# thu-ml/zhusuan

Hardware: NVIDIA H100
Metric: leapfrog-steps*chains/sec (higher is better)
Workload: dtype f32

## Files before the change

### include/zsb200.h

```cpp
#ifndef ZSB200_H_
#define ZSB200_H_
#include <stddef.h>
#include <stdint.h>

#ifdef __cplusplus
extern "C" {
#endif

#define ZSB_OK 0
#define ZSB_ERR_INVALID (-1)
#define ZSB_ERR_CUDA (-2)
#define ZSB_ERR_UNSUPPORTED (-3)

int zsb_version(void);
int zsb_last_error(char* buf, size_t n);
int zsb_device_count(void);
int zsb_stream_sync(void* stream);
int zsb_random_set_device_epoch(const uint32_t* epoch);
int zsb_random_bump_epoch(uint32_t* epoch, uint32_t by, void* stream);

enum {
  ZSB_HMC_STATE_T = 0, ZSB_HMC_STATE_STEP_SIZE = 1, ZSB_HMC_STATE_TUNER_STEP = 2,
  ZSB_HMC_STATE_LOG_EPS_BAR = 3, ZSB_HMC_STATE_H_BAR = 4, ZSB_HMC_STATE_MU = 5,
  ZSB_HMC_STATE_EWMV_T = 6, ZSB_HMC_STATE_EPS_USED = 7, ZSB_HMC_STATE_ACC_MEAN = 8,
  ZSB_HMC_STATE_FLAGS = 9 ,
  ZSB_HMC_STATE_SEARCH_LAST = 10, ZSB_HMC_STATE_SEARCH_COND = 11, ZSB_HMC_STATE_SIZE = 16
};

int zsb_logprob_normal_f32(const float* given, int64_t given_n, const float* mean, int64_t mean_n,
                           const float* logstd, int64_t logstd_n, float* out, int64_t n_out,
                           int64_t group, void* stream);
int zsb_logprob_normal_bwd_f32(const float* given, int64_t given_n, const float* mean,
                               int64_t mean_n, const float* logstd, int64_t logstd_n,
                               const float* gout, int64_t n_out, int64_t group, float* dgiven,
                               float* dmean, float* dlogstd, void* stream);
int zsb_logprob_bernoulli_f32(const float* given, int64_t given_n, const float* logits,
                              int64_t logits_n, float* out, int64_t n_out, int64_t group,
                              void* stream);
int zsb_logprob_bernoulli_bwd_f32(const float* given, int64_t given_n, const float* logits,
                                  int64_t logits_n, const float* gout, int64_t n_out,
                                  int64_t group, float* dlogits, void* stream);
int zsb_logprob_categorical_f32(const int32_t* given, int64_t given_n, const float* logits,
                                int64_t logits_rows, int64_t n_categories, float* out,
                                int64_t rows, void* stream);
int zsb_logprob_categorical_bwd_f32(const int32_t* given, int64_t given_n, const float* logits,
                                    int64_t logits_rows, int64_t n_categories, const float* gout,
                                    float* dlogits, int64_t rows, void* stream);
int zsb_logprob_dirichlet_f32(const float* given, int64_t given_rows, const float* alpha,
                              int64_t alpha_rows, int64_t n_categories, float* out, int64_t rows,
                              void* stream);
int zsb_logprob_dirichlet_bwd_given_f32(const float* given, int64_t given_rows,
                                        const float* alpha, int64_t alpha_rows,
                                        int64_t n_categories, const float* gout, float* dgiven,
                                        int64_t rows, void* stream);
int zsb_logprob_unnorm_multinomial_f32(const float* given, int64_t given_rows,
                                       const float* logits, int64_t logits_rows,
                                       int64_t n_categories, int normalize_logits, float* out,
                                       int64_t rows, void* stream);
int zsb_logprob_unnorm_multinomial_bwd_f32(const float* given, int64_t given_rows,
                                           const float* logits, int64_t logits_rows,
                                           int64_t n_categories, int normalize_logits,
                                           const float* gout, float* dlogits, int64_t rows,
                                           void* stream);
int zsb_logprob_mvn_chol_f32(const float* given, int64_t given_rows, const float* mean,
                             int64_t mean_rows, const float* cov_tril, int64_t tril_mats,
                             int64_t n_dim, float* out, float* x_out, int64_t rows, void* stream);
int zsb_logprob_mvn_chol_bwd_given_f32(const float* x_in, const float* cov_tril,
                                       int64_t tril_mats, int64_t n_dim, const float* gout,
                                       float* dgiven, int64_t rows, void* stream);
int zsb_group_sum_f32(const float* in, float* out, int64_t n_out, int64_t group, void* stream);

int zsb_reparam_normal_f32(const float* mean, int64_t mean_n, const float* logstd,
                           int64_t logstd_n, const float* eps, uint64_t seed, uint32_t iter,
                           float* z_out, float* eps_out, float* logq_out, int64_t n_out,
                           int64_t group, void* stream);
int zsb_sample_bernoulli_i32(const float* logits, int64_t logits_n, const float* u, uint64_t seed,
                             uint32_t iter, int32_t* out, int64_t n, void* stream);

int zsb_logprob_univariate_f32(int dist, const float* given, int64_t given_n, const float* a,
                               int64_t a_n, const float* b, int64_t b_n, float* out,
                               int64_t n_out, int64_t group, void* stream);
int zsb_logprob_univariate_bwd_f32(int dist, const float* given, int64_t given_n, const float* a,
                                   int64_t a_n, const float* b, int64_t b_n, const float* gout,
                                   int64_t n_out, int64_t group, float* dgiven, float* da,
                                   float* db, void* stream);

int zsb_reduce_fwd_f32(int op, const float* x, float* out, int64_t outer, int64_t K, int64_t inner,
                       void* stream);
int zsb_reduce_bwd_f32(int op, const float* x, const float* y, const float* gout, float* dx,
                       int64_t outer, int64_t K, int64_t inner, void* stream);

int zsb_vimco_signal_f32(const float* x, float* signal, float* lme, int64_t outer, int64_t K,
                         int64_t inner, void* stream);
int zsb_normalized_weights_f32(const float* x, float* w, int64_t outer, int64_t K, int64_t inner,
                               void* stream);

int zsb_linear_tc_kpad(int K);
int zsb_linear_tc_nparts(int J);
int zsb_split16_pad_f32(const float* src, int64_t rows, int K, void* planes, float* scale,
                        void* stream);
int zsb_linear_tc_slices(int64_t R, int J, int K);
int zsb_linear_tc_f32(int epi, const void* w_planes, const float* scale_w, const void* h_planes,
                      const float* scale_h, const float* bias, const float* x_obs, int64_t n_x,
                      const float* gout, float* out, float* part, int64_t R, int J, int K,
                      int relu, void* stream);
int zsb_linear_tc_amax_f32(int epi, const void* w_planes, const float* scale_w,
                           const void* h_planes, const float* scale_h, const float* bias,
                           const float* x_obs, int64_t n_x, const float* gout, float* out,
                           float* part, int64_t R, int J, int K, int relu, float* amax_scale,
                           void* stream);
int zsb_split16_dual_f32(const float* src, const float* mask_src, int64_t R, int K, void* planes,
                         float* col_sum, float* scale, int have_amax, void* stream);

int zsb_linear_tc_dgrad_f32(const void* w_planes, const float* scale_w, const void* g_planes,
                            const float* scale_g, int64_t R, int J, int K, float* out,
                            float* amax_scale, void* stream);
int zsb_linear_tc_wgrad_f32(const void* h_planes, const float* scale_h, int K,
                            const void* g_planes, const float* scale_g, int J, int64_t R,
                            float* out, float* part, void* stream);

int zsb_linear_tc_bern_sample_f32(const void* w_planes, const float* scale_w, const void* h_planes,
                                  const float* scale_h, int h_binary, const float* bias,
                                  const float* u_in, uint64_t seed, uint32_t iter, int S,
                                  void* h_out, int h_int, void* h_planes_out, float* logq,
                                  float* part, int64_t R, int J, int K, void* stream);
int zsb_linear_tc_bern_given_f32(int epi, const void* w_planes, const float* scale_w,
                                 const void* h_planes, const float* scale_h, int h_binary,
                                 const float* bias, const float* given, int S, const float* gout,
                                 float* out, float* part, int64_t R, int J, int K,
                                 float* amax_scale, void* stream);
int zsb_linear_tc_cat_sample_f32(const void* w_planes, const float* scale_w, const void* h_planes,
                                 const float* scale_h, int h_binary, const float* bias,
                                 const float* u_in, uint64_t seed, uint32_t iter, int S,
                                 int32_t* cls, void* onehot, int h_int, float* logq, int64_t R,
                                 int C, int K, void* stream);
int zsb_linear_tc_cat_given_f32(int epi, const void* w_planes, const float* scale_w,
                                const void* h_planes, const float* scale_h, int h_binary,
                                const float* bias, const float* given, int64_t n_g, int S,
                                const float* gout, float* out, int64_t R, int C, int K,
                                float* amax_scale, void* stream);
int zsb_linear_tc_normal_sample_f32(const void* w_planes, const float* scale_w,
                                    const void* h_planes, const float* scale_h, int h_binary,
                                    const float* bias, const float* eps_in, uint64_t seed,
                                    uint32_t iter, int S, float* z, float* logq, float* part,
                                    float* mean_out, float* logstd_out, int64_t R, int D, int K,
                                    float* amax_scale, void* stream);
int zsb_linear_normal_grad_f32(const float* logstd, const float* gz, const float* glq,
                               const float* eps_in, uint64_t seed, uint32_t iter,
                               const uint32_t* epoch, int reparam, int S, int64_t R, int D,
                               float* dpre, float* amax_scale, void* stream);
int zsb_linear_tc_bin_f32(int epi, const void* w_planes, const float* scale_w,
                          const void* h_planes, const float* scale_h, const float* bias,
                          const float* x_obs, int64_t n_x, const float* gout, float* out,
                          float* part, int64_t R, int J, int K, int relu, float* amax_scale,
                          void* stream);
int zsb_linear_tc_wgrad_bin_f32(const void* h_planes, const float* scale_h, int K,
                                const void* g_planes, const float* scale_g, int J, int64_t R,
                                float* out, float* part, void* stream);

int zsb_linear_tc_class_f32(const void* w_planes, const float* scale_w, const void* h_planes,
                            const float* scale_h, int h_binary, const float* bias,
                            const float* ctab, int C, const int32_t* cls, int64_t n_cls,
                            float* out, int64_t R, int J, int K, int relu, float* amax_scale,
                            void* stream);
int zsb_split16_class_f32(const float* src, const float* mask_src, int64_t R, int K,
                          const int32_t* cls, int64_t n_cls, int C, void* planes, float* col_sum,
                          float* dtab, float* scale, int have_amax, void* stream);

int zsb_split16_noisy_f32(const float* h, int64_t n_h, const float* noise, int64_t R, int K,
                          void* planes, float* scale, void* stream);
int zsb_linear_tc_bn_f32(int training, int bessel, const void* w_planes, const float* scale_w,
                         const void* h_planes, const float* scale_h, int h_binary,
                         const float* gamma, const float* beta, float* moving_mean,
                         float* moving_var, float rate, float eps, float* stats, float* a,
                         float* part, float* out, int64_t R, int J, int K, int relu,
                         float* amax_scale, void* stream);
int zsb_bn_finish_fused_f32(const float* a, const float* part, int64_t R, int J,
                            const float* gamma, const float* beta, float* moving_mean,
                            float* moving_var, float rate, float eps, float* stats, float* out,
                            int relu, float* amax_scale, void* stream);
int zsb_bn_grad_f32(int training, const float* g, const float* y, const float* a,
                    const float* stats, const float* gamma, int relu, int64_t R, int J,
                    float* part, float* dbeta, float* dgamma, void* planes, float* scale,
                    void* stream);
int zsb_bn_grad_f32out(int training, const float* g, const float* y, const float* a,
                       const float* stats, const float* gamma, int relu, int64_t R, int J,
                       float* part, float* dbeta, float* dgamma, float* da, float* scale,
                       void* stream);
int zsb_noisy_grad_f32(const float* d, const float* h, int64_t n_h, const float* noise, int64_t R,
                       int K, float* dnoise, float* dh, void* stream);

int zsb_effective_sample_size_f32(const float* samples, int64_t M, int64_t D, float* ess,
                                  void* stream);

int zsb_hmc_acc_parts(void);
int zsb_hmc_mass_parts(void);
int zsb_hmc_momentum_f32(float* p, const float* noise, const float* mass, int64_t mass_n,
                         int64_t chains, int64_t row_len, uint64_t seed, uint32_t iter,
                         uint32_t stream_id, int64_t row0, float* k_out, int accumulate,
                         const float* iter_state, void* stream);
int zsb_hmc_kinetic_f32(const float* p, const float* mass, int64_t mass_n, int64_t chains,
                        int64_t row_len, float* k_out, int accumulate, void* stream);
int zsb_hmc_leapfrog_q_f32(float* q, const float* p, const float* mass, int64_t mass_n,
                           int64_t row_len, const float* eps_dev, float scale, int64_t n,
                           void* stream);
int zsb_hmc_leapfrog_p_f32(float* p, const float* g, const float* eps_dev, float scale, int64_t n,
                           void* stream);
int zsb_hmc_mh_f32(const float* lp0, const float* lp1, const float* k0, const float* k1,
                   const float* u, uint64_t seed, uint32_t iter, int64_t row0, int64_t chains,
                   float* h0, float* h1, float* acc, int32_t* accept, float* lp_sel,
                   float* acc_part, int* n_part_out , float* state, void* stream);
int zsb_hmc_select_f32(float* q, const float* q_new, const int32_t* accept, int64_t chains,
                       int64_t row_len, void* stream);
int zsb_hmc_acc_sum_f32(const float* acc_part, int n_part, int64_t chains, float* stats,
                        void* stream);
int zsb_hmc_begin_f32(float* state, int start_search, void* stream);
int zsb_hmc_ewmv_bump_f32(float* state, void* stream);
int zsb_hmc_search_update_f32(float* state, const float* stats, float target, void* stream);
int zsb_hmc_tune_f32(float* state, const float* stats, int has_tuner, int adapt, float fresh_start,
                     float gamma, float t0, float kappa, float delta, float t_now, void* stream);
int zsb_hmc_mass_stats_f32(const float* q, const float* ewmv_mean, int64_t chains, int64_t D,
                           float* part, float* stats, void* stream);
int zsb_hmc_mass_update_f32(float* ewmv_mean, float* ewmv_var, float* mass, const float* stats,
                            float n_chains_global, int64_t D, float decay, float ewmv_t_new,
                            int adapt, int use_ones, float* state, void* stream);

int zsb_hmc_diag_normal_step_f32(float* q, const float* noise, const float* u, const float* mean,
                                 int64_t mean_n, const float* logstd, int64_t logstd_n,
                                 const float* mass, int64_t mass_n, float* state, int n_leapfrogs,
                                 int64_t chains, int64_t D, uint64_t seed, uint32_t iter,
                                 int64_t row0, int search_mode, float* p0_out, float* h0, float* h1,
                                 float* lp0, float* lp_sel, float* acc, int32_t* accept,
                                 float* acc_part, int* n_part_out , void* stream);

int zsb_hmc_dense_ntiles(int64_t D, int impl);
int zsb_hmc_dense_leapfrog_f32(const float* q_cur, const float* q_cur_lo, float* q_next,
                               float* q_next_lo, const float* p_in, float* p_out,
                               const float* P, const float* P_lo, const float* bvec,
                               const float* mu, const float* mass, const float* state,
                               float p_scale, float* lp_part, float* k_part, int64_t chains,
                               int64_t D, int impl, void* stream);
int zsb_hmc_dense_split_lo_f32(const float* q, float* lo, int64_t n, void* stream);
int zsb_hmc_dense_traj_prepare_f32(const float* q, const float* p, const float* mass, void* planes,
                                   float* scales, int64_t chains, int64_t D, void* stream);
int zsb_hmc_dense_leapfrog_h16_pass_f32(const float* q_cur, const void* q_cur_planes,
                                        float* q_next, void* q_next_planes, const float* p_in,
                                        float* p_out, const void* P_h16, const void* P_l16,
                                        float* scales, int pass_index, const float* bvec,
                                        const float* mu, const float* mass, const float* state,
                                        float p_scale, float* lp_part, float* k_part,
                                        int64_t chains, int64_t D, void* stream);
int zsb_hmc_dense_resident_h16_f32(void* planes0, void* planes1, void* spare0, void* spare1,
                                   const float* p0, float* pw, const void* P_h16,
                                   const void* P_l16, float* scales, const float* bvec,
                                   const float* mu, const float* mass, const float* state,
                                   float* lp0_part, float* lp1_part, float* k_part,
                                   int64_t chains, int64_t D, int n_leapfrogs, void* stream);
int zsb_hmc_dense_select_traj_planes_f32(float* q, const void* planes, const void* spare,
                                         const float* record, const int32_t* accept,
                                         int64_t chains, int64_t D, void* stream);
int zsb_hmc_dense_finish_f32(const float* lp_part, const float* k_part, int ntiles, int64_t chains,
                             float const_term, float* lp_out, float* k_out, void* stream);

int zsb_sample_categorical_i32(const float* logits, int64_t logit_rows, int64_t rows,
                               int64_t n_categories, int64_t n_samples, const float* u,
                               uint64_t seed, uint32_t iter, int32_t* out, void* stream);
int zsb_sample_dirichlet_f32(const float* alpha, int64_t alpha_rows, int64_t n_rows,
                             int64_t n_categories, const float* gammas, uint64_t seed,
                             uint32_t iter, float* out, void* stream);
int zsb_sample_gamma_f32(const float* alpha, int64_t alpha_rows, const float* beta,
                         int64_t beta_rows, int64_t n_rows, int64_t row_len, uint64_t seed,
                         uint32_t iter, float* out, void* stream);
int zsb_sample_base_noise_f32(int kind, float* out, int64_t n, uint64_t seed, uint32_t iter,
                              void* stream);
int zsb_sample_count_i32(int kind, const float* param, int64_t param_n, int64_t n_experiments,
                         const float* u, uint64_t seed, uint32_t iter, int32_t* out, int64_t n,
                         void* stream);

int zsb_lntm_phi_t_f32(const float* beta, int64_t n_topics, int64_t n_vocab, float* phi_t,
                       void* stream);
int zsb_lntm_logjoint_f32(const float* eta, const float* eta_mean, const float* eta_logstd,
                          const float* phi_t, const int64_t* doc_ptr, const int32_t* word_idx,
                          const float* word_cnt, const int64_t* doc_ids, const float* temperature,
                          float* lp_out, float* grad_out, int64_t chains, int64_t docs,
                          int64_t n_topics, void* stream);
int zsb_lntm_mstep_f32(const float* eta, const float* phi_t, const int64_t* doc_ptr,
                       const int32_t* word_idx, const float* word_cnt, const int64_t* doc_ids,
                       float* lp_out, float* ratio, float* theta, int64_t chains, int64_t docs,
                       int64_t nnz, int64_t n_topics, void* stream);
int zsb_lntm_mstep_grad_f32(const float* g, const float* ratio, const float* theta,
                            const float* phi_t, const int64_t* csc_ptr, const int32_t* csc_entry,
                            const int32_t* entry_doc, const int32_t* doc_slot, float* G,
                            float* dbeta, int64_t chains, int64_t docs, int64_t nnz,
                            int64_t n_topics, int64_t n_vocab, void* stream);

int zsb_pmf_logjoint_f32(const float* lat, const float* fixed, const int64_t* row_ptr,
                         const int32_t* col_idx, const float* rating, const int64_t* nbr_ptr,
                         const int32_t* nbr_idx, float logstd_lat, float logstd_fixed,
                         float logstd_rating, float* lp_out, float* grad_out, float* work,
                         int64_t K, int64_t n_rows, int64_t n_cols, int64_t D, int64_t chunk_size,
                         void* stream);

int zsb_planar_flow_fwd_f32(const float* z_in, const float* lq_in, const float* b,
                            const float* aux_u, const float* w, float* z_out, float* lq_out,
                            float* ck, int64_t R, int64_t d, int64_t n_iters, void* stream);
int zsb_planar_flow_warps(int64_t R, int64_t d, int64_t n_iters);
int zsb_planar_flow_bwd_f32(const float* ck, const float* gz_out, const float* glq,
                            const float* b, const float* aux_u, const float* w, float* gz_in,
                            float* part, float* db, float* daux_u, float* dw, int64_t R,
                            int64_t d, int64_t n_iters, void* stream);

int zsb_iaf_fwd_f32(const float* z_in, const float* lq_in, const float* m_w, const float* s_w,
                    float* z_out, float* lq_out, float* ck, int64_t R, int64_t d,
                    int64_t n_iters, int update, void* stream);
int zsb_iaf_slices(int64_t R, int64_t d, int64_t n_iters);
int zsb_iaf_bwd_f32(const float* ck, const float* gz_out, const float* glq, const float* m_w,
                    const float* s_w, float* gz_in, float* part, float* dm_w, float* ds_w,
                    int64_t R, int64_t d, int64_t n_iters, int update, void* stream);

int zsb_gp_cond_fwd_f32(const float* x, const float* z, const float* s, const float* Li,
                        const float* V, float* mean, float* stdv, float* A_out, int64_t B,
                        int64_t M, int64_t d, int64_t K, void* stream);
int zsb_gp_cond_parts(int64_t B, int64_t M, int64_t d, int64_t K);
int zsb_gp_cond_bwd_f32(const float* x, const float* z, const float* s, const float* Li,
                        const float* V, const float* A, const float* stdv, const float* g_mean,
                        const float* g_std, float* part, float* dz, float* ds, float* dLi,
                        float* dV, int64_t B, int64_t M, int64_t d, int64_t K, void* stream);

int zsb_conv3x3_fwd_f32(const float* x, const float* gate, const float* W, const float* b,
                        const float* residual, float* y, int64_t R, int64_t Hc, int64_t Wc,
                        int64_t Cin, int64_t Cout, int stride, int transpose, int relu,
                        void* stream);
int zsb_conv3x3_wgrad_parts(int64_t R, int64_t Hc, int64_t Wc, int stride);
int zsb_conv3x3_wgrad_f32(const float* big, const float* small, const float* gate, int grad_big,
                          float* part, float* dW, float* db, int64_t R, int64_t Hc, int64_t Wc,
                          int64_t Ca, int64_t Cb, int stride, void* stream);

int zsb_conv_gather_split_f32(const float* x, int64_t N, int64_t Hb, int64_t Wb, int64_t C,
                              int64_t Hs, int64_t Ws, int k, int stride, int pt, int pl,
                              void* planes, float* scale, int have_amax, void* stream);
int zsb_conv_col2im_f32(int epi, const float* cols, int64_t N, int64_t Hb, int64_t Wb, int64_t C,
                        int64_t Hs, int64_t Ws, int k, int stride, int pt, int pl,
                        const float* bias, const float* residual, const float* gamma,
                        const float* beta, const float* moving_mean, const float* moving_var,
                        float eps, int relu, float* stats, float* pre, float* part, float* out,
                        float* amax_scale, void* stream);
int zsb_conv_sigmoid_grad_f32(const float* g, const float* y, int64_t R, int C, float* gp,
                              float* part, float* db, float* scale, void* stream);
int zsb_conv_relu_grad_f32(const float* g, const float* y, int64_t R, int C, int relu, float* gp,
                           float* part, float* db, float* scale, void* stream);

int zsb_sgmcmc_parts(void);
int zsb_sgmcmc_sgld_f32(float* q, const float* g, const float* noise, float lr, int64_t chains,
                        int64_t row_len, uint64_t seed, uint32_t iter, int64_t row0,
                        void* stream);
int zsb_sgmcmc_psgld_f32(float* q, float* aux, const float* g, const float* noise, float lr,
                         float decay, float epsilon, int64_t chains, int64_t row_len,
                         uint64_t seed, uint32_t iter, int64_t row0, void* stream);
int zsb_sgmcmc_resample_v_f32(float* v, const float* noise, float lr, int64_t chains,
                              int64_t row_len, uint64_t seed, uint32_t iter, int64_t row0,
                              void* stream);
int zsb_sgmcmc_half_q_f32(float* q, const float* v, int64_t n, void* stream);
int zsb_sgmcmc_sghmc_f32(float* q, float* v, const float* g, const float* noise, float lr,
                         float alpha, float beta, int second_order, int64_t chains,
                         int64_t row_len, uint64_t seed, uint32_t iter, int64_t row0,
                         float* part, float* mean_k, void* stream);
int zsb_sgmcmc_sgnht_vec_f32(float* q, float* v, float* alpha, const float* g, const float* noise,
                             float lr, float a, float tune_rate, int second_order, int64_t chains,
                             int64_t row_len, uint64_t seed, uint32_t iter, int64_t row0,
                             float* mean_k_out, void* stream);
int zsb_sgmcmc_mean_sq_f32(const float* v, int64_t n, float* part, float* out, void* stream);
int zsb_sgmcmc_sgnht_scalar_f32(float* q, float* v, const float* alpha_eff, const float* g,
                                const float* noise, float lr, float a, int second_order,
                                int64_t chains, int64_t row_len, uint64_t seed, uint32_t iter,
                                int64_t row0, float* part, float* mean_k, void* stream);
int zsb_sgmcmc_sgnht_alpha_f32(float* out, const float* in, const float* mean_k, float coef,
                               float lr, void* stream);

int zsb_sgmcmc_sghmc_bnn_f32(float* w0, float* w1, float* v0, float* v1, const float* x,
                             const float* y, int B, int n_in, int H, const float* logstd0,
                             int64_t logstd0_n, const float* logstd1, int64_t logstd1_n,
                             float y_logstd, float n_train, float lr, float alpha, float beta,
                             int second_order, int resample, const float* noise0,
                             const float* noise1, const float* resample0, const float* resample1,
                             uint64_t seed, uint32_t iter, int64_t row0, float* part,
                             float* mean_k, int64_t chains, void* stream);

enum zsb_sgmcmc_method {
  ZSB_SGMCMC_SGHMC = 0,
  ZSB_SGMCMC_SGLD = 1,
  ZSB_SGMCMC_PSGLD = 2,
  ZSB_SGMCMC_SGNHT_VEC = 3,
  ZSB_SGMCMC_SGNHT_SCALAR = 4
};

int zsb_sgmcmc_bnn_step_f32(int method, float* w0, float* w1, float* v0, float* v1, float* aux0,
                            float* aux1, const float* alpha_eff0, const float* alpha_eff1,
                            const float* x, const float* y, int B, int n_in, int H,
                            const float* logstd0, int64_t logstd0_n, const float* logstd1,
                            int64_t logstd1_n, float y_logstd, float n_train, float lr,
                            float friction, float variance_estimate, float decay, float epsilon,
                            float variance_extra, float tune_rate, int second_order, int resample,
                            const float* noise0, const float* noise1, const float* resample0,
                            const float* resample1, uint64_t seed, uint32_t iter, int64_t row0,
                            float* part, float* mean_k0, float* mean_k1, int64_t chains,
                            void* stream);

int zsb_bnn_logjoint_f32(const float* w0, const float* w1, const float* x, const float* y,
                         int64_t B, int n_in, int H, const float* logstd0, int64_t logstd0_n,
                         const float* logstd1, int64_t logstd1_n, const float* y_logstd,
                         float n_train, float* lp, float* g0, float* g1, float* g_ylogstd,
                         float* y_mean, float* log_lik, int64_t K, void* stream);

#ifdef __cplusplus
}
#endif
#endif
```

### zhusuan_b200/_lib.py

```python
import ctypes
import os
import re

_HERE = os.path.dirname(os.path.abspath(__file__))
_ROOT = os.path.dirname(_HERE)
LIB_PATH = os.path.join(_HERE, "libzsb200.so")
HEADER_PATH = os.path.join(_ROOT, "include", "zsb200.h")

_CTYPES = {
    "int": ctypes.c_int, "int64_t": ctypes.c_int64, "uint64_t": ctypes.c_uint64,
    "uint32_t": ctypes.c_uint32, "int32_t": ctypes.c_int32,
    "float": ctypes.c_float, "size_t": ctypes.c_size_t,
}


def parse_header(path=HEADER_PATH):
    src = open(path).read()
    src = re.sub(r"/\*\s*host\s*\*/", " __host__ ", src)
    src = re.sub(r"/\*.*?\*/", " ", src, flags=re.S)
    protos = {}
    for m in re.finditer(r"\bint\s+(zsb_\w+)\s*\(([^)]*)\)\s*;", src):
        name, args = m.group(1), m.group(2).strip()
        sig = []
        if args and args != "void":
            for a in args.split(","):
                a = a.strip()
                host = "__host__" in a
                a = a.replace("__host__", "").strip()
                is_ptr = "*" in a
                toks = a.replace("*", " ").replace("const", " ").split()
                base, argname = toks[0], toks[-1]
                if is_ptr:
                    if host and base == "int":
                        ct = ctypes.POINTER(ctypes.c_int)
                    elif base == "char":
                        ct = ctypes.c_char_p
                    else:
                        ct = ctypes.c_void_p
                else:
                    ct = _CTYPES[base]
                sig.append((ct, argname, host))
        protos[name] = sig
    return protos


class ZsbError(RuntimeError):
    pass


class _Lib(object):
    def __init__(self):
        self._dll = None
        self.protos = parse_header()

    def load(self):
        if self._dll is None:
            if not os.path.exists(LIB_PATH):
                raise ZsbError(
                    "zhusuan_b200: %s is missing -- build it with "
                    "`python -c 'import __graft_entry__ as g; g.build()'` "
                    "(make -C zhusuan_b200/csrc).  There is no CPU fallback."
                    % LIB_PATH)
            dll = ctypes.CDLL(LIB_PATH)
            for name, sig in self.protos.items():
                fn = getattr(dll, name)
                fn.restype = ctypes.c_int
                fn.argtypes = [s[0] for s in sig]
            self._dll = dll
        return self._dll

    def last_error(self):
        buf = ctypes.create_string_buffer(512)
        self.load().zsb_last_error(buf, 512)
        return buf.value.decode("utf-8", "replace")

    _KERNELS = {"zsb_hmc_mass_stats_f32": 2, "zsb_hmc_dense_traj_prepare_f32": 3, "zsb_hmc_dense_resident_h16_f32": 1, "zsb_sgmcmc_sghmc_f32": 2,
                "zsb_sgmcmc_mean_sq_f32": 2, "zsb_sgmcmc_sgnht_scalar_f32": 2,
                "zsb_split16_pad_f32": 3, "zsb_linear_tc_f32": 2, "zsb_planar_flow_bwd_f32": 2,
                "zsb_iaf_bwd_f32": 2, "zsb_lntm_mstep_grad_f32": 2,
                "zsb_gp_cond_bwd_f32": 2, "zsb_conv3x3_wgrad_f32": 2,
                "zsb_conv_gather_split_f32": 3, "zsb_conv_sigmoid_grad_f32": 2,
                "zsb_conv_relu_grad_f32": 2,
                "zsb_linear_tc_bn_f32": 3, "zsb_bn_finish_fused_f32": 2, "zsb_bn_grad_f32": 5,
                "zsb_bn_grad_f32out": 3}
    launches = 0

    def call(self, name, *args):
        fn = getattr(self.load(), name)
        rc = fn(*args)
        self.launches += self._KERNELS.get(name, 1)
        if rc != 0:
            raise ZsbError("%s failed (%d): %s" % (name, rc, self.last_error()))
        return rc


lib = _Lib()


def ptr(t):
    if t is None:
        return None
    if not t.is_cuda:
        raise ZsbError(
            "zhusuan_b200 kernels need CUDA tensors (got a %s tensor); "
            "there is no CPU fallback." % t.device)
    if not t.is_contiguous():
        raise ZsbError("zhusuan_b200: non-contiguous tensor passed to a kernel")
    return t.data_ptr()


def stream():
    import torch
    return torch.cuda.current_stream().cuda_stream
```

### zhusuan_b200/csrc/hmc_dense.cu

```cuda
#include "common.cuh"

namespace {

constexpr int BM = 128, BN = 128, BK = 16;
constexpr int APAD = 4;


__global__ void __launch_bounds__(256, 2)
dense_leapfrog_simt_kernel(const float* __restrict__ q_cur, float* __restrict__ q_next,
                           const float* __restrict__ p_in, float* __restrict__ p_out,
                           const float* __restrict__ P, const float* __restrict__ bvec,
                           const float* __restrict__ mu, const float* __restrict__ mass,
                           const float* __restrict__ state, float p_scale,
                           float* __restrict__ lp_part, float* __restrict__ k_part,
                           int64_t chains, int D) {
  __shared__ __align__(16) float As[2][BK][BM + APAD];
  __shared__ __align__(16) float Bs[2][BK][BN];

  const int tid = threadIdx.x;
  const int tx = tid & 15, ty = tid >> 4;
  const int64_t m0 = (int64_t)blockIdx.y * BM;
  const int n0 = blockIdx.x * BN;

  const int a_row = tid >> 2;
  const int a_k4 = (tid & 3) * 4;
  const int b_row = tid >> 5;
  const int b_n4 = (tid & 31) * 4;

  float acc[8][8];
#pragma unroll
  for (int i = 0; i < 8; ++i)
#pragma unroll
    for (int j = 0; j < 8; ++j) acc[i][j] = 0.f;

  float4 a_reg[2], b_reg[2];
  auto load_tiles = [&](int k0) {
#pragma unroll
    for (int h = 0; h < 2; ++h) {
      const int64_t m = m0 + a_row + h * 64;
      a_reg[h] = (m < chains)
                     ? *reinterpret_cast<const float4*>(q_cur + m * D + k0 + a_k4)
                     : make_float4(0.f, 0.f, 0.f, 0.f);
      const int n = n0 + b_n4;
      b_reg[h] = (n < D) ? *reinterpret_cast<const float4*>(P + (int64_t)(k0 + b_row + h * 8) * D + n)
                         : make_float4(0.f, 0.f, 0.f, 0.f);
    }
  };
  auto store_tiles = [&](int buf) {
#pragma unroll
    for (int h = 0; h < 2; ++h) {
      const int r = a_row + h * 64;
      As[buf][a_k4 + 0][r] = a_reg[h].x;
      As[buf][a_k4 + 1][r] = a_reg[h].y;
      As[buf][a_k4 + 2][r] = a_reg[h].z;
      As[buf][a_k4 + 3][r] = a_reg[h].w;
      *reinterpret_cast<float4*>(&Bs[buf][b_row + h * 8][b_n4]) = b_reg[h];
    }
  };

  const int nk = D / BK;
  load_tiles(0);
  store_tiles(0);
  __syncthreads();
  for (int kt = 0; kt < nk; ++kt) {
    const int buf = kt & 1;
    if (kt + 1 < nk) load_tiles((kt + 1) * BK);
#pragma unroll
    for (int k = 0; k < BK; ++k) {
      const float4 a0 = *reinterpret_cast<const float4*>(&As[buf][k][ty * 4]);
      const float4 a1 = *reinterpret_cast<const float4*>(&As[buf][k][64 + ty * 4]);
      const float4 b0 = *reinterpret_cast<const float4*>(&Bs[buf][k][tx * 4]);
      const float4 b1 = *reinterpret_cast<const float4*>(&Bs[buf][k][64 + tx * 4]);
      const float a[8] = {a0.x, a0.y, a0.z, a0.w, a1.x, a1.y, a1.z, a1.w};
      const float b[8] = {b0.x, b0.y, b0.z, b0.w, b1.x, b1.y, b1.z, b1.w};
#pragma unroll
      for (int i = 0; i < 8; ++i)
#pragma unroll
        for (int j = 0; j < 8; ++j) acc[i][j] = fmaf(a[i], b[j], acc[i][j]);
    }
    if (kt + 1 < nk) store_tiles(buf ^ 1);
    __syncthreads();
  }

  const float eps = state[ZSB_ST_EPS_USED];
  const float s2 = mul(eps, p_scale);
#pragma unroll
  for (int i = 0; i < 8; ++i) {
    const int64_t m = m0 + (i < 4 ? ty * 4 + i : 64 + ty * 4 + (i - 4));
    float lp_acc = 0.f, k_acc = 0.f;
    if (m < chains) {
#pragma unroll
      for (int h = 0; h < 2; ++h) {
        const int n = n0 + h * 64 + tx * 4;
        if (n < D) {
          const float4 pv = *reinterpret_cast<const float4*>(p_in + m * D + n);
          const float4 qv = *reinterpret_cast<const float4*>(q_cur + m * D + n);
          const float4 ms = *reinterpret_cast<const float4*>(mass + n);
          float4 bv = make_float4(0.f, 0.f, 0.f, 0.f), mv = bv;
          if (bvec) bv = *reinterpret_cast<const float4*>(bvec + n);
          if (mu) mv = *reinterpret_cast<const float4*>(mu + n);
          const float pe[4] = {pv.x, pv.y, pv.z, pv.w}, qe[4] = {qv.x, qv.y, qv.z, qv.w};
          const float me[4] = {ms.x, ms.y, ms.z, ms.w}, be[4] = {bv.x, bv.y, bv.z, bv.w};
          const float ue[4] = {mv.x, mv.y, mv.z, mv.w};
          float pn[4], qn[4];
#pragma unroll
          for (int j = 0; j < 4; ++j) {
            const float g = sub(be[j], acc[i][h * 4 + j]);
            pn[j] = add(pe[j], mul(s2, g));
            qn[j] = add(qe[j], mul(eps, fdiv(pn[j], me[j])));
            lp_acc += (qe[j] - ue[j]) * g;
            k_acc += fdiv(mul(pn[j], pn[j]), me[j]);
          }
          *reinterpret_cast<float4*>(p_out + m * D + n) = make_float4(pn[0], pn[1], pn[2], pn[3]);
          if (q_next)
            *reinterpret_cast<float4*>(q_next + m * D + n) = make_float4(qn[0], qn[1], qn[2], qn[3]);
        }
      }
    }
    if (lp_part) {
#pragma unroll
      for (int o = 8; o > 0; o >>= 1) lp_acc += __shfl_xor_sync(0xffffffffu, lp_acc, o);
      if (tx == 0 && m < chains) lp_part[(int64_t)blockIdx.x * chains + m] = lp_acc;
    }
    if (k_part) {
#pragma unroll
      for (int o = 8; o > 0; o >>= 1) k_acc += __shfl_xor_sync(0xffffffffu, k_acc, o);
      if (tx == 0 && m < chains) k_part[(int64_t)blockIdx.x * chains + m] = k_acc;
    }
  }
}

__global__ void __launch_bounds__(256) dense_finish_kernel(const float* __restrict__ lp_part,
                                                           const float* __restrict__ k_part,
                                                           int ntiles, int64_t chains,
                                                           float const_term,
                                                           float* __restrict__ lp_out,
                                                           float* __restrict__ k_out) {
  for (int64_t c = (int64_t)blockIdx.x * blockDim.x + threadIdx.x; c < chains;
       c += (int64_t)gridDim.x * blockDim.x) {
    if (lp_part && lp_out) {
      float s = 0.f;
      for (int t = 0; t < ntiles; ++t) s += lp_part[(int64_t)t * chains + c];
      lp_out[c] = add(mul(0.5f, s), const_term);
    }
    if (k_part && k_out) {
      float s = 0.f;
      for (int t = 0; t < ntiles; ++t) s += k_part[(int64_t)t * chains + c];
      k_out[c] = mul(0.5f, s);
    }
  }
}

}

int zsb_dense_leapfrog_tc_launch(const float* q_cur, const float* q_cur_lo, float* q_next,
                                 float* q_next_lo, const float* p_in, float* p_out,
                                 const float* P_hi, const float* P_lo, const float* bvec,
                                 const float* mu, const float* mass, const float* state,
                                 float p_scale, float* lp_part, float* k_part, int64_t chains,
                                 int D, cudaStream_t st);
int zsb_dense_split_lo_launch(const float* q, float* lo, int64_t n, cudaStream_t st);
int zsb_dense_tc_ntiles(int D);
int zsb_dense_leapfrog_h16_launch(const float* q_cur, const void* q_cur_planes, float* q_next,
                                  void* q_next_planes, const float* p_in, float* p_out,
                                  const void* P_h16, const void* P_l16, float* scales,
                                  int pass_index, const float* bvec, const float* mu,
                                  const float* mass, const float* state, float p_scale,
                                  float* lp_part, float* k_part, int64_t chains, int D,
                                  cudaStream_t st);
int zsb_dense_h16_prepare_launch(const float* q, const float* p, const float* mass, void* planes,
                                 float* scales, int64_t chains, int64_t D, cudaStream_t st);
int zsb_dense_res_h16_launch(void* planes0, void* planes1, void* spare0, void* spare1,
                             const float* p0, float* pw, const void* P_h16, const void* P_l16,
                             float* scales, const float* bvec, const float* mu, const float* mass,
                             const float* state, float* lp0_part, float* lp1_part, float* k_part,
                             int64_t chains, int D, int L, cudaStream_t st);
int zsb_dense_select_planes_launch(float* q, const void* planes, const void* spare,
                                   const float* record, const int32_t* accept, int64_t chains,
                                   int64_t D, cudaStream_t st);

extern "C" {

int zsb_hmc_dense_ntiles(int64_t D, int impl) {
  if (impl == 1) return zsb_dense_tc_ntiles((int)D);
  return (int)zsb_ceil_div(D, BN);
}

int zsb_hmc_dense_leapfrog_f32(const float* q_cur, const float* q_cur_lo, float* q_next,
                               float* q_next_lo, const float* p_in, float* p_out,
                               const float* P, const float* P_lo, const float* bvec,
                               const float* mu, const float* mass, const float* state,
                               float p_scale, float* lp_part, float* k_part, int64_t chains,
                               int64_t D, int impl, void* stream) {
  ZSB_REQUIRE(q_cur && p_in && p_out && P && mass && state, "zsb_hmc_dense_leapfrog_f32: null arg");
  ZSB_REQUIRE(chains > 0 && D > 0 && D % BK == 0 && D <= (1 << 20),
              "zsb_hmc_dense_leapfrog_f32: D must be a positive multiple of 16");
  ZSB_REQUIRE(q_next != q_cur, "zsb_hmc_dense_leapfrog_f32: q_next must not alias q_cur");
  cudaStream_t st = (cudaStream_t)stream;
  if (impl == 1) {
    ZSB_REQUIRE(P_lo && q_cur_lo, "zsb_hmc_dense_leapfrog_f32: impl 1 needs the P_lo / q_lo splits");
    return zsb_dense_leapfrog_tc_launch(q_cur, q_cur_lo, q_next, q_next_lo, p_in, p_out, P, P_lo,
                                        bvec, mu, mass, state, p_scale, lp_part, k_part, chains,
                                        (int)D, st);
  }
  ZSB_REQUIRE(impl == 0, "zsb_hmc_dense_leapfrog_f32: unknown impl %d", impl);
  dim3 grid((unsigned)zsb_ceil_div(D, BN), (unsigned)zsb_ceil_div(chains, BM));
  dense_leapfrog_simt_kernel<<<grid, 256, 0, st>>>(q_cur, q_next, p_in, p_out, P, bvec, mu, mass,
                                                   state, p_scale, lp_part, k_part, chains, (int)D);
  return zsb_check_launch("hmc_dense_leapfrog_simt");
}

int zsb_hmc_dense_split_lo_f32(const float* q, float* lo, int64_t n, void* stream) {
  ZSB_REQUIRE(q && lo && n >= 0, "zsb_hmc_dense_split_lo_f32: bad args");
  if (n == 0) return ZSB_OK;
  return zsb_dense_split_lo_launch(q, lo, n, (cudaStream_t)stream);
}

int zsb_hmc_dense_traj_prepare_f32(const float* q, const float* p, const float* mass, void* planes,
                                   float* scales, int64_t chains, int64_t D, void* stream) {
  ZSB_REQUIRE(q && p && mass && planes && scales && chains > 0 && D > 0,
              "zsb_hmc_dense_traj_prepare_f32: bad args");
  return zsb_dense_h16_prepare_launch(q, p, mass, planes, scales, chains, D,
                                      (cudaStream_t)stream);
}
int zsb_hmc_dense_leapfrog_h16_pass_f32(const float* q_cur, const void* q_cur_planes,
                                        float* q_next, void* q_next_planes, const float* p_in,
                                        float* p_out, const void* P_h16, const void* P_l16,
                                        float* scales, int pass_index, const float* bvec,
                                        const float* mu, const float* mass, const float* state,
                                        float p_scale, float* lp_part, float* k_part,
                                        int64_t chains, int64_t D, void* stream) {
  ZSB_REQUIRE(q_cur && p_in && p_out && P_h16 && P_l16 && mass && state && scales,
              "zsb_hmc_dense_leapfrog_h16_pass_f32: null arg");
  ZSB_REQUIRE(q_next != q_cur, "zsb_hmc_dense_leapfrog_h16_pass_f32: q_next must not alias q_cur");
  ZSB_REQUIRE(pass_index >= 0, "zsb_hmc_dense_leapfrog_h16_pass_f32: pass_index < 0");
  return zsb_dense_leapfrog_h16_launch(q_cur, q_cur_planes, q_next, q_next_planes, p_in, p_out,
                                       P_h16, P_l16, scales, pass_index, bvec, mu, mass, state,
                                       p_scale, lp_part, k_part, chains, (int)D,
                                       (cudaStream_t)stream);
}

int zsb_hmc_dense_resident_h16_f32(void* planes0, void* planes1, void* spare0, void* spare1,
                                   const float* p0, float* pw, const void* P_h16,
                                   const void* P_l16, float* scales, const float* bvec,
                                   const float* mu, const float* mass, const float* state,
                                   float* lp0_part, float* lp1_part, float* k_part,
                                   int64_t chains, int64_t D, int n_leapfrogs, void* stream) {
  ZSB_REQUIRE(planes0 && planes1 && spare0 && spare1 && p0 && pw && P_h16 && P_l16 && scales &&
                  mass && state && lp0_part && lp1_part && k_part,
              "zsb_hmc_dense_resident_h16_f32: null arg");
  ZSB_REQUIRE(p0 != pw, "zsb_hmc_dense_resident_h16_f32: aliased buffers");
  return zsb_dense_res_h16_launch(planes0, planes1, spare0, spare1, p0, pw, P_h16, P_l16, scales,
                                  bvec, mu, mass, state, lp0_part, lp1_part, k_part, chains, (int)D,
                                  n_leapfrogs, (cudaStream_t)stream);
}
int zsb_hmc_dense_select_traj_planes_f32(float* q, const void* planes, const void* spare,
                                         const float* record, const int32_t* accept,
                                         int64_t chains, int64_t D, void* stream) {
  ZSB_REQUIRE(q && planes && spare && record && accept && chains > 0 && D > 0 && D % 2 == 0,
              "zsb_hmc_dense_select_traj_planes_f32: bad args");
  return zsb_dense_select_planes_launch(q, planes, spare, record, accept, chains, D,
                                        (cudaStream_t)stream);
}

int zsb_hmc_dense_finish_f32(const float* lp_part, const float* k_part, int ntiles, int64_t chains,
                             float const_term, float* lp_out, float* k_out, void* stream) {
  ZSB_REQUIRE(chains > 0 && ntiles > 0, "zsb_hmc_dense_finish_f32: bad sizes");
  int64_t blocks = zsb_ceil_div(chains, 256);
  if (blocks > ZSB_NUM_SMS * 8) blocks = ZSB_NUM_SMS * 8;
  dense_finish_kernel<<<(unsigned)blocks, 256, 0, (cudaStream_t)stream>>>(
      lp_part, k_part, ntiles, chains, const_term, lp_out, k_out);
  return zsb_check_launch("hmc_dense_finish");
}

}
```

### zhusuan_b200/csrc/hmc_dense_epilogue.cuh

```cuda
#pragma once
#include "tc_common.cuh"

namespace {

constexpr int kScaleHdr = 8, kScaleRec = 4;
constexpr float kPlaneKeep = 65280.f;
constexpr float kHalfOverflow = 65520.f;

__device__ __forceinline__ const float* scale_rec(const float* scales, int pass) {
  return scales + kScaleHdr + kScaleRec * pass;
}
__device__ __forceinline__ bool plane_spare_in(const float* scales, int pass) {
  return pass > 0 && __float_as_uint(scale_rec(scales, pass)[3]) != 0u;
}
__device__ __forceinline__ float plane_scale_in(const float* scales, int pass) {
  return scale_rec(scales, pass)[plane_spare_in(scales, pass) ? 1 : 0];
}
__device__ __forceinline__ float next_plane_scale(const float* __restrict__ scales, int pass,
                                                  float eps, float s2, float sq) {
  const float* r = scale_rec(scales, pass);
  const float mq = r[2];
  const float drift = pass == 0 ? eps * r[3] : mq + r[2 - kScaleRec];
  const float bound = mq + drift + eps * s2 * scales[7] * (scales[5] + scales[4] * mq);
  if (bound * sq < kPlaneKeep || !(bound <= 3.0e38f)) return sq;
  return pow2_plane_scale(bound);
}
__device__ __forceinline__ void publish_plane_scale(float* __restrict__ scales, int pass,
                                                    float sq_next, float sq_alt, float qmax,
                                                    bool overflow, int quarter, int lane) {
  unsigned int* r = reinterpret_cast<unsigned int*>(scales + kScaleHdr + kScaleRec * (pass + 1));
  const float mq = warp_max(qmax);
  const bool any_overflow = __any_sync(0xffffffffu, overflow);
  if (lane == 0) {
    atomicMax(r + 2, __float_as_uint(mq));
    if (any_overflow) atomicOr(r + 3, 1u);
  }
  if (blockIdx.x == 0 && quarter == 0 && lane == 0) {
    reinterpret_cast<float*>(r)[0] = sq_next;
    reinterpret_cast<float*>(r)[1] = sq_alt;
    r[kScaleRec + 2] = 0u;
    r[kScaleRec + 3] = 0u;
  }
}

struct EpiArgs {
  const float* __restrict__ q_cur; float* __restrict__ q_next; float* __restrict__ q_next_lo;
  const float* __restrict__ p_in; float* __restrict__ p_out;
  float* __restrict__ lp_part; float* __restrict__ k_part;
  int64_t chains; int D;
  float acc_scale; float q_scale;
};
template <int H16>
__device__ __forceinline__ void store_split(const EpiArgs& a, float* __restrict__ lo_f32,
                                            __half* __restrict__ hi_pl, __half* __restrict__ lo_pl,
                                            uint32_t off, float qn) {
  if (H16) {
    const float x = qn * a.q_scale;
    const __half h = __float2half_rn(x);
    hi_pl[off] = h;
    lo_pl[off] = __float2half_rn(x - __half2float(h));
  } else {
    lo_f32[off] = qn - __uint_as_float(__float_as_uint(qn) & 0xFFFFE000u);
  }
}
template <int MODE, int DC, int H16>
__device__ __forceinline__ void epilogue_half_tile(const EpiArgs& a, uint32_t trow, int n,
                                                   bool n_ok, int64_t c0, int64_t part_row,
                                                   int lane, float s2, float eps_over_m,
                                                   float inv_m, float b_n, float mu_n,
                                                   float& amax) {
  constexpr int NCOL = BN;
  const uint32_t D = DC ? (uint32_t)DC : (uint32_t)a.D;
  const int64_t chains = a.chains;
  const bool has_next = a.q_next != nullptr;
  const bool warp_n_ok = __all_sync(0xffffffffu, n_ok);
  const bool fast_tile = warp_n_ok && (c0 + NCOL <= chains);

  const int64_t off_t = c0 * (int64_t)D + n;
  const float* __restrict__ pin0 = a.p_in + off_t;
  const float* __restrict__ qc0 = a.q_cur + off_t;
  float* __restrict__ po0 = a.p_out + off_t;
  float* __restrict__ qn0 = has_next ? a.q_next + off_t : nullptr;
  float* __restrict__ lo0 = (has_next && H16 == 0) ? a.q_next_lo + off_t : nullptr;
  __half* __restrict__ hi_pl0 =
      (has_next && H16 == 1) ? reinterpret_cast<__half*>(a.q_next_lo) + off_t : nullptr;
  __half* __restrict__ lo_pl0 = (has_next && H16 == 1) ? hi_pl0 + chains * (int64_t)D : nullptr;

  auto compute = [&](const uint32_t* v, const float* pe, const float* qe, int c) {
    const size_t cb = (size_t)c * D;
    float* __restrict__ po = po0 + cb;
    float* __restrict__ qn_p = has_next ? qn0 + cb : nullptr;
    float* __restrict__ lo_p = (has_next && H16 == 0) ? lo0 + cb : nullptr;
    __half* __restrict__ hp = (has_next && H16 == 1) ? hi_pl0 + cb : nullptr;
    __half* __restrict__ lp = (has_next && H16 == 1) ? lo_pl0 + cb : nullptr;
    float lpv[MODE >= 1 ? 16 : 1], kv[MODE >= 2 ? 16 : 1];
#pragma unroll
    for (int j = 0; j < 16; ++j) {
      const float g = b_n - a.acc_scale * __uint_as_float(v[j]);
      const float pn = fmaf(s2, g, pe[j]);
      po[(uint32_t)j * D] = pn;
      if (MODE >= 1) lpv[j] = (qe[j] - mu_n) * g;
      if (MODE >= 2) kv[j] = pn * pn * inv_m;
      if (has_next) {
        const float qn = fmaf(eps_over_m, pn, qe[j]);
        qn_p[(uint32_t)j * D] = qn;
        if (H16 == 1) amax = fmaxf(amax, fabsf(qn));
        store_split<H16>(a, lo_p, hp, lp, (uint32_t)j * D, qn);
      }
    }
    if (MODE >= 1) {
      const float sum = warp_transpose_sum16(lpv, lane);
      if (lane < 16) a.lp_part[part_row + c0 + c + lane] = sum;
    }
    if (MODE >= 2) {
      const float sum = warp_transpose_sum16(kv, lane);
      if (lane < 16) a.k_part[part_row + c0 + c + lane] = sum;
    }
  };
  auto load = [&](float* pe, float* qe, int c) {
    const float* __restrict__ pin = pin0 + (size_t)c * D;
    const float* __restrict__ qc = qc0 + (size_t)c * D;
#pragma unroll
    for (int j = 0; j < 16; ++j) {
      pe[j] = __ldcs(pin + (uint32_t)j * D);
      qe[j] = __ldg(qc + (uint32_t)j * D);
    }
  };

  if (fast_tile) {
    float pa[16], qa[16], pb[16], qb[16];
    uint32_t va[16], vb[16];
    load(pa, qa, 0);
#pragma unroll 1
    for (int c = 0; c < NCOL; c += 32) {
      load(pb, qb, c + 16);
      acc_ld16(trow + 4u * (uint32_t)c, va);
      compute(va, pa, qa, c);
      if (c + 32 < NCOL) load(pa, qa, c + 32);
      acc_ld16(trow + 4u * (uint32_t)(c + 16), vb);
      compute(vb, pb, qb, c + 16);
    }
  } else {
#pragma unroll 1
    for (int c = 0; c < NCOL; c += 16) {
      uint32_t v[16];
      acc_ld16(trow + 4u * (uint32_t)c, v);
      const int64_t cbase = c0 + c;
      if (cbase < chains) {
        const size_t cb = (size_t)c * D;
        float pe[16], qe[16];
        float lpv[MODE >= 1 ? 16 : 1], kv[MODE >= 2 ? 16 : 1];
#pragma unroll
        for (int j = 0; j < 16; ++j) {
          const bool ok = n_ok && cbase + j < chains;
          pe[j] = ok ? pin0[cb + (uint32_t)j * D] : 0.f;
          qe[j] = ok ? qc0[cb + (uint32_t)j * D] : 0.f;
        }
#pragma unroll
        for (int j = 0; j < 16; ++j) {
          const bool ok = n_ok && cbase + j < chains;
          const float g = b_n - a.acc_scale * __uint_as_float(v[j]);
          const float pn = fmaf(s2, g, pe[j]);
          if (MODE >= 1) lpv[j] = ok ? (qe[j] - mu_n) * g : 0.f;
          if (MODE >= 2) kv[j] = ok ? pn * pn * inv_m : 0.f;
          if (ok) {
            po0[cb + (uint32_t)j * D] = pn;
            if (has_next) {
              const float qn = fmaf(eps_over_m, pn, qe[j]);
              qn0[cb + (uint32_t)j * D] = qn;
              if (H16 == 1) amax = fmaxf(amax, fabsf(qn));
              store_split<H16>(a, lo0 + cb, hi_pl0 + cb, lo_pl0 + cb, (uint32_t)j * D, qn);
            }
          }
        }
        if (MODE >= 1) {
          const float sum = warp_transpose_sum16(lpv, lane);
          if (lane < 16 && cbase + lane < chains) a.lp_part[part_row + cbase + lane] = sum;
        }
        if (MODE >= 2) {
          const float sum = warp_transpose_sum16(kv, lane);
          if (lane < 16 && cbase + lane < chains) a.k_part[part_row + cbase + lane] = sum;
        }
      }
    }
  }
}

}
```

### zhusuan_b200/csrc/hmc_dense_res.cu

```cuda
#include "hmc_dense_epilogue.cuh"

namespace {

struct ResEpi {
  const __half* __restrict__ hi_cur; const __half* __restrict__ lo_cur;
  __half* __restrict__ hi_nxt; __half* __restrict__ lo_nxt;
  const __half* __restrict__ hi_cur_s; const __half* __restrict__ lo_cur_s;
  __half* __restrict__ hi_nxt_s; __half* __restrict__ lo_nxt_s;
  const float* __restrict__ p_in; float* __restrict__ p_out;
  float* __restrict__ lp_part; float* __restrict__ k_part;
  int64_t chains; int D;
  float sq, inv_sq, acc_scale;
  float rescale;
};

template <int MODE, int NEXT, int DC, bool SPARE>
__device__ __forceinline__ void epilogue_planes(const ResEpi& a, uint32_t trow, int n, bool n_ok,
                                                int64_t c0, int64_t part_row, int lane, float s2,
                                                float eps_over_m_sq, float inv_m, float b_n,
                                                float mu_n, float& qmax) {
  constexpr int NCOL = BN;
  const uint32_t D = DC ? (uint32_t)DC : (uint32_t)a.D;
  const int64_t chains = a.chains;
  const bool warp_n_ok = __all_sync(0xffffffffu, n_ok);
  const bool fast_tile = warp_n_ok && (c0 + NCOL <= chains);
  const int64_t off_t = c0 * (int64_t)D + n;
  const float* __restrict__ pin0 = a.p_in + off_t;
  float* __restrict__ po0 = a.p_out + off_t;
  const unsigned short* __restrict__ hc0 =
      reinterpret_cast<const unsigned short*>(a.hi_cur) + off_t;
  const unsigned short* __restrict__ lc0 =
      reinterpret_cast<const unsigned short*>(a.lo_cur) + off_t;
  __half* __restrict__ hn0 = NEXT ? a.hi_nxt + off_t : nullptr;
  __half* __restrict__ ln0 = NEXT ? a.lo_nxt + off_t : nullptr;
  __half* __restrict__ hs0 = SPARE ? a.hi_nxt_s + off_t : nullptr;
  __half* __restrict__ ls0 = SPARE ? a.lo_nxt_s + off_t : nullptr;

  auto element = [&](float acc, float p, uint32_t hl, float& pn, float& lpv, float& kv,
                     float& Qn) {
    const float Q = __half2float(__ushort_as_half((unsigned short)(hl & 0xFFFFu))) +
                    __half2float(__ushort_as_half((unsigned short)(hl >> 16)));
    const float g = b_n - a.acc_scale * acc;
    pn = fmaf(s2, g, p);
    if (MODE >= 1) lpv = (Q * a.inv_sq - mu_n) * g;
    if (MODE >= 2) kv = pn * pn * inv_m;
    if (NEXT) Qn = fmaf(eps_over_m_sq, pn, Q);
  };

  if (fast_tile) {
    auto load = [&](float* pe, uint32_t* he, int c) {
      const size_t cb = (size_t)c * D;
#pragma unroll
      for (int j = 0; j < 16; ++j) {
        pe[j] = __ldcg(pin0 + cb + (uint32_t)j * D);
        const uint32_t h = __ldcg(hc0 + cb + (uint32_t)j * D);
        const uint32_t l = __ldcg(lc0 + cb + (uint32_t)j * D);
        he[j] = h | (l << 16);
      }
    };
    float ss_a = 0.f, ss_b = 0.f;
    auto compute = [&](const uint32_t* v, const float* pe, const uint32_t* he, int c, float& ss) {
      const size_t cb = (size_t)c * D;
      float lpv[MODE >= 1 ? 16 : 1], kv[MODE >= 2 ? 16 : 1];
#pragma unroll
      for (int j = 0; j < 16; j += 2) {
        float pn[2], lp1[2] = {0.f, 0.f}, k1[2] = {0.f, 0.f}, Qn[2] = {0.f, 0.f};
#pragma unroll
        for (int t = 0; t < 2; ++t) {
          element(__uint_as_float(v[j + t]), pe[j + t], he[j + t], pn[t], lp1[t], k1[t], Qn[t]);
          po0[cb + (uint32_t)(j + t) * D] = pn[t];
          if (MODE >= 1) lpv[j + t] = lp1[t];
          if (MODE >= 2) kv[j + t] = k1[t];
          if (NEXT && !SPARE) ss = fmaf(Qn[t], Qn[t], ss);
          if (SPARE) qmax = fmaxf(qmax, fabsf(Qn[t]));
        }
        if (NEXT) {
          const __half2 h2 = __floats2half2_rn(Qn[0], Qn[1]);
          const float2 hf = __half22float2(h2);
          const __half2 l2 = __floats2half2_rn(Qn[0] - hf.x, Qn[1] - hf.y);
          hn0[cb + (uint32_t)j * D] = __low2half(h2);
          hn0[cb + (uint32_t)(j + 1) * D] = __high2half(h2);
          ln0[cb + (uint32_t)j * D] = __low2half(l2);
          ln0[cb + (uint32_t)(j + 1) * D] = __high2half(l2);
        }
        if (SPARE) {
          const float x0 = Qn[0] * a.rescale, x1 = Qn[1] * a.rescale;
          const __half2 h2 = __floats2half2_rn(x0, x1);
          const float2 hf = __half22float2(h2);
          const __half2 l2 = __floats2half2_rn(x0 - hf.x, x1 - hf.y);
          hs0[cb + (uint32_t)j * D] = __low2half(h2);
          hs0[cb + (uint32_t)(j + 1) * D] = __high2half(h2);
          ls0[cb + (uint32_t)j * D] = __low2half(l2);
          ls0[cb + (uint32_t)(j + 1) * D] = __high2half(l2);
        }
      }
      if (MODE >= 1) {
        const float sum = warp_transpose_sum16(lpv, lane);
        if (lane < 16) a.lp_part[part_row + c0 + c + lane] = sum;
      }
      if (MODE >= 2) {
        const float sum = warp_transpose_sum16(kv, lane);
        if (lane < 16) a.k_part[part_row + c0 + c + lane] = sum;
      }
    };
    float pa[16], pb[16];
    uint32_t ha[16], hb[16], va[16], vb[16];
    load(pa, ha, 0);
#pragma unroll 1
    for (int c = 0; c < NCOL; c += 32) {
      load(pb, hb, c + 16);
      acc_ld16(trow + 4u * (uint32_t)c, va);
      compute(va, pa, ha, c, ss_a);
      if (c + 32 < NCOL) load(pa, ha, c + 32);
      acc_ld16(trow + 4u * (uint32_t)(c + 16), vb);
      compute(vb, pb, hb, c + 16, ss_b);
    }
    if (NEXT && !SPARE) {
      const float norm = sqrtf(ss_a + ss_b) * (1.f + 0x1p-10f);
      qmax = fmaxf(qmax, norm == norm ? norm : INFINITY);
    }
  } else {
#pragma unroll 1
    for (int c = 0; c < NCOL; c += 16) {
      uint32_t v[16];
      acc_ld16(trow + 4u * (uint32_t)c, v);
      const int64_t cbase = c0 + c;
      if (cbase < chains) {
        const size_t cb = (size_t)c * D;
        float lpv[MODE >= 1 ? 16 : 1], kv[MODE >= 2 ? 16 : 1];
#pragma unroll
        for (int j = 0; j < 16; ++j) {
          const bool ok = n_ok && cbase + j < chains;
          float p = 0.f;
          uint32_t hl = 0u;
          if (ok) {
            p = __ldcg(pin0 + cb + (uint32_t)j * D);
            hl = (uint32_t)__ldcg(hc0 + cb + (uint32_t)j * D) |
                 ((uint32_t)__ldcg(lc0 + cb + (uint32_t)j * D) << 16);
          }
          float pn, lp1 = 0.f, k1 = 0.f, Qn = 0.f;
          element(__uint_as_float(v[j]), p, hl, pn, lp1, k1, Qn);
          const __half hh = __float2half_rn(Qn);
          const __half ll = __float2half_rn(Qn - __half2float(hh));
          if (NEXT && ok) qmax = fmaxf(qmax, fabsf(Qn));
          if (MODE >= 1) lpv[j] = ok ? lp1 : 0.f;
          if (MODE >= 2) kv[j] = ok ? k1 : 0.f;
          if (ok) {
            po0[cb + (uint32_t)j * D] = pn;
            if (NEXT) {
              hn0[cb + (uint32_t)j * D] = hh;
              ln0[cb + (uint32_t)j * D] = ll;
            }
            if (SPARE) {
              const float x = Qn * a.rescale;
              const __half hs = __float2half_rn(x);
              hs0[cb + (uint32_t)j * D] = hs;
              ls0[cb + (uint32_t)j * D] = __float2half_rn(x - __half2float(hs));
            }
          }
        }
        if (MODE >= 1) {
          const float sum = warp_transpose_sum16(lpv, lane);
          if (lane < 16 && cbase + lane < chains) a.lp_part[part_row + cbase + lane] = sum;
        }
        if (MODE >= 2) {
          const float sum = warp_transpose_sum16(kv, lane);
          if (lane < 16 && cbase + lane < chains) a.k_part[part_row + cbase + lane] = sum;
        }
      }
    }
  }
}


struct ProducerState {
  int spare_in, n0, c0;
};
__device__ __forceinline__ ProducerState& producer_state() {
  __shared__ ProducerState ps;
  return ps;
}

template <int MODE, int NEXT, int DC, int CX, int CY>
struct ResW {
  static constexpr int KIND = 1, RB = 64, MNA = 0, MNB = 0;
  static constexpr int CLUSTER = CX * CY;
  static constexpr int KE = RB / 2;
  static constexpr uint32_t TX = Cfg<RB>::STAGE;
  CUtensorMap m_phi, m_plo, m_qhi, m_qlo, m_shi, m_slo;
  ResEpi ea;
  const float* bvec; const float* mu; const float* mass; const float* state;
  float* scales;
  float p_scale;
  int n_blk, D_rt, pass;
  struct EpiState { float qmax = 0.f; };

  __device__ __forceinline__ int D() const { return DC ? DC : D_rt; }
  __host__ __device__ __forceinline__ int64_t units() const {
    return ((ea.chains + BN - 1) / BN) * (int64_t)n_blk;
  }
  __device__ __forceinline__ void tile(int64_t u, int& nb, int64_t& cb) const {
    const uint64_t cu = (uint64_t)u / CLUSTER;
    const int r = (int)((uint64_t)u % CLUSTER);
    const uint32_t nbx = (uint32_t)(n_blk / CX);
    nb = (int)(cu % nbx) * CX + r % CX;
    cb = (int64_t)(cu / nbx) * CY + r / CX;
  }
  __device__ __forceinline__ void kb_range(int64_t, int& kb0, int& kb1) const {
    kb0 = 0;
    kb1 = D() / KE;
  }
  __device__ __forceinline__ void prefetch() const {
    tma_prefetch_desc(&m_phi); tma_prefetch_desc(&m_plo);
    tma_prefetch_desc(&m_qhi); tma_prefetch_desc(&m_qlo);
    tma_prefetch_desc(&m_shi); tma_prefetch_desc(&m_slo);
    producer_state().spare_in = plane_spare_in(scales, pass);
  }
  __device__ __forceinline__ void load(int64_t u, int kb, uint32_t sa, uint32_t fb) const {
    using C = Cfg<RB>;
    ProducerState& ps = producer_state();
    if (kb == 0) {
      int nb;
      int64_t cb;
      tile(u, nb, cb);
      ps.n0 = nb * BM;
      ps.c0 = (int)cb * BN;
    }
    const int n0 = ps.n0, c0 = ps.c0;
    const bool s = ps.spare_in != 0;
    const CUtensorMap* qh = s ? &m_shi : &m_qhi;
    const CUtensorMap* ql = s ? &m_slo : &m_qlo;
    const int r = (int)(u % CLUSTER), rx = r % CX, ry = r / CX;
    if constexpr (CY == 1) {
      tma_load_2d(sa, &m_phi, fb, kb * KE, n0);
      tma_load_2d(sa + C::A_TILE, &m_plo, fb, kb * KE, n0);
    } else {
      constexpr int rows = BM / CY;
      uint16_t mask = 0;
#pragma unroll
      for (int y = 0; y < CY; ++y) mask |= (uint16_t)(1u << (y * CX + rx));
      const uint32_t o = (uint32_t)(ry * rows * RB);
      tma_load_2d_mc(sa + o, &m_phi, fb, kb * KE, n0 + ry * rows, mask);
      tma_load_2d_mc(sa + C::A_TILE + o, &m_plo, fb, kb * KE, n0 + ry * rows, mask);
    }
    if constexpr (CX == 1) {
      tma_load_2d(sa + 2 * C::A_TILE, qh, fb, kb * KE, c0);
      tma_load_2d(sa + 2 * C::A_TILE + C::B_TILE, ql, fb, kb * KE, c0);
    } else {
      constexpr int rows = BN / CX;
      const uint16_t mask = (uint16_t)(((1u << CX) - 1u) << (ry * CX));
      const uint32_t o = (uint32_t)(rx * rows * RB);
      tma_load_2d_mc(sa + 2 * C::A_TILE + o, qh, fb, kb * KE, c0 + rx * rows, mask);
      tma_load_2d_mc(sa + 2 * C::A_TILE + C::B_TILE + o, ql, fb, kb * KE, c0 + rx * rows, mask);
    }
  }
  __device__ __forceinline__ float sq_alt(float eps, float sq) const {
    return next_plane_scale(scales, pass, eps, mul(eps, p_scale), sq);
  }
  __device__ __forceinline__ void epilogue(int64_t u, uint32_t trow, int quarter, int lane,
                                           EpiState& st) const {
    int nb;
    int64_t cb;
    tile(u, nb, cb);
    const int n = nb * BM + quarter * 32 + lane;
    const int64_t c0 = cb * BN;
    const bool n_ok = n < D();
    const float eps = state[ZSB_ST_EPS_USED];
    const float s2 = mul(eps, p_scale);
    const bool spare_in = plane_spare_in(scales, pass);
    const float sq = plane_scale_in(scales, pass);
    const float m_n = n_ok ? mass[n] : 1.f;
    const float eps_over_m_sq = mul(fdiv(eps, m_n), sq);
    const float inv_m = fdiv(1.f, m_n);
    const float b_n = (n_ok && bvec) ? bvec[n] : 0.f;
    const float mu_n = (n_ok && mu) ? mu[n] : 0.f;
    const int64_t part_row = (int64_t)(nb * 4 + quarter) * ea.chains;
    ResEpi a = ea;
    if (spare_in) {
      a.hi_cur = ea.hi_cur_s;
      a.lo_cur = ea.lo_cur_s;
    }
    a.sq = sq;
    a.inv_sq = fdiv(1.f, sq);
    a.acc_scale = 1.f / (scales[3] * sq);
    a.rescale = NEXT ? sq_alt(eps, sq) * a.inv_sq : 1.f;
    if (a.rescale == 1.f)
      epilogue_planes<MODE, NEXT, DC, false>(a, trow, n, n_ok, c0, part_row, lane, s2,
                                             eps_over_m_sq, inv_m, b_n, mu_n, st.qmax);
    else
      epilogue_planes<MODE, NEXT, DC, true>(a, trow, n, n_ok, c0, part_row, lane, s2,
                                            eps_over_m_sq, inv_m, b_n, mu_n, st.qmax);
  }
  __device__ __forceinline__ void epi_finish(EpiState& st, int quarter, int lane) const {
    if (!NEXT) return;
    const float sq = plane_scale_in(scales, pass);
    const float alt = sq_alt(state[ZSB_ST_EPS_USED], sq);
    publish_plane_scale(scales, pass, sq, alt, st.qmax * (1.f / sq),
                        alt != sq && !(st.qmax < kHalfOverflow), quarter, lane);
  }
};

constexpr int RES_CX = 2, RES_CY = 1;

template <int DC, int CX, int CY>
int res_pass(const CUtensorMap& phi, const CUtensorMap& plo, const CUtensorMap& qhi,
             const CUtensorMap& qlo, const CUtensorMap& shi, const CUtensorMap& slo,
             const ResEpi& ea, const float* bvec, const float* mu, const float* mass,
             const float* state, float* scales, int pass, float p_scale, int n_blk, int D,
             int mode, cudaStream_t st) {
  if (mode == 1) {
    const ResW<1, 1, DC, CX, CY> w{phi, plo, qhi, qlo, shi, slo, ea, bvec, mu, mass, state,
                                   scales, p_scale, n_blk, D, pass};
    return tc_launch(w, st, "hmc_dense_resident");
  }
  if (mode == 0) {
    const ResW<0, 1, DC, CX, CY> w{phi, plo, qhi, qlo, shi, slo, ea, bvec, mu, mass, state,
                                   scales, p_scale, n_blk, D, pass};
    return tc_launch(w, st, "hmc_dense_resident");
  }
  const ResW<2, 0, DC, CX, CY> w{phi, plo, qhi, qlo, shi, slo, ea, bvec, mu, mass, state, scales,
                                 p_scale, n_blk, D, pass};
  return tc_launch(w, st, "hmc_dense_resident");
}

template <int DC>
int res_pass(bool cluster, const CUtensorMap& phi, const CUtensorMap& plo, const CUtensorMap& qhi,
             const CUtensorMap& qlo, const CUtensorMap& shi, const CUtensorMap& slo,
             const ResEpi& ea, const float* bvec, const float* mu, const float* mass,
             const float* state, float* scales, int pass, float p_scale, int n_blk, int D,
             int mode, cudaStream_t st) {
  return cluster ? res_pass<DC, RES_CX, RES_CY>(phi, plo, qhi, qlo, shi, slo, ea, bvec, mu, mass,
                                                state, scales, pass, p_scale, n_blk, D, mode, st)
                 : res_pass<DC, 1, 1>(phi, plo, qhi, qlo, shi, slo, ea, bvec, mu, mass, state,
                                      scales, pass, p_scale, n_blk, D, mode, st);
}

__global__ void __launch_bounds__(256) select_planes_kernel(float* __restrict__ q,
                                                            const __half* __restrict__ planes,
                                                            const __half* __restrict__ spare,
                                                            const float* __restrict__ record,
                                                            const int32_t* __restrict__ accept,
                                                            int64_t chains, int64_t D) {
  const bool use_spare = __float_as_uint(record[3]) != 0u;
  const float inv_sq = 1.f / record[use_spare ? 1 : 0];
  if (use_spare) planes = spare;
  const int lane = threadIdx.x & 31;
  const int n8 = (int)(D >> 3);
  const int64_t wstride = (int64_t)gridDim.x * 8;
  for (int64_t c = (int64_t)blockIdx.x * 8 + (threadIdx.x >> 5); c < chains; c += wstride) {
    if (!accept[c]) continue;
    const uint4* __restrict__ hi = reinterpret_cast<const uint4*>(planes + c * D);
    const uint4* __restrict__ lo = reinterpret_cast<const uint4*>(planes + (chains + c) * D);
    float4* __restrict__ qr = reinterpret_cast<float4*>(q + c * D);
    for (int i0 = lane; i0 < n8; i0 += 128) {
      uint4 h[4], l[4];
#pragma unroll
      for (int u = 0; u < 4; ++u) {
        const int i = i0 + 32 * u;
        if (i < n8) { h[u] = __ldcs(hi + i); l[u] = __ldcs(lo + i); }
      }
#pragma unroll
      for (int u = 0; u < 4; ++u) {
        const int i = i0 + 32 * u;
        if (i < n8) {
          const uint32_t hw[4] = {h[u].x, h[u].y, h[u].z, h[u].w};
          const uint32_t lw[4] = {l[u].x, l[u].y, l[u].z, l[u].w};
          float o[8];
#pragma unroll
          for (int k = 0; k < 4; ++k) {
            const float2 hf = __half22float2(*reinterpret_cast<const __half2*>(&hw[k]));
            const float2 lf = __half22float2(*reinterpret_cast<const __half2*>(&lw[k]));
            o[2 * k] = (hf.x + lf.x) * inv_sq;
            o[2 * k + 1] = (hf.y + lf.y) * inv_sq;
          }
          qr[2 * i] = make_float4(o[0], o[1], o[2], o[3]);
          qr[2 * i + 1] = make_float4(o[4], o[5], o[6], o[7]);
        }
      }
    }
  }
}

}

int zsb_dense_res_h16_launch(void* planes0, void* planes1, void* spare0, void* spare1,
                             const float* p0, float* pw,
                             const void* P_h16, const void* P_l16, float* scales,
                             const float* bvec, const float* mu, const float* mass,
                             const float* state, float* lp0_part, float* lp1_part, float* k_part,
                             int64_t chains, int D, int L, cudaStream_t st) {
  if (D % 64 != 0 || D < 64 || L < 1 || chains <= 0 || chains >= (1LL << 31)) {
    zsb_set_error("dense_res: needs D %% 64 == 0, n_leapfrogs >= 1");
    return ZSB_ERR_INVALID;
  }
  if (planes0 == planes1 || !spare0 || !spare1 || spare0 == spare1) {
    zsb_set_error("dense_res: planes1, spare0 and spare1 must be separate work buffers");
    return ZSB_ERR_INVALID;
  }
  const int n_blk = (D + BM - 1) / BM;
  const int64_t c_blk = (chains + BN - 1) / BN;
  const bool cluster = n_blk % RES_CX == 0 && c_blk % RES_CY == 0;
  const uint32_t p_box = cluster ? BM / RES_CY : BM, q_box = cluster ? BN / RES_CX : BN;
  CUtensorMap phi, plo, qhi[2], qlo[2], shi[2], slo[2];
  int rc;
  constexpr int RB = ResW<0, 1, 0, 1, 1>::RB;
  if ((rc = make_map(&phi, P_h16, (uint64_t)D, (uint64_t)D, p_box, RB, 1))) return rc;
  if ((rc = make_map(&plo, P_l16, (uint64_t)D, (uint64_t)D, p_box, RB, 1))) return rc;
  __half* pl[2] = {reinterpret_cast<__half*>(planes0), reinterpret_cast<__half*>(planes1)};
  __half* sp[2] = {reinterpret_cast<__half*>(spare0), reinterpret_cast<__half*>(spare1)};
  const int64_t plane = chains * (int64_t)D;
  for (int b = 0; b < 2; ++b) {
    if ((rc = make_map(&qhi[b], pl[b], (uint64_t)chains, (uint64_t)D, q_box, RB, 1))) return rc;
    if ((rc = make_map(&qlo[b], pl[b] + plane, (uint64_t)chains, (uint64_t)D, q_box, RB, 1)))
      return rc;
    if ((rc = make_map(&shi[b], sp[b], (uint64_t)chains, (uint64_t)D, q_box, RB, 1))) return rc;
    if ((rc = make_map(&slo[b], sp[b] + plane, (uint64_t)chains, (uint64_t)D, q_box, RB, 1)))
      return rc;
  }
  for (int i = 0; i <= L; ++i) {
    const bool last = i == L;
    const int buf = i & 1;
    const ResEpi ea{pl[buf], pl[buf] + plane, pl[buf ^ 1], pl[buf ^ 1] + plane,
                    sp[buf], sp[buf] + plane, sp[buf ^ 1], sp[buf ^ 1] + plane,
                    i == 0 ? p0 : pw, pw, i == 0 ? lp0_part : lp1_part, k_part, chains, D,
                    1.f, 1.f, 1.f, 1.f};
    const int mode = last ? 2 : (i == 0 ? 1 : 0);
    const float p_scale = (i > 0 && !last) ? 1.f : 0.5f;
    rc = (D == 1024)
             ? res_pass<1024>(cluster, phi, plo, qhi[buf], qlo[buf], shi[buf], slo[buf], ea, bvec,
                              mu, mass, state, scales, i, p_scale, n_blk, D, mode, st)
             : res_pass<0>(cluster, phi, plo, qhi[buf], qlo[buf], shi[buf], slo[buf], ea, bvec, mu,
                           mass, state, scales, i, p_scale, n_blk, D, mode, st);
    if (rc != ZSB_OK) return rc;
  }
  return ZSB_OK;
}

#ifdef ZSB_PASS_PROFILE
extern "C" int zsb_pass_profile_read(unsigned long long* host, int ctas) {
  if (ctas < 0 || ctas > PASS_PROF_CTAS) return ZSB_ERR_INVALID;
  const size_t bytes = sizeof(unsigned long long) * PASS_PROF_SLOTS * (size_t)ctas;
  if (cudaMemcpyFromSymbol(host, g_pass_prof, bytes) != cudaSuccess) return ZSB_ERR_CUDA;
  static unsigned long long zeros[PASS_PROF_CTAS * PASS_PROF_SLOTS];
  if (cudaMemcpyToSymbol(g_pass_prof, zeros, sizeof(zeros)) != cudaSuccess) return ZSB_ERR_CUDA;
  return ZSB_OK;
}
#endif

int zsb_dense_select_planes_launch(float* q, const void* planes, const void* spare,
                                   const float* record, const int32_t* accept, int64_t chains,
                                   int64_t D, cudaStream_t st) {
  ZSB_REQUIRE(D % 8 == 0, "zsb_dense_select_planes: D must be a multiple of 8");
  int64_t blocks = zsb_ceil_div(chains, 8);
  if (blocks > ZSB_NUM_SMS * 16) blocks = ZSB_NUM_SMS * 16;
  if (blocks < 1) blocks = 1;
  select_planes_kernel<<<(unsigned)blocks, 256, 0, st>>>(
      q, reinterpret_cast<const __half*>(planes), reinterpret_cast<const __half*>(spare), record,
      accept, chains, D);
  return zsb_check_launch("hmc_select_planes");
}
```

### zhusuan_b200/csrc/hmc_dense_tc.cu

```cuda
#include "hmc_dense_epilogue.cuh"

namespace {

template <int OP, int MODE, int DC>
struct DenseW {
  static constexpr int KIND = OP, RB = 128, MNA = 0, MNB = 0;
  static constexpr int KE = OP ? RB / 2 : RB / 4;
  static constexpr uint32_t TX = Cfg<RB>::STAGE;
  CUtensorMap m_phi, m_plo, m_qhi, m_qlo;
  EpiArgs ea;
  const float* bvec; const float* mu; const float* mass; const float* state;
  float* scales;
  float p_scale;
  int n_blk, D_rt, pass_index;
  struct EpiState { float amax = 0.f; };

  __device__ __forceinline__ int D() const { return DC ? DC : D_rt; }
  __host__ __device__ __forceinline__ int64_t units() const {
    return ((ea.chains + BN - 1) / BN) * (int64_t)n_blk;
  }
  __device__ __forceinline__ void kb_range(int64_t, int& kb0, int& kb1) const {
    kb0 = 0;
    kb1 = D() / KE;
  }
  __device__ __forceinline__ void prefetch() const {
    tma_prefetch_desc(&m_phi);
    tma_prefetch_desc(&m_plo);
    tma_prefetch_desc(&m_qhi);
    tma_prefetch_desc(&m_qlo);
  }
  __device__ __forceinline__ void load(int64_t u, int kb, uint32_t sa, uint32_t fb) const {
    using C = Cfg<RB>;
    const int n0 = (int)(u % n_blk) * BM;
    const int c0 = (int)(u / n_blk) * BN;
    tma_load_2d(sa, &m_phi, fb, kb * KE, n0);
    tma_load_2d(sa + C::A_TILE, &m_plo, fb, kb * KE, n0);
    tma_load_2d(sa + 2 * C::A_TILE, &m_qhi, fb, kb * KE, c0);
    tma_load_2d(sa + 2 * C::A_TILE + C::B_TILE, &m_qlo, fb, kb * KE, c0);
  }
  __device__ __forceinline__ void epilogue(int64_t u, uint32_t trow, int quarter, int lane,
                                           EpiState& st) const {
    const int nb = (int)(u % n_blk);
    const int n = nb * BM + quarter * 32 + lane;
    const int64_t c0 = (u / n_blk) * BN;
    const int Dv = D();
    const bool n_ok = n < Dv;
    const float eps = state[ZSB_ST_EPS_USED];
    const float s2 = mul(eps, p_scale);
    const float m_n = n_ok ? mass[n] : 1.f;
    const float eps_over_m = fdiv(eps, m_n);
    const float inv_m = fdiv(1.f, m_n);
    const float b_n = (n_ok && bvec) ? bvec[n] : 0.f;
    const float mu_n = (n_ok && mu) ? mu[n] : 0.f;
    const int64_t part_row = (int64_t)(nb * 4 + quarter) * ea.chains;
    EpiArgs a = ea;
    if (OP == 1) {
      const float sq = scale_rec(scales, pass_index)[0];
      a.acc_scale = 1.f / (scales[3] * sq);
      a.q_scale = ea.q_next ? next_plane_scale(scales, pass_index, eps, s2, sq) : sq;
    }
    epilogue_half_tile<MODE, DC, OP>(a, trow, n, n_ok, c0, part_row, lane, s2, eps_over_m, inv_m,
                                     b_n, mu_n, st.amax);
  }
  __device__ __forceinline__ void epi_finish(EpiState& st, int quarter, int lane) const {
    if (OP == 1 && ea.q_next) {
      const float eps = state[ZSB_ST_EPS_USED];
      const float sq = next_plane_scale(scales, pass_index, eps, mul(eps, p_scale),
                                        scale_rec(scales, pass_index)[0]);
      publish_plane_scale(scales, pass_index, sq, sq, st.amax, false, quarter, lane);
    }
  }
};

__global__ void __launch_bounds__(256) split_lo_kernel(const float* __restrict__ q,
                                                       float* __restrict__ lo, int64_t n4) {
  for (int64_t i = (int64_t)blockIdx.x * blockDim.x + threadIdx.x; i < n4;
       i += (int64_t)gridDim.x * blockDim.x) {
    const float4 v = reinterpret_cast<const float4*>(q)[i];
    float4 r;
    r.x = v.x - __uint_as_float(__float_as_uint(v.x) & 0xFFFFE000u);
    r.y = v.y - __uint_as_float(__float_as_uint(v.y) & 0xFFFFE000u);
    r.z = v.z - __uint_as_float(__float_as_uint(v.z) & 0xFFFFE000u);
    r.w = v.w - __uint_as_float(__float_as_uint(v.w) & 0xFFFFE000u);
    reinterpret_cast<float4*>(lo)[i] = r;
  }
}

__global__ void __launch_bounds__(256) absmax_kernel(const float* __restrict__ q,
                                                     const float* __restrict__ p,
                                                     const float* __restrict__ mass, int64_t n,
                                                     int64_t D, float* __restrict__ scales) {
  float mq = 0.f, mv = 0.f;
  for (int64_t i = (int64_t)blockIdx.x * blockDim.x + threadIdx.x; i < n;
       i += (int64_t)gridDim.x * blockDim.x) {
    mq = finite_absmax(mq, q[i]);
    mv = finite_absmax(mv, fdiv(p[i], mass[i % D]));
  }
  mq = warp_max(mq);
  mv = warp_max(mv);
  if ((threadIdx.x & 31) == 0) {
    atomicMax(reinterpret_cast<unsigned int*>(scales) + 2, __float_as_uint(mq));
    atomicMax(reinterpret_cast<unsigned int*>(scales) + 6, __float_as_uint(mv));
  }
}
__global__ void scale_kernel(float* __restrict__ scales, const float* __restrict__ mass,
                             int64_t D) {
  float w = 0.f;
  for (int64_t i = threadIdx.x; i < D; i += 32) w = finite_absmax(w, fdiv(1.f, mass[i]));
  w = warp_max(w);
  if (threadIdx.x != 0) return;
  unsigned int* u = reinterpret_cast<unsigned int*>(scales);
  const float mq = __uint_as_float(u[2]), mv = __uint_as_float(u[6]);
  const float sq = pow2_plane_scale(mq);
  scales[0] = sq;
  scales[1] = 1.f / (scales[3] * sq);
  u[2] = 0u;
  float* r0 = scales + kScaleHdr;
  r0[0] = sq;
  r0[1] = sq;
  r0[2] = mq;
  r0[3] = mv;
  u[kScaleHdr + kScaleRec + 2] = 0u;
  u[kScaleHdr + kScaleRec + 3] = 0u;
  scales[7] = w;
  u[6] = 0u;
}
__global__ void __launch_bounds__(256) split16_kernel(const float* __restrict__ q,
                                                      __half* __restrict__ planes, int64_t n,
                                                      const float* __restrict__ scales) {
  const float sq = scales[0];
  for (int64_t i = (int64_t)blockIdx.x * blockDim.x + threadIdx.x; i < n;
       i += (int64_t)gridDim.x * blockDim.x) {
    const float x = q[i] * sq;
    const __half h = __float2half_rn(x);
    planes[i] = h;
    planes[n + i] = __float2half_rn(x - __half2float(h));
  }
}

template <int OP>
int launch_dense(const float* q_cur, const void* q_lo, float* q_next, void* q_next_lo,
                 const float* p_in, float* p_out, const void* P_hi, const void* P_lo,
                 const float* bvec, const float* mu, const float* mass, const float* state,
                 float p_scale, float* lp_part, float* k_part, int64_t chains, int D, float* scales,
                 int pass_index, cudaStream_t st, const char* what) {
  if (k_part && !lp_part) {
    zsb_set_error("%s: k_part requires lp_part", what);
    return ZSB_ERR_INVALID;
  }
  constexpr int RB = DenseW<OP, 0, 0>::RB;
  CUtensorMap m_phi, m_plo, m_qhi, m_qlo;
  int rc;
  if ((rc = make_map(&m_phi, P_hi, (uint64_t)D, (uint64_t)D, BM, RB, OP))) return rc;
  if ((rc = make_map(&m_plo, P_lo, (uint64_t)D, (uint64_t)D, BM, RB, OP))) return rc;
  const void* qh = OP ? q_lo : (const void*)q_cur;
  const void* ql = OP ? (const void*)(reinterpret_cast<const __half*>(q_lo) + chains * D) : q_lo;
  if ((rc = make_map(&m_qhi, qh, (uint64_t)chains, (uint64_t)D, BN, RB, OP))) return rc;
  if ((rc = make_map(&m_qlo, ql, (uint64_t)chains, (uint64_t)D, BN, RB, OP))) return rc;
  const EpiArgs ea{q_cur, q_next, reinterpret_cast<float*>(q_next_lo), p_in, p_out, lp_part,
                   k_part, chains, D, 1.f, 1.f};
  const int n_blk = (D + BM - 1) / BM;
#define ZSB_DENSE(MODE, DCV)                                                                   \
  do {                                                                                         \
    const DenseW<OP, MODE, DCV> w{m_phi, m_plo, m_qhi, m_qlo, ea, bvec, mu, mass, state,       \
                                  scales, p_scale, n_blk, D, pass_index};                      \
    return tc_launch(w, st, what);                                                             \
  } while (0)
#define ZSB_DENSE_MODE(DCV)                                                                    \
  do {                                                                                         \
    if (k_part) ZSB_DENSE(2, DCV);                                                             \
    else if (lp_part) ZSB_DENSE(1, DCV);                                                       \
    else ZSB_DENSE(0, DCV);                                                                    \
  } while (0)
  if constexpr (OP == 1)
    if (D == 1024) ZSB_DENSE_MODE(1024);
  ZSB_DENSE_MODE(0);
#undef ZSB_DENSE_MODE
#undef ZSB_DENSE
}

}

int zsb_dense_tc_ntiles(int D) { return 4 * ((D + BM - 1) / BM); }

int zsb_dense_leapfrog_tc_launch(const float* q_cur, const float* q_cur_lo, float* q_next,
                                 float* q_next_lo, const float* p_in, float* p_out,
                                 const float* P_hi, const float* P_lo, const float* bvec,
                                 const float* mu, const float* mass, const float* state,
                                 float p_scale, float* lp_part, float* k_part, int64_t chains,
                                 int D, cudaStream_t st) {
  if (D % 32 != 0 || D < 32) {
    zsb_set_error("dense_tc: D must be a multiple of 32");
    return ZSB_ERR_INVALID;
  }
  if (chains >= (1LL << 31) || (q_next && !q_next_lo) || !q_cur_lo) {
    zsb_set_error("dense_tc: bad arguments");
    return ZSB_ERR_INVALID;
  }
  return launch_dense<0>(q_cur, q_cur_lo, q_next, q_next_lo, p_in, p_out, P_hi, P_lo, bvec, mu,
                         mass, state, p_scale, lp_part, k_part, chains, D, nullptr, 0, st,
                         "hmc_dense_leapfrog_tc");
}

int zsb_dense_split_lo_launch(const float* q, float* lo, int64_t n, cudaStream_t st) {
  if (n % 4 != 0) {
    zsb_set_error("dense split: element count must be a multiple of 4");
    return ZSB_ERR_INVALID;
  }
  const int64_t n4 = n / 4;
  int64_t blocks = zsb_ceil_div(n4, 256);
  if (blocks > ZSB_NUM_SMS * 16) blocks = ZSB_NUM_SMS * 16;
  if (blocks < 1) blocks = 1;
  split_lo_kernel<<<(unsigned)blocks, 256, 0, st>>>(q, lo, n4);
  return zsb_check_launch("hmc_dense_split_lo");
}

int zsb_dense_leapfrog_h16_launch(const float* q_cur, const void* q_cur_planes, float* q_next,
                                  void* q_next_planes, const float* p_in, float* p_out,
                                  const void* P_h16, const void* P_l16, float* scales,
                                  int pass_index, const float* bvec, const float* mu,
                                  const float* mass, const float* state, float p_scale,
                                  float* lp_part, float* k_part, int64_t chains, int D,
                                  cudaStream_t st) {
  if (D % 64 != 0 || D < 64) {
    zsb_set_error("dense_h16: D must be a multiple of 64");
    return ZSB_ERR_INVALID;
  }
  if (chains >= (1LL << 31) || (q_next && !q_next_planes) || !q_cur_planes || !scales ||
      pass_index < 0) {
    zsb_set_error("dense_h16: bad arguments");
    return ZSB_ERR_INVALID;
  }
  return launch_dense<1>(q_cur, q_cur_planes, q_next, q_next_planes, p_in, p_out, P_h16, P_l16,
                         bvec, mu, mass, state, p_scale, lp_part, k_part, chains, D, scales,
                         pass_index, st, "hmc_dense_leapfrog_h16");
}

int zsb_dense_h16_prepare_launch(const float* q, const float* p, const float* mass, void* planes,
                                 float* scales, int64_t chains, int64_t D, cudaStream_t st) {
  const int64_t n = chains * D;
  int64_t blocks = zsb_ceil_div(n, 256 * 8);
  if (blocks > ZSB_NUM_SMS * 16) blocks = ZSB_NUM_SMS * 16;
  if (blocks < 1) blocks = 1;
  absmax_kernel<<<(unsigned)blocks, 256, 0, st>>>(q, p, mass, n, D, scales);
  scale_kernel<<<1, 32, 0, st>>>(scales, mass, D);
  split16_kernel<<<(unsigned)blocks, 256, 0, st>>>(q, reinterpret_cast<__half*>(planes), n, scales);
  return zsb_check_launch("hmc_dense_h16_prepare");
}
```

### zhusuan_b200/csrc/tc_common.cuh

```cuda
#pragma once
#include "common.cuh"
#include <cuda.h>
#include <cuda_fp16.h>

namespace {

constexpr int BM = 128;
constexpr int BN = 128;
constexpr int NUM_EPI_WARPS = 4;
constexpr int PRODUCER_WARP = 4;
constexpr int EPI_WARP0 = 5;
constexpr int NUM_THREADS = 32 * (EPI_WARP0 + NUM_EPI_WARPS);
constexpr int ACC_LD = BN + 4;
constexpr int ACC_BYTES = BM * ACC_LD * 4;
constexpr unsigned long long WAIT_TIMEOUT_NS = 2000000000ULL;

enum PassProfSlot {
  PROF_MMA_TOTAL,
  PROF_MMA_FULL,
  PROF_MMA_TEMPTY,
  PROF_MMA_STORE,
  PROF_PROD_EMPTY,
  PROF_EPI_TFULL,
  PROF_EPI_UNIT,
  PROF_UNITS,
  PASS_PROF_SLOTS
};
constexpr int PASS_PROF_CTAS = 1024;
#ifdef ZSB_PASS_PROFILE
constexpr bool kPassProfile = true;
__device__ unsigned long long g_pass_prof[PASS_PROF_CTAS * PASS_PROF_SLOTS];
#else
constexpr bool kPassProfile = false;
#endif
__device__ __forceinline__ long long prof_clock() {
  if constexpr (kPassProfile) return clock64();
  return 0;
}
__device__ __forceinline__ void prof_add(int slot, long long v) {
#ifdef ZSB_PASS_PROFILE
  if (blockIdx.x < PASS_PROF_CTAS)
    atomicAdd(&g_pass_prof[blockIdx.x * PASS_PROF_SLOTS + slot], (unsigned long long)v);
#endif
}

template <int RB>
struct Cfg {
  static constexpr int A_TILE = BM * RB;
  static constexpr int B_TILE = BN * RB;
  static constexpr int STAGE = 2 * A_TILE + 2 * B_TILE;
  static constexpr int STAGES = RB == 128 ? 2 : 5;
  static constexpr int ALIGN = RB == 128 ? 1024 : 512;
  static constexpr int SMEM = STAGES * STAGE + ACC_BYTES + 128 + ALIGN;
  static_assert(SMEM <= 227 * 1024, "operand ring exceeds shared memory");
};

__device__ __forceinline__ uint32_t smem_u32(const void* p) {
  return (uint32_t)__cvta_generic_to_shared(p);
}
__device__ __forceinline__ void mbar_init(uint32_t bar, uint32_t count) {
  asm volatile("mbarrier.init.shared::cta.b64 [%0], %1;" ::"r"(bar), "r"(count) : "memory");
}
__device__ __forceinline__ void mbar_expect_tx(uint32_t bar, uint32_t bytes) {
  asm volatile("mbarrier.arrive.expect_tx.shared::cta.b64 _, [%0], %1;" ::"r"(bar), "r"(bytes)
               : "memory");
}
__device__ __forceinline__ void mbar_arrive(uint32_t bar) {
  asm volatile("mbarrier.arrive.shared::cta.b64 _, [%0];" ::"r"(bar) : "memory");
}
__device__ __forceinline__ bool mbar_try_wait(uint32_t bar, uint32_t parity) {
  uint32_t ok;
  asm volatile(
      "{\n\t.reg .pred P1;\n\t"
      "mbarrier.try_wait.parity.shared::cta.b64 P1, [%1], %2;\n\t"
      "selp.b32 %0, 1, 0, P1;\n\t}"
      : "=r"(ok)
      : "r"(bar), "r"(parity)
      : "memory");
  return ok != 0;
}
__device__ __forceinline__ unsigned long long global_ns() {
  unsigned long long t;
  asm volatile("mov.u64 %0, %%globaltimer;" : "=l"(t));
  return t;
}
__device__ __forceinline__ void mbar_wait(uint32_t bar, uint32_t parity) {
  if (mbar_try_wait(bar, parity)) return;
  const unsigned long long t0 = global_ns();
  while (!mbar_try_wait(bar, parity))
    if (global_ns() - t0 > WAIT_TIMEOUT_NS) __trap();
}
__device__ __forceinline__ void mbar_spin(uint32_t bar, uint32_t parity) {
  while (!mbar_try_wait(bar, parity)) {
  }
}
__device__ __forceinline__ void tma_load_2d(uint32_t dst, const CUtensorMap* map, uint32_t bar,
                                            int c0, int c1) {
  asm volatile(
      "cp.async.bulk.tensor.2d.shared::cluster.global.mbarrier::complete_tx::bytes"
      " [%0], [%1, {%3, %4}], [%2];"
      ::"r"(dst), "l"(map), "r"(bar), "r"(c0), "r"(c1)
      : "memory");
}
__device__ __forceinline__ void tma_load_2d_mc(uint32_t dst, const CUtensorMap* map, uint32_t bar,
                                               int c0, int c1, uint16_t mask) {
  asm volatile(
      "cp.async.bulk.tensor.2d.shared::cluster.global.mbarrier::complete_tx::bytes"
      ".multicast::cluster [%0], [%1, {%3, %4}], [%2], %5;"
      ::"r"(dst), "l"(map), "r"(bar), "r"(c0), "r"(c1), "h"(mask)
      : "memory");
}
__device__ __forceinline__ void mbar_arrive_cluster(uint32_t bar, uint32_t cta) {
  asm volatile(
      "{\n\t.reg .b32 rb;\n\t"
      "mapa.shared::cluster.u32 rb, %0, %1;\n\t"
      "mbarrier.arrive.shared::cluster.b64 _, [rb];\n\t}"
      ::"r"(bar), "r"(cta)
      : "memory");
}
__device__ __forceinline__ void cluster_sync() {
  asm volatile("barrier.cluster.arrive.release;\n\tbarrier.cluster.wait.acquire;" ::: "memory");
}
__device__ __forceinline__ void tma_prefetch_desc(const CUtensorMap* map) {
  asm volatile("prefetch.tensormap [%0];" ::"l"(map) : "memory");
}

template <int MN, int RB>
__device__ __forceinline__ uint64_t gmma_desc(uint32_t saddr) {
  uint64_t d = (uint64_t)((saddr & 0x3FFFF) >> 4);
  if (MN) {
    d |= (uint64_t)(8192 >> 4) << 16;
    d |= (uint64_t)(1024 >> 4) << 32;
    d |= (uint64_t)1 << 62;
  } else {
    d |= (uint64_t)1 << 16;
    d |= (uint64_t)((8 * RB) >> 4) << 32;
    d |= (uint64_t)(RB == 128 ? 1 : 2) << 62;
  }
  return d;
}
__device__ __forceinline__ void wgmma_fence() {
  asm volatile("wgmma.fence.sync.aligned;" ::: "memory");
}
__device__ __forceinline__ void wgmma_commit() {
  asm volatile("wgmma.commit_group.sync.aligned;" ::: "memory");
}
template <int N>
__device__ __forceinline__ void wgmma_wait() {
  asm volatile("wgmma.wait_group.sync.aligned %0;" ::"n"(N) : "memory");
}
__device__ __forceinline__ void wgmma_tf32(float (&d)[64], uint64_t da, uint64_t db) {
  asm volatile(
      "{\n\t.reg .pred p;\n\tsetp.ne.b32 p, 1, 0;\n\t"
      "wgmma.mma_async.sync.aligned.m64n128k8.f32.tf32.tf32 {%0, %1, %2, %3, %4, %5, %6, %7, %8, %9, %10, %11, %12, %13, %14, %15, %16, %17, %18, %19, %20, %21, %22, %23, %24, %25, %26, %27, %28, %29, %30, %31, %32, %33, %34, %35, %36, %37, %38, %39, %40, %41, %42, %43, %44, %45, %46, %47, %48, %49, %50, %51, %52, %53, %54, %55, %56, %57, %58, %59, %60, %61, %62, %63}, %64, %65, p, 1, 1;\n\t}"
      : "+f"(d[0]), "+f"(d[1]), "+f"(d[2]), "+f"(d[3]), "+f"(d[4]), "+f"(d[5]), "+f"(d[6]), "+f"(d[7]), "+f"(d[8]), "+f"(d[9]), "+f"(d[10]), "+f"(d[11]), "+f"(d[12]), "+f"(d[13]), "+f"(d[14]), "+f"(d[15]), "+f"(d[16]), "+f"(d[17]), "+f"(d[18]), "+f"(d[19]), "+f"(d[20]), "+f"(d[21]), "+f"(d[22]), "+f"(d[23]), "+f"(d[24]), "+f"(d[25]), "+f"(d[26]), "+f"(d[27]), "+f"(d[28]), "+f"(d[29]), "+f"(d[30]), "+f"(d[31]), "+f"(d[32]), "+f"(d[33]), "+f"(d[34]), "+f"(d[35]), "+f"(d[36]), "+f"(d[37]), "+f"(d[38]), "+f"(d[39]), "+f"(d[40]), "+f"(d[41]), "+f"(d[42]), "+f"(d[43]), "+f"(d[44]), "+f"(d[45]), "+f"(d[46]), "+f"(d[47]), "+f"(d[48]), "+f"(d[49]), "+f"(d[50]), "+f"(d[51]), "+f"(d[52]), "+f"(d[53]), "+f"(d[54]), "+f"(d[55]), "+f"(d[56]), "+f"(d[57]), "+f"(d[58]), "+f"(d[59]), "+f"(d[60]), "+f"(d[61]), "+f"(d[62]), "+f"(d[63])
      : "l"(da), "l"(db));
}
template <int TA, int TB>
__device__ __forceinline__ void wgmma_f16(float (&d)[64], uint64_t da, uint64_t db) {
  asm volatile(
      "{\n\t.reg .pred p;\n\tsetp.ne.b32 p, 1, 0;\n\t"
      "wgmma.mma_async.sync.aligned.m64n128k16.f32.f16.f16 {%0, %1, %2, %3, %4, %5, %6, %7, %8, %9, %10, %11, %12, %13, %14, %15, %16, %17, %18, %19, %20, %21, %22, %23, %24, %25, %26, %27, %28, %29, %30, %31, %32, %33, %34, %35, %36, %37, %38, %39, %40, %41, %42, %43, %44, %45, %46, %47, %48, %49, %50, %51, %52, %53, %54, %55, %56, %57, %58, %59, %60, %61, %62, %63}, %64, %65, p, 1, 1, %66, %67;\n\t}"
      : "+f"(d[0]), "+f"(d[1]), "+f"(d[2]), "+f"(d[3]), "+f"(d[4]), "+f"(d[5]), "+f"(d[6]), "+f"(d[7]), "+f"(d[8]), "+f"(d[9]), "+f"(d[10]), "+f"(d[11]), "+f"(d[12]), "+f"(d[13]), "+f"(d[14]), "+f"(d[15]), "+f"(d[16]), "+f"(d[17]), "+f"(d[18]), "+f"(d[19]), "+f"(d[20]), "+f"(d[21]), "+f"(d[22]), "+f"(d[23]), "+f"(d[24]), "+f"(d[25]), "+f"(d[26]), "+f"(d[27]), "+f"(d[28]), "+f"(d[29]), "+f"(d[30]), "+f"(d[31]), "+f"(d[32]), "+f"(d[33]), "+f"(d[34]), "+f"(d[35]), "+f"(d[36]), "+f"(d[37]), "+f"(d[38]), "+f"(d[39]), "+f"(d[40]), "+f"(d[41]), "+f"(d[42]), "+f"(d[43]), "+f"(d[44]), "+f"(d[45]), "+f"(d[46]), "+f"(d[47]), "+f"(d[48]), "+f"(d[49]), "+f"(d[50]), "+f"(d[51]), "+f"(d[52]), "+f"(d[53]), "+f"(d[54]), "+f"(d[55]), "+f"(d[56]), "+f"(d[57]), "+f"(d[58]), "+f"(d[59]), "+f"(d[60]), "+f"(d[61]), "+f"(d[62]), "+f"(d[63])
      : "l"(da), "l"(db), "n"(TA), "n"(TB));
}

__device__ __forceinline__ void acc_ld16(uint32_t addr, uint32_t v[16]) {
#pragma unroll
  for (int i = 0; i < 4; ++i)
    asm volatile("ld.shared.v4.b32 {%0, %1, %2, %3}, [%4];"
                 : "=r"(v[4 * i]), "=r"(v[4 * i + 1]), "=r"(v[4 * i + 2]), "=r"(v[4 * i + 3])
                 : "r"(addr + 16u * i));
}

__device__ __forceinline__ float warp_transpose_sum16(float v[16], int lane) {
#pragma unroll
  for (int i = 0; i < 16; ++i) v[i] += __shfl_xor_sync(0xffffffffu, v[i], 16);
#pragma unroll
  for (int o = 8, cnt = 16; o >= 1; o >>= 1, cnt >>= 1) {
    const bool upper = (lane & o) != 0;
#pragma unroll
    for (int i = 0; i < cnt / 2; ++i) {
      const float keep = upper ? v[i + cnt / 2] : v[i];
      const float send = upper ? v[i] : v[i + cnt / 2];
      v[i] = keep + __shfl_xor_sync(0xffffffffu, send, o);
    }
  }
  return v[0];
}

__device__ __forceinline__ float pow2_plane_scale(float m) {
  int e = 0;
  if (m > 0.f) frexpf(m, &e);
  return ldexpf(1.f, 12 - e);
}
__device__ __forceinline__ float finite_absmax(float m, float x) {
  const float a = fabsf(x);
  return (a <= 3.0e38f) ? fmaxf(m, a) : m;
}
__device__ __forceinline__ void store_hilo(__half* p, int64_t lo, float x) {
  const __half h = __float2half_rn(x);
  p[0] = h;
  p[lo] = __float2half_rn(x - __half2float(h));
}
__device__ __forceinline__ void fold_amax(float* scale, float m, int lane) {
  m = warp_max(m);
  if (lane == 0 && m > 0.f) atomicMax(reinterpret_cast<unsigned int*>(scale) + 2, __float_as_uint(m));
}

template <int KIND, int RB, int MNA, int MNB, int ZLO = 0>
__device__ __forceinline__ void mma_kblock(float (&d)[2][64], uint32_t sa) {
  using C = Cfg<RB>;
#pragma unroll
  for (int k = 0; k < RB / 32; ++k) {
    const uint32_t bo = MNB ? (uint32_t)k * 2048u : (uint32_t)k * 32u;
    const uint64_t b_hi = gmma_desc<MNB, RB>(sa + 2 * C::A_TILE + bo);
    const uint64_t b_lo = gmma_desc<MNB, RB>(sa + 2 * C::A_TILE + C::B_TILE + bo);
#pragma unroll
    for (int mh = 0; mh < 2; ++mh) {
      const uint32_t ao = MNA ? (uint32_t)mh * 8192u + (uint32_t)k * 2048u
                              : (uint32_t)(mh * 64 * RB) + (uint32_t)k * 32u;
      const uint64_t a_hi = gmma_desc<MNA, RB>(sa + ao);
      const uint64_t a_lo = gmma_desc<MNA, RB>(sa + C::A_TILE + ao);
      if (KIND == 0) {
        wgmma_tf32(d[mh], a_lo, b_hi);
        wgmma_tf32(d[mh], a_hi, b_lo);
        wgmma_tf32(d[mh], a_hi, b_hi);
      } else {
        if (!(ZLO & 1)) wgmma_f16<MNA, MNB>(d[mh], a_lo, b_hi);
        if (!(ZLO & 2)) wgmma_f16<MNA, MNB>(d[mh], a_hi, b_lo);
        wgmma_f16<MNA, MNB>(d[mh], a_hi, b_hi);
      }
    }
  }
}

template <class W, class = void>
struct ClusterOf {
  static constexpr int value = 1;
};
template <class W>
struct ClusterOf<W, decltype((void)W::CLUSTER)> {
  static constexpr int value = W::CLUSTER;
};

template <class W, class = void>
struct ZloOf {
  static constexpr int value = 0;
};
template <class W>
struct ZloOf<W, decltype((void)W::ZLO)> {
  static constexpr int value = W::ZLO;
};

__device__ __forceinline__ void acc_tile_write(uint32_t acc_base, int tid, const float (&d)[2][64],
                                               bool add) {
  const int row = 16 * (tid >> 5) + ((tid & 31) >> 2);
  const int col = 2 * (tid & 3);
#pragma unroll
  for (int mh = 0; mh < 2; ++mh)
#pragma unroll
    for (int j = 0; j < 16; ++j) {
      const uint32_t a0 = acc_base + (uint32_t)(((64 * mh + row) * ACC_LD + 8 * j + col) * 4);
      float v0 = d[mh][4 * j], v1 = d[mh][4 * j + 1], v2 = d[mh][4 * j + 2], v3 = d[mh][4 * j + 3];
      if (add) {
        float p0, p1, p2, p3;
        asm volatile("ld.shared.v2.f32 {%0, %1}, [%2];" : "=f"(p0), "=f"(p1) : "r"(a0) : "memory");
        asm volatile("ld.shared.v2.f32 {%0, %1}, [%2];" : "=f"(p2), "=f"(p3)
                     : "r"(a0 + 8u * ACC_LD * 4u) : "memory");
        v0 += p0; v1 += p1; v2 += p2; v3 += p3;
      }
      asm volatile("st.shared.v2.f32 [%0], {%1, %2};" ::"r"(a0), "f"(v0), "f"(v1) : "memory");
      asm volatile("st.shared.v2.f32 [%0], {%1, %2};" ::"r"(a0 + 8u * ACC_LD * 4u), "f"(v2),
                   "f"(v3) : "memory");
    }
}

template <class W, class = void>
struct PromoteOf {
  static constexpr int value = 0;
};
template <class W>
struct PromoteOf<W, decltype((void)W::PROMOTE_KB)> {
  static constexpr int value = W::PROMOTE_KB;
};

template <class W>
__global__ void __launch_bounds__(NUM_THREADS, 1) tc_pipeline_kernel(const __grid_constant__ W w) {
  using C = Cfg<W::RB>;
  constexpr int CS = ClusterOf<W>::value;
  extern __shared__ uint8_t smem_raw[];
  const uint32_t smem_base = (smem_u32(smem_raw) + (C::ALIGN - 1)) & ~(uint32_t)(C::ALIGN - 1);
  const uint32_t acc_base = smem_base + C::STAGES * C::STAGE;
  const uint32_t bars = acc_base + ACC_BYTES;
  const uint32_t full_bar = bars;
  const uint32_t empty_bar = bars + 8 * C::STAGES;
  const uint32_t tfull_bar = bars + 16 * C::STAGES;
  const uint32_t tempty_bar = tfull_bar + 8;

  const int warp = __shfl_sync(0xffffffffu, (int)(threadIdx.x >> 5), 0);
  const int lane = threadIdx.x & 31;
  const int64_t n_units = w.units();

  if (threadIdx.x == 0) {
    for (int s = 0; s < C::STAGES; ++s) {
      mbar_init(full_bar + 8 * s, 1);
      mbar_init(empty_bar + 8 * s, CS);
    }
    mbar_init(tfull_bar, 128);
    mbar_init(tempty_bar, 32 * NUM_EPI_WARPS);
    asm volatile("fence.mbarrier_init.release.cluster;" ::: "memory");
  }
  if constexpr (CS > 1)
    cluster_sync();
  else
    __syncthreads();
  auto release = [&](int s) {
    if constexpr (CS > 1) {
#pragma unroll
      for (int r = 0; r < CS; ++r) mbar_arrive_cluster(empty_bar + 8 * s, (uint32_t)r);
    } else {
      mbar_arrive(empty_bar + 8 * s);
    }
  };

  if (warp < 4) {
    const int tid = threadIdx.x;
    float d[2][64];
    int stage = 0;
    uint32_t phase = 0, acc_phase = 0;
    const long long t_begin = prof_clock();
    long long t_full = 0, t_tempty = 0, t_store = 0, units = 0;
    for (int64_t u = blockIdx.x; u < n_units; u += gridDim.x) {
      int kb0, kb1;
      w.kb_range(u, kb0, kb1);
#pragma unroll
      for (int mh = 0; mh < 2; ++mh)
#pragma unroll
        for (int i = 0; i < 64; ++i) d[mh][i] = 0.f;
      int prev = -1;
      [[maybe_unused]] int since = 0;
      [[maybe_unused]] bool in_tile = false;
      if constexpr (PromoteOf<W>::value > 0) {
        const long long t1 = prof_clock();
        mbar_wait(tempty_bar, acc_phase ^ 1);
        t_tempty += prof_clock() - t1;
      }
      for (int kb = kb0; kb < kb1; ++kb) {
        const uint32_t sa = smem_base + stage * C::STAGE;
        const long long t0 = prof_clock();
        mbar_spin(full_bar + 8 * stage, phase);
        t_full += prof_clock() - t0;
        wgmma_fence();
        mma_kblock<W::KIND, W::RB, W::MNA, W::MNB, ZloOf<W>::value>(d, sa);
        wgmma_commit();
        wgmma_wait<1>();
        if (prev >= 0 && tid == 0) release(prev);
        prev = stage;
        if (++stage == C::STAGES) { stage = 0; phase ^= 1; }
        if constexpr (PromoteOf<W>::value > 0) {
          if (++since == PromoteOf<W>::value && kb + 1 < kb1) {
            wgmma_wait<0>();
            if (tid == 0) release(prev);
            prev = -1;
            acc_tile_write(acc_base, tid, d, in_tile);
            in_tile = true;
            since = 0;
#pragma unroll
            for (int mh = 0; mh < 2; ++mh)
#pragma unroll
              for (int i = 0; i < 64; ++i) d[mh][i] = 0.f;
          }
        }
      }
      wgmma_wait<0>();
      if (prev >= 0 && tid == 0) release(prev);
      const long long t1 = prof_clock();
      if constexpr (PromoteOf<W>::value == 0)
        mbar_wait(tempty_bar, acc_phase ^ 1);
      const long long t2 = prof_clock();
      t_tempty += t2 - t1;
      acc_tile_write(acc_base, tid, d, in_tile);
      mbar_arrive(tfull_bar);
      acc_phase ^= 1;
      t_store += prof_clock() - t2;
      ++units;
    }
    if (kPassProfile && tid == 0) {
      prof_add(PROF_MMA_TOTAL, prof_clock() - t_begin);
      prof_add(PROF_MMA_FULL, t_full);
      prof_add(PROF_MMA_TEMPTY, t_tempty);
      prof_add(PROF_MMA_STORE, t_store);
      prof_add(PROF_UNITS, units);
    }
  } else if (warp == PRODUCER_WARP) {
    if (lane == 0) {
      w.prefetch();
      int stage = 0;
      uint32_t phase = 0;
      long long t_empty = 0;
      for (int64_t u = blockIdx.x; u < n_units; u += gridDim.x) {
        int kb0, kb1;
        w.kb_range(u, kb0, kb1);
        for (int kb = kb0; kb < kb1; ++kb) {
          const long long t0 = prof_clock();
          mbar_wait(empty_bar + 8 * stage, phase ^ 1);
          t_empty += prof_clock() - t0;
          const uint32_t fb = full_bar + 8 * stage;
          mbar_expect_tx(fb, W::TX);
          w.load(u, kb, smem_base + stage * C::STAGE, fb);
          if (++stage == C::STAGES) { stage = 0; phase ^= 1; }
        }
      }
      if (kPassProfile) prof_add(PROF_PROD_EMPTY, t_empty);
    }
  } else {
    const int quarter = warp - EPI_WARP0;
    const uint32_t trow = acc_base + (uint32_t)((quarter * 32 + lane) * ACC_LD * 4);
    typename W::EpiState st;
    uint32_t acc_phase = 0;
    long long t_tfull = 0, t_unit = 0;
    for (int64_t u = blockIdx.x; u < n_units; u += gridDim.x) {
      const long long t0 = prof_clock();
      mbar_wait(tfull_bar, acc_phase);
      const long long t1 = prof_clock();
      w.epilogue(u, trow, quarter, lane, st);
      __syncwarp();
      mbar_arrive(tempty_bar);
      acc_phase ^= 1;
      t_tfull += t1 - t0;
      t_unit += prof_clock() - t1;
    }
    if (kPassProfile && quarter == 0 && lane == 0) {
      prof_add(PROF_EPI_TFULL, t_tfull);
      prof_add(PROF_EPI_UNIT, t_unit);
    }
    w.epi_finish(st, quarter, lane);
  }
  if constexpr (CS > 1) cluster_sync();
}

template <class W>
int tc_launch(const W& w, cudaStream_t st, const char* what) {
  constexpr int CS = ClusterOf<W>::value;
  static const cudaError_t attr = cudaFuncSetAttribute(
      tc_pipeline_kernel<W>, cudaFuncAttributeMaxDynamicSharedMemorySize, Cfg<W::RB>::SMEM);
  if (attr != cudaSuccess) {
    zsb_set_error("%s: cudaFuncSetAttribute: %s", what, cudaGetErrorString(attr));
    return ZSB_ERR_CUDA;
  }
  if constexpr (CS > 1) {
    const int64_t units = w.units();
    if (units < 1 || units % CS != 0) {
      zsb_set_error("%s: %lld units do not tile by clusters of %d", what, (long long)units, CS);
      return ZSB_ERR_INVALID;
    }
    cudaLaunchAttribute cl[1];
    cl[0].id = cudaLaunchAttributeClusterDimension;
    cl[0].val.clusterDim.x = CS;
    cl[0].val.clusterDim.y = 1;
    cl[0].val.clusterDim.z = 1;
    cudaLaunchConfig_t cfg = {};
    cfg.blockDim = dim3(NUM_THREADS);
    cfg.dynamicSmemBytes = Cfg<W::RB>::SMEM;
    cfg.stream = st;
    cfg.attrs = cl;
    cfg.numAttrs = 1;
    static int max_clusters = 0;
    if (max_clusters < 1) {
      cfg.gridDim = dim3(CS);
      const cudaError_t e =
          cudaOccupancyMaxActiveClusters(&max_clusters, tc_pipeline_kernel<W>, &cfg);
      if (e != cudaSuccess || max_clusters < 1) {
        zsb_set_error("%s: no cluster of %d CTAs fits (%s)", what, CS, cudaGetErrorString(e));
        max_clusters = 0;
        return ZSB_ERR_CUDA;
      }
    }
    int64_t grid = (int64_t)max_clusters * CS;
    if (grid > units) grid = units;
    cfg.gridDim = dim3((unsigned)grid);
    const cudaError_t e = cudaLaunchKernelEx(&cfg, tc_pipeline_kernel<W>, w);
    if (e != cudaSuccess) {
      zsb_set_error("%s: cudaLaunchKernelEx: %s", what, cudaGetErrorString(e));
      return ZSB_ERR_CUDA;
    }
    return zsb_check_launch(what);
  } else {
    int dev = 0, sms = ZSB_NUM_SMS;
    cudaGetDevice(&dev);
    cudaDeviceGetAttribute(&sms, cudaDevAttrMultiProcessorCount, dev);
    int64_t grid = w.units();
    if (grid > sms) grid = sms;
    if (grid < 1) grid = 1;
    tc_pipeline_kernel<W><<<(unsigned)grid, NUM_THREADS, Cfg<W::RB>::SMEM, st>>>(w);
    return zsb_check_launch(what);
  }
}

typedef CUresult (*EncodeTiledFn)(CUtensorMap*, CUtensorMapDataType, cuuint32_t, void*,
                                  const cuuint64_t*, const cuuint64_t*, const cuuint32_t*,
                                  const cuuint32_t*, CUtensorMapInterleave, CUtensorMapSwizzle,
                                  CUtensorMapL2promotion, CUtensorMapFloatOOBfill);

EncodeTiledFn get_encode_fn() {
  static EncodeTiledFn fn = nullptr;
  if (!fn) {
    void* p = nullptr;
    cudaDriverEntryPointQueryResult qres;
    if (cudaGetDriverEntryPoint("cuTensorMapEncodeTiled", &p, cudaEnableDefault, &qres) !=
            cudaSuccess || qres != cudaDriverEntryPointSuccess)
      return nullptr;
    fn = (EncodeTiledFn)p;
  }
  return fn;
}

int make_map(CUtensorMap* map, const void* base, uint64_t rows, uint64_t cols, uint32_t box_rows,
             int rb, int half_elems = 0) {
  EncodeTiledFn enc = get_encode_fn();
  if (!enc) {
    zsb_set_error("tc: cuTensorMapEncodeTiled unavailable");
    return ZSB_ERR_CUDA;
  }
  const int esz = half_elems ? 2 : 4;
  cuuint64_t dims[2] = {cols, rows};
  cuuint64_t strides[1] = {cols * esz};
  cuuint32_t box[2] = {(cuuint32_t)(rb / esz), box_rows};
  cuuint32_t estr[2] = {1, 1};
  CUresult r = enc(map, half_elems ? CU_TENSOR_MAP_DATA_TYPE_FLOAT16 : CU_TENSOR_MAP_DATA_TYPE_FLOAT32,
                   2, (void*)base, dims, strides, box, estr,
                   CU_TENSOR_MAP_INTERLEAVE_NONE,
                   rb == 128 ? CU_TENSOR_MAP_SWIZZLE_128B : CU_TENSOR_MAP_SWIZZLE_64B,
                   CU_TENSOR_MAP_L2_PROMOTION_L2_256B, CU_TENSOR_MAP_FLOAT_OOB_FILL_NONE);
  if (r != CUDA_SUCCESS) {
    zsb_set_error("tc: cuTensorMapEncodeTiled failed (%d)", (int)r);
    return ZSB_ERR_CUDA;
  }
  return ZSB_OK;
}

}
```

### zhusuan_b200/fused.py

```python
import math

import numpy as np
import torch
from torch.autograd.function import once_differentiable

from .distributions.base import Distribution
from .distributions.multivariate import MultivariateNormalCholesky
from .distributions.univariate import Normal

__all__ = ["GaussianLogJoint", "BNNRegressionLogJoint", "LNTMLogJoint", "PMFLogJoint", "linear",
           "class_linear", "noisy_bn_linear", "bn_linear", "linear_bernoulli_log_prob",
           "LinearBernoulli", "LinearOnehotCategorical", "LinearNormal", "RBFKernel",
           "gp_conditional", "conv2d", "conv2d_transpose", "bn_conv2d", "bn_conv2d_transpose",
           "sigmoid_conv2d_transpose", "conv2d_tc", "conv2d_transpose_tc"]


class GaussianLogJoint(object):

    def __init__(self, precision, mean=None, log_det_cov=None, name="x",
                 device="cuda", impl=None):
        P64 = np.asarray(precision.detach().cpu().numpy()
                         if isinstance(precision, torch.Tensor)
                         else precision, dtype=np.float64)
        D = P64.shape[0]
        if P64.shape != (D, D):
            raise ValueError("precision must be square")
        if D % 16 != 0:
            raise ValueError("the fused dense-Gaussian path needs D % 16 == 0")
        P64 = 0.5 * (P64 + P64.T)
        self.name = name
        self.D = D
        if log_det_cov is None:
            sign, ld = np.linalg.slogdet(P64)
            log_det_cov = -ld
        self.const = float(-0.5 * (D * math.log(2 * math.pi) + log_det_cov))
        P32 = P64.astype(np.float32)
        self.P = torch.as_tensor(P32, device=device).contiguous()
        d = {"kind": "dense_gaussian", "D": D, "P": self.P,
             "const": self.const, "impl": impl}
        self.mu = None
        if mean is not None:
            mu64 = np.asarray(mean, np.float64).reshape(D)
            self.mu = torch.as_tensor(mu64.astype(np.float32), device=device)
            d["mu"] = self.mu
            d["b"] = torch.as_tensor(
                (P32.astype(np.float64) @ mu64).astype(np.float32),
                device=device)
        hi = (P32.view(np.uint32) & np.uint32(0xFFFFE000)).view(np.float32)
        lo = (P32 - hi).astype(np.float32)
        d["P_hi"] = torch.as_tensor(hi, device=device).contiguous()
        d["P_lo"] = torch.as_tensor(lo, device=device).contiguous()
        pmax = float(np.abs(P32).max())
        sP = float(2.0 ** (12 - np.frexp(pmax)[1])) if pmax > 0 else 1.0
        x = P32.astype(np.float64) * sP
        h16 = x.astype(np.float16)
        l16 = (x - h16.astype(np.float64)).astype(np.float16)
        d["sP"] = sP
        d["P_inf"] = float(np.abs(P32.astype(np.float64)).sum(1).max())
        d["b_max"] = float(d["b"].abs().max()) if "b" in d else 0.0
        d["P_h16"] = torch.as_tensor(h16, device=device).contiguous()
        d["P_l16"] = torch.as_tensor(l16, device=device).contiguous()
        self._zsb_fused = d

    def __call__(self, observed):
        x = observed[self.name]
        if self.mu is not None:
            x = x - self.mu
        return -0.5 * ((x @ self.P) * x).sum(-1) + self.const


class BNNRegressionLogJoint(object):

    MAX_IN1, MAX_H = 16, 64

    def __init__(self, x, y, logstds, n_train, y_logstd=-0.95,
                 names=("w0", "w1")):
        from .distributions import Normal
        self._Normal = Normal
        self.x, self.y = x, y
        self.logstds = [l.contiguous() for l in logstds]
        self.n_train = float(n_train)
        if isinstance(y_logstd, torch.Tensor):
            if y_logstd.dim() != 0 or y_logstd.dtype != torch.float32 or \
                    not y_logstd.is_cuda:
                raise ValueError("y_logstd must be a float or a 0-d float32 CUDA tensor, "
                                 "got %s %s on %s" % (y_logstd.dtype, tuple(y_logstd.shape),
                                                      y_logstd.device))
            self.y_logstd = y_logstd
        else:
            self.y_logstd = float(y_logstd)
        self.names = tuple(names)
        self._prior_cache = {}
        self._ys_dev = None
        self._zsb_fused = {"kind": "bnn_regression", "obj": self}

    def fused_prior_logstd(self, k, shape):
        ls = self.logstds[k]
        s = list(ls.shape)
        while s and s[0] == 1:
            s.pop(0)
        shape = tuple(int(d) for d in shape)
        if len(s) > len(shape) or any(a != 1 and a != b for a, b in
                                      zip(s[::-1], shape[::-1])):
            return None
        if not s or tuple(s) == shape[len(shape) - len(s):]:
            return ls
        key = (k, shape, ls.data_ptr(), tuple(ls.shape), ls._version)
        e = self._prior_cache.get(k)
        if e is None or e[0] != key:
            e = (key, ls.reshape(s).expand(shape).contiguous())
            self._prior_cache[k] = e
        return e[1]

    def set_batch(self, observed):
        if "x" in observed:
            self.x = observed["x"]
        if "y" in observed:
            self.y = observed["y"]

    def _y_logstd_dev(self, device):
        if isinstance(self.y_logstd, torch.Tensor):
            return self.y_logstd
        e = self._ys_dev
        if e is None or e[0] != (self.y_logstd, device):
            e = ((self.y_logstd, device),
                 torch.tensor(self.y_logstd, dtype=torch.float32, device=device))
            self._ys_dev = e
        return e[1]

    def fused_inputs(self, observed):
        try:
            w0, w1 = (_unwrap(observed[n]) for n in self.names)
        except KeyError:
            return None
        x, y = _unwrap(observed.get("x", self.x)), _unwrap(observed.get("y", self.y))
        ts = (w0, w1, x, y)
        if not all(isinstance(t, torch.Tensor) and t.is_cuda for t in ts) or \
                w0.dtype != torch.float32 or w1.dtype != torch.float32:
            return None
        if w0.dim() != 3 or w1.dim() != 3:
            return None
        K, H, in1 = (int(d) for d in w0.shape)
        if tuple(w1.shape) != (K, 1, H + 1) or not (2 <= in1 <= self.MAX_IN1) or \
                not (1 <= H <= self.MAX_H) or K < 1:
            return None
        if x.dim() != 2 or int(x.shape[1]) + 1 != in1 or x.shape[0] < 1 or \
                y.numel() != x.shape[0]:
            return None
        dev = w0.device
        if w1.device != dev or x.device != dev or y.device != dev:
            return None
        if any(ls.requires_grad or ls.dtype != torch.float32 or ls.device != dev
               for ls in self.logstds):
            return None
        if isinstance(self.y_logstd, torch.Tensor) and self.y_logstd.device != dev:
            return None
        if self.fused_prior_logstd(0, w0.shape[1:]) is None or \
                self.fused_prior_logstd(1, w1.shape[1:]) is None:
            return None
        return w0, w1, x, y

    def _launch(self, w0, w1, x, y, ys, lp=False, g0=False, g1=False, gys=False,
                ym=False, ll=False):
        from ._lib import lib, ptr, stream
        K, H, in1 = (int(d) for d in w0.shape)
        B = int(x.shape[0])
        dev = w0.device
        w0, w1 = w0.detach().contiguous(), w1.detach().contiguous()
        x = x.detach().to(torch.float32).contiguous()
        y = y.detach().to(torch.float32).contiguous().view(-1)
        ys = ys.detach()
        ls0 = self.fused_prior_logstd(0, w0.shape[1:]).detach()
        ls1 = self.fused_prior_logstd(1, w1.shape[1:]).detach()
        e = lambda want, *s: torch.empty(s, dtype=torch.float32, device=dev) if want else None
        out = (e(lp, K), e(g0, K, H, in1), e(g1, K, 1, H + 1), e(gys, K), e(ym, K, B),
               e(ll, K, B))
        lib.call("zsb_bnn_logjoint_f32", ptr(w0), ptr(w1), ptr(x), ptr(y), B, in1 - 1, H,
                 ptr(ls0), ls0.numel(), ptr(ls1), ls1.numel(), ptr(ys), self.n_train,
                 *[ptr(o) for o in out], K, stream())
        return out

    def fused_log_joint(self, observed):
        got = self.fused_inputs(observed)
        if got is None:
            raise ValueError("BNNRegressionLogJoint.fused_log_joint: these inputs need the "
                             "generic path (see fused_inputs)")
        w0, w1, x, y = got
        ys = self._y_logstd_dev(w0.device)
        if not torch.is_grad_enabled():
            return self._launch(w0, w1, x, y, ys, lp=True)[0]
        return _BNNLogJoint.apply(w0.contiguous(), w1.contiguous(), ys, self, x, y)

    def predictive(self, observed):
        got = self.fused_inputs(observed)
        if got is None:
            raise ValueError("BNNRegressionLogJoint.predictive: shapes outside the fused "
                             "kernel's limits (see fused_inputs)")
        w0, w1, x, y = got
        _, _, _, _, ym, ll = self._launch(w0, w1, x, y, self._y_logstd_dev(w0.device),
                                          ym=True, ll=True)
        return ym, ll

    def hmc_provider(self, latent_names, observed, latents):
        if list(latent_names) != list(self.names):
            return None
        obs = dict(observed)
        obs.update(zip(self.names, latents))
        if self.fused_inputs(obs) is None:
            return None
        return _BNNProvider(self, observed)

    def __call__(self, observed):
        x = observed.get("x", self.x)
        y = observed.get("y", self.y)
        w0, w1 = observed[self.names[0]], observed[self.names[1]]
        C = w0.shape[0]
        h = x.unsqueeze(0).expand(C, -1, -1)
        lp = 0.0
        for w, ls in zip((w0, w1), self.logstds):
            ones = torch.ones(h.shape[:-1] + (1,), device=h.device)
            h = torch.cat([h, ones], -1)
            h = torch.einsum("imk,ijk->ijm", w, h) / math.sqrt(h.shape[2])
            if w is w0:
                h = torch.relu(h)
            lp = lp + self._Normal(torch.zeros_like(ls), logstd=ls,
                                   group_ndims=2).log_prob(w)
        y_mean = h.squeeze(2)
        if isinstance(self.y_logstd, torch.Tensor):
            y_ls = self.y_logstd.to(y_mean.dtype).expand_as(y_mean)
        else:
            y_ls = torch.full_like(y_mean, self.y_logstd)
        lpy = self._Normal(y_mean, logstd=y_ls).log_prob(y.unsqueeze(0))
        return lp + lpy.mean(1) * self.n_train


def _unwrap(v):
    return v if isinstance(v, torch.Tensor) else getattr(v, "tensor", v)


class _BNNLogJoint(torch.autograd.Function):

    @staticmethod
    def forward(ctx, w0, w1, ys, obj, x, y):
        need = ctx.needs_input_grad
        lp, g0, g1, gys, _, _ = obj._launch(w0, w1, x, y, ys, lp=True, g0=need[0], g1=need[1],
                                            gys=need[2])
        ctx.save_for_backward(g0, g1, gys)
        return lp

    @staticmethod
    @once_differentiable
    def backward(ctx, glp):
        g0, g1, gys = ctx.saved_tensors
        glp = glp.to(torch.float32)
        d0 = g0 * glp.view(-1, 1, 1) if g0 is not None else None
        d1 = g1 * glp.view(-1, 1, 1) if g1 is not None else None
        dys = (gys * glp).sum() if gys is not None else None
        return d0, d1, dys, None, None, None


class _BNNProvider(object):

    def __init__(self, obj, observed):
        self.obj, self.observed = obj, observed

    def _obs(self, var_list):
        obs = dict(self.observed)
        obs.update(zip(self.obj.names, var_list))
        return obs

    def logp(self, var_list):
        obs = self._obs(var_list)
        got = self.obj.fused_inputs(obs)
        if got is None:
            return self.obj(obs)
        w0, w1, x, y = got
        return self.obj._launch(w0, w1, x, y, self.obj._y_logstd_dev(w0.device), lp=True)[0]

    def grad(self, var_list):
        got = self.obj.fused_inputs(self._obs(var_list))
        if got is None:
            xs = [v.detach().requires_grad_(True) for v in var_list]
            with torch.enable_grad():
                gs = torch.autograd.grad(self.obj(self._obs(xs)).sum(), xs, allow_unused=True)
            return [g.contiguous() if g is not None else torch.zeros_like(x)
                    for g, x in zip(gs, xs)]
        w0, w1, x, y = got
        out = self.obj._launch(w0, w1, x, y, self.obj._y_logstd_dev(w0.device), g0=True,
                               g1=True)
        return [out[1], out[2]]


class LNTMLogJoint(object):

    def __init__(self, x, beta, eta_mean, eta_logstd, name="eta"):
        from ._lib import lib
        self.name = name
        dev = beta.device
        x = torch.as_tensor(x, device=dev)
        self.x = x.to(torch.float32)
        self.n_docs, self.n_vocab = int(x.shape[0]), int(x.shape[1])
        nz = (self.x != 0)
        per_doc = nz.sum(1)
        self.doc_ptr = torch.zeros(self.n_docs + 1, dtype=torch.int64, device=dev)
        self.doc_ptr[1:] = torch.cumsum(per_doc, 0)
        idx = nz.nonzero(as_tuple=False)
        self.word_idx = idx[:, 1].to(torch.int32).contiguous()
        self.word_cnt = self.x[idx[:, 0], idx[:, 1]].contiguous()
        self.nnz = int(idx.shape[0])
        order = torch.sort(idx[:, 1], stable=True)[1]
        self.csc_entry = order.to(torch.int32).contiguous()
        self.entry_doc = idx[order, 0].to(torch.int32).contiguous()
        self.csc_ptr = torch.zeros(self.n_vocab + 1, dtype=torch.int64, device=dev)
        self.csc_ptr[1:] = torch.cumsum(torch.bincount(idx[:, 1], minlength=self.n_vocab), 0)
        self.eta_mean = eta_mean.detach().to(torch.float32).contiguous()
        self.eta_logstd = eta_logstd.detach().to(torch.float32).contiguous()
        self.n_topics = int(beta.shape[0])
        if self.n_topics < 1:
            raise ValueError("LNTMLogJoint: n_topics must be at least 1")
        self.n_topics_padded = 16 * -(-self.n_topics // 16)
        self.fused = dev.type == "cuda" and self.n_topics <= 128
        self.set_docs(None)
        self.set_beta(beta)
        if self.fused:
            self._zsb_fused = {"kind": "provider", "obj": self}

    def set_beta(self, beta):
        from ._lib import lib, ptr, stream
        self.beta = beta.detach().to(torch.float32).contiguous()
        if not self.fused:
            return
        self.phi_t = torch.empty((self.n_vocab, self.n_topics_padded), dtype=torch.float32,
                                 device=self.beta.device)
        lib.call("zsb_lntm_phi_t_f32", ptr(self.beta), self.n_topics, self.n_vocab,
                 ptr(self.phi_t), stream())

    def set_docs(self, doc_ids):
        if doc_ids is None:
            self.doc_ids, self._doc_slot, self.n_batch = None, None, self.n_docs
            return
        if not isinstance(doc_ids, torch.Tensor) or doc_ids.dim() != 1 or \
                doc_ids.dtype != torch.int64 or doc_ids.device != self.doc_ptr.device:
            raise ValueError("doc_ids must be a 1-D int64 tensor on %s" % self.doc_ptr.device)
        self.doc_ids = doc_ids.contiguous()
        self.n_batch = int(doc_ids.shape[0])
        self._doc_slot = torch.full((self.n_docs,), -1, dtype=torch.int32,
                                    device=doc_ids.device).scatter_(
            0, self.doc_ids, torch.arange(self.n_batch, dtype=torch.int32,
                                          device=doc_ids.device))

    def _check_eta(self, eta):
        if eta.dim() != 3 or int(eta.shape[1]) != self.n_batch or \
                int(eta.shape[2]) != self.n_topics:
            raise ValueError("eta must be [chains, %d, %d]" % (self.n_batch, self.n_topics))
        return eta.detach().to(torch.float32).contiguous()

    def _launch(self, eta, want_lp, want_grad, temperature=None):
        from ._lib import lib, ptr, stream
        if not self.fused:
            raise ValueError("LNTMLogJoint: the fused kernels need 1 <= n_topics <= 128 and a "
                             "CUDA beta (got %d topics on %s); call the object for the dense "
                             "log-joint" % (self.n_topics, self.beta.device))
        eta = self._check_eta(eta)
        chains = int(eta.shape[0])
# ... 1986 lines not shown
```

### zhusuan_b200/hmc.py

```python
import ctypes

import torch

from . import dist as zdist
from . import random as zrandom
from ._lib import lib, ptr, stream
from .framework.bn import StochasticTensor
from .utils import merge_dicts

__all__ = ["HMCInfo", "HMC"]

_F32 = torch.float32
ST_T, ST_STEP, ST_TSTEP, ST_LEB, ST_HBAR, ST_MU, ST_EWT, ST_EPS, ST_ACC, \
    ST_FLAGS, ST_SLAST, ST_SCOND = range(12)
STREAM_MOMENTUM = 1


class HMCInfo(object):

    def __init__(self, samples, acceptance_rate, updated_step_size,
                 init_momentum, orig_hamiltonian, hamiltonian, orig_log_prob,
                 log_prob):
        self.samples = samples
        self.acceptance_rate = acceptance_rate
# ... 188 lines not shown
            orig_hamiltonian=self._h0.view(chain_shape),
            hamiltonian=self._h1.view(chain_shape),
            orig_log_prob=self._lp0.view(chain_shape),
            log_prob=self._lpsel.view(chain_shape))
        self._info = info
        return _SampleOp(self), info

    def _get_log_posterior(self, var_list):
        if self._provider is not None:
            return self._provider.logp(var_list)
        joint_obs = merge_dicts(dict(zip(self._latent_k, var_list)),
                                self._observed)
        return self._log_joint(joint_obs)

    def _get_gradient(self, var_list):
        if self._provider is not None:
            return self._provider.grad(var_list)
        xs = [v.detach().requires_grad_(True) for v in var_list]
        with torch.enable_grad():
            lp = self._get_log_posterior(xs)
            gs = torch.autograd.grad(lp.sum(), xs, allow_unused=True)
        return [g.contiguous() if g is not None else torch.zeros_like(x)
                for g, x in zip(gs, xs)]

    def _eps_ptr(self):
        return self._state.data_ptr() + 4 * ST_EPS

    def _check_flags(self, final=False):
        if self._flag_event is not None and (final or self._flag_event.query()):
            self._flag_event.synchronize()
            self._flag_event = None
            if int(self._flag_host[0]) & 1:
                self._state[ST_FLAGS:ST_FLAGS + 1].zero_()
                self._flag_host.zero_()
                raise FloatingPointError(
                    'HMC: old_log_prob has numeric errors! Try better '
                    'initialization.')
        elif final and self._state.is_cuda:
            torch.cuda.current_stream().synchronize()

    def _mass_stats_into_packed(self, s):
        off = 0
        for k, q in enumerate(self._q):
            r = self._row_len[k]
            lib.call("zsb_hmc_mass_stats_f32", ptr(q), ptr(self._ew_mean[k]), self._chains, r,
                     ptr(self._mass_part[k]), self._mass_stats.data_ptr() + 4 * off, s)
            off += 2 * r

    def _prefetch_ok(self):
        return (self._pk.mass_valid and self._q_versions is not None and
                self._q_versions == [q._version for q in self._q])

    def _queue_flag_check(self):
        if self._state.is_cuda:
            self._flag_host.copy_(
                self._state[ST_FLAGS:ST_FLAGS + 1].view(torch.int32),
                non_blocking=True)
            ev = torch.cuda.Event()
            ev.record()
            self._flag_event = ev

    def _seed_now(self):
        return self._seed if self._seed is not None else zrandom.get_seed()

    def _iterate(self, adapt_step_size, adapt_mass, noise, use_graph=None):
        if not self._built:
            raise RuntimeError("call HMC.sample() first")
        self._check_flags()
        adapt_step = _flag(self.adapt_step_size if adapt_step_size is None
                           else adapt_step_size)
        adapt_m = _flag(self.adapt_mass if adapt_mass is None else adapt_mass)
        self._t += 1
        t = self._t
        init = self._has_step and (t == 1 or t == self.mass_collect_iters)
        want_graph = self._use_graph if use_graph is None else bool(use_graph)
        if (want_graph and noise is None and not init and self._fused
                and self._state.is_cuda
                and (not (adapt_m and self._has_mass) or self._prefetch_ok())):
            return self._iterate_graph(adapt_step, adapt_m)
        return self._iterate_eager(adapt_step, adapt_m, noise, t, init)

    def _needs_acc_exchange(self, adapt_step):
        return bool(self._has_step and adapt_step)

    def _iterate_graph(self, adapt_step, adapt_m):
        key = (adapt_step, adapt_m, self._seed_now())
        g = self._graphs.get(key)
        if g is None:
            self._state[ST_T] = float(self._t - 1)
            self._state[ST_EWT] = float(self._ewmv_t)
            torch.cuda.synchronize()
            g = torch.cuda.CUDAGraph()
            self._dev_mode = True
            l0 = lib.launches
            try:
                with torch.cuda.graph(g):
                    self._iterate_eager(adapt_step, adapt_m, None, self._t,
                                        False)
            finally:
                self._dev_mode = False
            self._graphs[key] = g
            self._graph_launches[key] = lib.launches - l0
            lib.launches = l0
        if adapt_m and self._has_mass:
            self._ewmv_t += 1
        g.replay()
        lib.launches += self._graph_launches[key]
        if self._world > 1 and ((adapt_m and self._has_mass) or
                                self._needs_acc_exchange(adapt_step)):
            self._pk.n_collectives += 1
        self._pk.mass_valid = bool(adapt_m and self._has_mass)
        self._q_versions = [q._version for q in self._q]
        self._queue_flag_check()
        return None

    def _iterate_eager(self, adapt_step, adapt_m, noise, t, init):
        s = stream()
        dev = self._dev_mode
        it = 0xFFFFFFFF if dev else (t & 0xFFFFFFFF)
        seed = self._seed_now()
        noise_p = noise_u = None
        if noise is not None:
            noise_p = [noise["p"][k].contiguous() for k in self._latent_k]
            noise_u = noise["u"].contiguous().view(-1)

        lib.call("zsb_hmc_begin_f32", ptr(self._state),
                 -1 if dev else int(init), s)

        if self._has_mass:
            if adapt_m:
                if not dev and not self._prefetch_ok():
                    self._mass_stats_into_packed(s)
                    self._pk.reduce_mass()
                if not dev:
                    self._ewmv_t += 1
            use_ones = 1 if t < self.mass_collect_iters else 0
            if dev:
                use_ones = -(self.mass_collect_iters + 1)
            off = 0
            for k in range(len(self._q)):
                r = self._row_len[k]
                lib.call("zsb_hmc_mass_update_f32", ptr(self._ew_mean[k]),
                         ptr(self._ew_var[k]), ptr(self._mass[k]),
                         self._mass_stats.data_ptr() + 4 * off,
                         self._n_global, r, self.mass_decay,
                         float(self._ewmv_t), int(adapt_m), use_ones,
                         ptr(self._state), s)
                off += 2 * r
            if dev and adapt_m:
                lib.call("zsb_hmc_ewmv_bump_f32", ptr(self._state), s)

        kind = self._fused["kind"] if self._fused else "generic"
        if kind == "diag_normal":
            self._iterate_diag(noise_p, noise_u, seed, it, init, s)
        elif kind == "dense_gaussian":
            self._iterate_dense(noise_p, noise_u, seed, it, init, s)
        else:
            self._iterate_generic(noise_p, noise_u, seed, it, init, s)

        lib.call("zsb_hmc_acc_sum_f32", ptr(self._acc_part),
                 self._npart.value, self._chains, ptr(self._stats), s)
        prefetch = bool(self._has_mass and adapt_m)
        if prefetch:
            self._mass_stats_into_packed(s)
        exchange = prefetch or self._needs_acc_exchange(adapt_step)
        if dev:
            if self._world > 1 and exchange:
                zdist.all_reduce_sum(self._pk.buf if prefetch else self._pk.acc, self._group)
        else:
            if exchange:
                self._pk.reduce_all(prefetch)
            else:
                self._pk.mass_valid = False
            self._q_versions = [q._version for q in self._q]
        lib.call("zsb_hmc_tune_f32", ptr(self._state), ptr(self._stats),
                 int(self._has_step), int(adapt_step), 1.0 if init else 0.0,
                 self.gamma, self.t0, self.kappa, self.target_acceptance_rate,
                 -1.0 if dev else float(t), s)
        if not dev:
            self._queue_flag_check()
        return None

    def _search(self, probe, s):
        while True:
            self.n_search_iters += 1
            probe()
            lib.call("zsb_hmc_acc_sum_f32", ptr(self._acc_part),
                     self._npart.value, self._chains, ptr(self._stats), s)
            self._pk.reduce_acc()
            lib.call("zsb_hmc_search_update_f32", ptr(self._state),
                     ptr(self._stats), self.target_acceptance_rate, s)
            if float(self._state[ST_SCOND].item()) == 0.0:
                break

    def _momentum(self, noise_p, seed, it, s):
        for k, q in enumerate(self._q):
            lib.call("zsb_hmc_momentum_f32", ptr(self._p0[k]),
                     ptr(noise_p[k]) if noise_p else None, ptr(self._mass[k]),
                     self._row_len[k], self._chains, self._row_len[k], seed,
                     it, STREAM_MOMENTUM + 16 * k, self._row0, ptr(self._k0),
                     int(k > 0), ptr(self._state), s)

    def _lf_q(self, q, p, scale, s):
        for k in range(len(q)):
            lib.call("zsb_hmc_leapfrog_q_f32", ptr(q[k]), ptr(p[k]),
                     ptr(self._mass[k]), self._row_len[k], self._row_len[k],
                     self._eps_ptr(), scale, q[k].numel(), s)

    def _lf_p(self, p, g, scale, s):
        for k in range(len(p)):
            lib.call("zsb_hmc_leapfrog_p_f32", ptr(p[k]), ptr(g[k]),
                     self._eps_ptr(), scale, p[k].numel(), s)

    def _mh_generic(self, q_new, p_new, noise_u, seed, it, s, full):
        with torch.no_grad():
            lp0 = self._get_log_posterior(self._q).reshape(-1).contiguous()
            lp1 = self._get_log_posterior(q_new).reshape(-1).contiguous()
        for k in range(len(p_new)):
            lib.call("zsb_hmc_kinetic_f32", ptr(p_new[k]), ptr(self._mass[k]),
                     self._row_len[k], self._chains, self._row_len[k],
                     ptr(self._k1), int(k > 0), s)
        if full:
            self._lp0.copy_(lp0)
        lib.call("zsb_hmc_mh_f32", ptr(lp0), ptr(lp1), ptr(self._k0),
                 ptr(self._k1), ptr(noise_u) if noise_u is not None else None,
                 seed, it, self._row0, self._chains,
                 ptr(self._h0) if full else None,
                 ptr(self._h1) if full else None, ptr(self._acc),
                 ptr(self._accept) if full else None,
                 ptr(self._lpsel) if full else None, ptr(self._acc_part),
                 ctypes.byref(self._npart), ptr(self._state), s)

    def _iterate_generic(self, noise_p, noise_u, seed, it, init, s):
        self._momentum(noise_p, seed, it, s)
        if init:
            def probe():
                q = [x.clone() for x in self._q]
                p = [x.clone() for x in self._p0]
                self._lf_p(p, self._get_gradient(q), 0.5, s)
                self._lf_q(q, p, 1.0, s)
                self._lf_p(p, self._get_gradient(q), 0.5, s)
                self._mh_generic(q, p, noise_u, seed, it, s, full=False)
            self._search(probe, s)
        cq = [x.clone() for x in self._q]
        cp = [x.clone() for x in self._p0]
        L = self.n_leapfrogs
        for i in range(L + 1):
            if i > 0:
                self._lf_q(cq, cp, 1.0, s)
            g = self._get_gradient(cq)
            self._lf_p(cp, g, 1.0 if 0 < i < L else 0.5, s)
        self._mh_generic(cq, cp, noise_u, seed, it, s, full=True)
        for k, q in enumerate(self._q):
            lib.call("zsb_hmc_select_f32", ptr(q), ptr(cq[k]),
                     ptr(self._accept), self._chains, self._row_len[k], s)

    def _iterate_diag(self, noise_p, noise_u, seed, it, init, s):
        f = self._fused
        q = self._q[0]

        def launch(search):
            lib.call("zsb_hmc_diag_normal_step_f32", ptr(q),
                     ptr(noise_p[0]) if noise_p else None,
                     ptr(noise_u) if noise_u is not None else None,
                     ptr(f["mean"]), f["mean"].numel(), ptr(f["logstd"]),
                     f["logstd"].numel(), ptr(self._mass[0]),
                     self._row_len[0], ptr(self._state), self.n_leapfrogs,
                     self._chains, self._row_len[0], seed, it, self._row0,
                     int(search), None if search else ptr(self._p0[0]),
                     ptr(self._h0), ptr(self._h1), ptr(self._lp0),
                     ptr(self._lpsel), ptr(self._acc), ptr(self._accept),
                     ptr(self._acc_part), ctypes.byref(self._npart), s)
        if init:
            self._search(lambda: launch(True), s)
        launch(False)

    def _setup_dense(self, dev):
        f = self._fused
        impl = self._dense_impl
        if impl is None:
            impl = f.get("impl")
        if impl is not None and impl not in (0, 1, 2, 5):
            raise ValueError("dense_impl must be None, 0, 1, 2 or 5, got {!r}".format(impl))
        D = f["D"]
        if impl is None:
            impl = (5 if self.n_leapfrogs >= 1 else 2) if D % 64 == 0 else \
                (1 if D % 32 == 0 else 0)
        if int(impl) in (2, 5) and D % 64 != 0:
            raise ValueError("dense_impl=2/5 (fp16 split) needs D % 64 == 0")
        self._res = int(impl) == 5 and self.n_leapfrogs >= 1
        if int(impl) == 5:
            impl = 2
        self._impl = int(impl)
        nt = lib.load().zsb_hmc_dense_ntiles(D, min(self._impl, 1))
        z = lambda *s: torch.zeros(*s, dtype=_F32, device=dev)
        self._pw = torch.empty_like(self._q[0])
        self._lo = {}
        self._pass_k = 0
        self._lp0_part, self._lp1_part = z(nt * self._chains), \
            z(nt * self._chains)
        self._k_part = z(nt * self._chains)
        self._ntiles = nt
        if self._res:
            shape = (2,) + tuple(self._q[0].shape)
            self._planes = [torch.empty(shape, dtype=torch.float16, device=dev)
                            for _ in range(2)]
            self._spare = [torch.empty(shape, dtype=torch.float16, device=dev)
                           for _ in range(2)]
            self._scales = self._plane_scales(dev)
            return
        self._qa, self._qb = torch.empty_like(self._q[0]), \
            torch.empty_like(self._q[0])
        if self._impl == 1:
            for t in (self._q[0], self._qa, self._qb):
                self._lo[t.data_ptr()] = torch.empty_like(t)
        if self._impl == 2:
            for t in (self._q[0], self._qa, self._qb):
                self._lo[t.data_ptr()] = torch.empty(
                    (2,) + tuple(t.shape), dtype=torch.float16, device=dev)
            self._scales = self._plane_scales(dev)

    def _plane_scales(self, dev):
        f = self._fused
        sc = torch.zeros(8 + 4 * (max(self.n_leapfrogs, 1) + 2), dtype=_F32, device=dev)
        sc[3], sc[4], sc[5] = f["sP"], f["P_inf"], f["b_max"]
        return sc

    def _plane_scale_of_pass(self, i):
        return self._scales[8 + 4 * i:]

    def _dense_pass(self, q_cur, q_next, p_in, p_out, scale, lp_part, k_part,
                    s):
        f = self._fused
        if self._impl == 2:
            lib.call("zsb_hmc_dense_leapfrog_h16_pass_f32", ptr(q_cur),
                     ptr(self._lo[q_cur.data_ptr()]), ptr(q_next),
                     ptr(self._lo[q_next.data_ptr()])
                     if q_next is not None else None, ptr(p_in), ptr(p_out),
                     ptr(f["P_h16"]), ptr(f["P_l16"]), ptr(self._scales),
                     self._pass_k, ptr(f.get("b")), ptr(f.get("mu")),
                     ptr(self._mass[0]), ptr(self._state), scale, ptr(lp_part),
                     ptr(k_part), self._chains, f["D"], s)
            self._pass_k += 1
            return
        tc = self._impl == 1
        lo_cur = self._lo[q_cur.data_ptr()] if tc else None
        lo_next = self._lo[q_next.data_ptr()] if tc and q_next is not None \
            else None
        lib.call("zsb_hmc_dense_leapfrog_f32", ptr(q_cur), ptr(lo_cur),
                 ptr(q_next), ptr(lo_next), ptr(p_in), ptr(p_out),
                 ptr(f["P_hi"] if tc else f["P"]),
                 ptr(f["P_lo"]) if tc else None,
                 ptr(f.get("b")), ptr(f.get("mu")), ptr(self._mass[0]),
                 ptr(self._state), scale, ptr(lp_part), ptr(k_part),
                 self._chains, f["D"], self._impl, s)

    def _dense_finish_mh(self, noise_u, seed, it, s, full):
        f = self._fused
        lib.call("zsb_hmc_dense_finish_f32", ptr(self._lp0_part), None,
                 self._ntiles, self._chains, f["const"], ptr(self._lp0), None,
                 s)
        lib.call("zsb_hmc_dense_finish_f32", ptr(self._lp1_part),
                 ptr(self._k_part), self._ntiles, self._chains, f["const"],
                 ptr(self._lp1), ptr(self._k1), s)
        lib.call("zsb_hmc_mh_f32", ptr(self._lp0), ptr(self._lp1),
                 ptr(self._k0), ptr(self._k1),
                 ptr(noise_u) if noise_u is not None else None, seed, it,
                 self._row0, self._chains,
                 ptr(self._h0) if full else None,
                 ptr(self._h1) if full else None, ptr(self._acc),
                 ptr(self._accept) if full else None,
                 ptr(self._lpsel) if full else None, ptr(self._acc_part),
                 ctypes.byref(self._npart), ptr(self._state), s)

    def _resident_trajectory(self, L, s):
        f = self._fused
        lib.call("zsb_hmc_dense_resident_h16_f32", ptr(self._planes[0]),
                 ptr(self._planes[1]), ptr(self._spare[0]), ptr(self._spare[1]),
                 ptr(self._p0[0]), ptr(self._pw),
                 ptr(f["P_h16"]), ptr(f["P_l16"]), ptr(self._scales), ptr(f.get("b")),
                 ptr(f.get("mu")), ptr(self._mass[0]), ptr(self._state),
                 ptr(self._lp0_part), ptr(self._lp1_part), ptr(self._k_part),
                 self._chains, f["D"], L, s)
        return self._planes[L & 1], self._spare[L & 1]

    def _iterate_dense_resident(self, noise_u, seed, it, init, s):
        q0 = self._q[0]

        def prepare():
            lib.call("zsb_hmc_dense_traj_prepare_f32", ptr(q0), ptr(self._p0[0]),
                     ptr(self._mass[0]), ptr(self._planes[0]), ptr(self._scales),
                     self._chains, self._row_len[0], s)
        if init:
            def probe():
                prepare()
                self._resident_trajectory(1, s)
                self._dense_finish_mh(noise_u, seed, it, s, full=False)
            self._search(probe, s)
        prepare()
        prop, spare = self._profiled(lambda: self._resident_trajectory(self.n_leapfrogs, s))
        self._dense_finish_mh(noise_u, seed, it, s, full=True)
        lib.call("zsb_hmc_dense_select_traj_planes_f32", ptr(q0), ptr(prop), ptr(spare),
                 ptr(self._plane_scale_of_pass(self.n_leapfrogs)), ptr(self._accept),
                 self._chains, self._row_len[0], s)

    def _iterate_dense(self, noise_p, noise_u, seed, it, init, s):
        q0 = self._q[0]
        self._momentum(noise_p, seed, it, s)
        if self._res:
            return self._iterate_dense_resident(noise_u, seed, it, init, s)
        if self._impl == 1:
            lib.call("zsb_hmc_dense_split_lo_f32", ptr(q0),
                     ptr(self._lo[q0.data_ptr()]), q0.numel(), s)

        def prepare():
            if self._impl == 2:
                lib.call("zsb_hmc_dense_traj_prepare_f32", ptr(q0), ptr(self._p0[0]),
                         ptr(self._mass[0]), ptr(self._lo[q0.data_ptr()]),
                         ptr(self._scales), self._chains, self._row_len[0], s)
            self._pass_k = 0
        if init:
            def probe():
                prepare()
                self._dense_pass(q0, self._qa, self._p0[0], self._pw, 0.5,
                                 self._lp0_part, None, s)
                self._dense_pass(self._qa, None, self._pw, self._pw, 0.5,
                                 self._lp1_part, self._k_part, s)
                self._dense_finish_mh(noise_u, seed, it, s, full=False)
            self._search(probe, s)
        L = self.n_leapfrogs
        prepare()

        def passes():
            cur, nxt = q0, self._qa
            p_in = self._p0[0]
            for i in range(L + 1):
                last = i == L
                self._dense_pass(
                    cur, None if last else nxt, p_in, self._pw,
                    1.0 if 0 < i < L else 0.5,
                    self._lp0_part if i == 0 else
                    (self._lp1_part if last else None),
                    self._k_part if last else None, s)
                p_in = self._pw
                if not last:
                    cur, nxt = nxt, (self._qb if nxt is self._qa else self._qa)
            return cur
        cur = self._profiled(passes)
        if L == 0:
            self._lp1_part.copy_(self._lp0_part)
        self._dense_finish_mh(noise_u, seed, it, s, full=True)
        lib.call("zsb_hmc_select_f32", ptr(q0), ptr(cur), ptr(self._accept),
                 self._chains, self._row_len[0], s)

    def _profiled(self, launch):
        prof = None if self._dev_mode else getattr(self, "_profile_events", None)
        if prof is None:
            return launch()
        e0, e1 = torch.cuda.Event(True), torch.cuda.Event(True)
        e0.record()
        out = launch()
        e1.record()
        prof.append((e0, e1))
        return out

    def state_dict(self):
        st = self._state.clone()
        st[ST_FLAGS] = 0
        d = {"t": self._t, "ewmv_t": self._ewmv_t, "state": st}
        if self._has_mass:
            d["ewmv_mean"] = [m.clone() for m in self._ew_mean]
            d["ewmv_var"] = [v.clone() for v in self._ew_var]
        return d

    def load_state_dict(self, d):
        self._t, self._ewmv_t = int(d["t"]), int(d["ewmv_t"])
        self._state.copy_(d["state"])
        self._state[ST_FLAGS] = 0
        self._pk.mass_valid = False
        self._state[ST_T] = float(self._t)
        self._state[ST_EWT] = float(self._ewmv_t)
        if self._has_mass:
            for m, s in zip(self._ew_mean, d["ewmv_mean"]):
                m.copy_(s)
            for v, s in zip(self._ew_var, d["ewmv_var"]):
                v.copy_(s)


def _suffix_ok(param_shape, data_shape):
    shape = list(param_shape)
    while shape and shape[0] == 1:
        shape.pop(0)
    n = len(shape)
    return n == 0 or list(data_shape[len(data_shape) - n:]) == shape


def _detect_diag_normal(meta_bn, observed, latent):
    from .distributions import Normal
    if len(latent) != 1 or meta_bn.log_joint is not None:
        return None
    name, q = next(iter(latent.items()))
    if not isinstance(q, torch.Tensor) or not q.is_cuda:
        return None
    try:
        bn = meta_bn.observe(**merge_dicts(latent, observed))
    except Exception:
        return None
    stoch = [n for n in bn.nodes.values() if isinstance(n, StochasticTensor)]
    if len(stoch) != 1 or stoch[0].name != name:
        return None
    d = stoch[0].dist
    if type(d) is not Normal or d.use_path_derivative:
        return None
    g = d.group_ndims
    if g < 1 or g >= q.dim() + 1:
        return None
    data_shape = tuple(q.shape[q.dim() - g:])
    if q.dim() - g < 1:
        return None
    row_len = 1
    for s in data_shape:
        row_len *= int(s)
    if row_len > 1024:
        return None
    if not (_suffix_ok(d.mean.shape, data_shape)
            and _suffix_ok(d.logstd.shape, data_shape)):
        return None
    return {"kind": "diag_normal",
            "mean": d.mean.detach().to(_F32).contiguous().reshape(-1),
            "logstd": d.logstd.detach().to(_F32).contiguous().reshape(-1)}
```

Measured before the change: 76.93 million.

## Interleave hi/lo fp16 planes so one TMA load fetches both per k-block

Stores the precision matrix and the resident position planes with hi and lo fp16 halves interleaved in 32-element chunks along each row. Each pipeline stage then needs one TMA load per operand instead of two, with a wider 128-byte row box, and the stage count is raised to five. The producer state moves into the barrier region of dynamic shared memory, and the alignment slack is dropped in favour of a runtime trap if the base is misaligned. This is meant to cut TMA issue count and descriptor overhead, in exchange for stricter D%64 requirements and more complex epilogue addressing.

Measured after the change: 78.90 million (median of 6 runs). +2.6%, better.

```diff
diff --git a/include/zsb200.h b/include/zsb200.h
--- a/include/zsb200.h
+++ b/include/zsb200.h
@@ -250,9 +250,12 @@
                                         const float* mu, const float* mass, const float* state,
                                         float p_scale, float* lp_part, float* k_part,
                                         int64_t chains, int64_t D, void* stream);
+int zsb_hmc_dense_resident_prepare_f32(const float* q, const float* p, const float* mass,
+                                       void* planes, float* scales, int64_t chains, int64_t D,
+                                       void* stream);
 int zsb_hmc_dense_resident_h16_f32(void* planes0, void* planes1, void* spare0, void* spare1,
-                                   const float* p0, float* pw, const void* P_h16,
-                                   const void* P_l16, float* scales, const float* bvec,
+                                   const float* p0, float* pw, const void* P_planes,
+                                   float* scales, const float* bvec,
                                    const float* mu, const float* mass, const float* state,
                                    float* lp0_part, float* lp1_part, float* k_part,
                                    int64_t chains, int64_t D, int n_leapfrogs, void* stream);
diff --git a/zhusuan_b200/_lib.py b/zhusuan_b200/_lib.py
--- a/zhusuan_b200/_lib.py
+++ b/zhusuan_b200/_lib.py
@@ -74,7 +74,8 @@
         self.load().zsb_last_error(buf, 512)
         return buf.value.decode("utf-8", "replace")
 
-    _KERNELS = {"zsb_hmc_mass_stats_f32": 2, "zsb_hmc_dense_traj_prepare_f32": 3, "zsb_hmc_dense_resident_h16_f32": 1, "zsb_sgmcmc_sghmc_f32": 2,
+    _KERNELS = {"zsb_hmc_mass_stats_f32": 2, "zsb_hmc_dense_traj_prepare_f32": 3, "zsb_hmc_dense_resident_prepare_f32": 3,
+                "zsb_hmc_dense_resident_h16_f32": 1, "zsb_sgmcmc_sghmc_f32": 2,
                 "zsb_sgmcmc_mean_sq_f32": 2, "zsb_sgmcmc_sgnht_scalar_f32": 2,
                 "zsb_split16_pad_f32": 3, "zsb_linear_tc_f32": 2, "zsb_planar_flow_bwd_f32": 2,
                 "zsb_iaf_bwd_f32": 2, "zsb_lntm_mstep_grad_f32": 2,
diff --git a/zhusuan_b200/csrc/hmc_dense.cu b/zhusuan_b200/csrc/hmc_dense.cu
--- a/zhusuan_b200/csrc/hmc_dense.cu
+++ b/zhusuan_b200/csrc/hmc_dense.cu
@@ -169,10 +169,10 @@
                                   float* lp_part, float* k_part, int64_t chains, int D,
                                   cudaStream_t st);
 int zsb_dense_h16_prepare_launch(const float* q, const float* p, const float* mass, void* planes,
-                                 float* scales, int64_t chains, int64_t D, cudaStream_t st);
+                                 float* scales, int64_t chains, int64_t D, bool interleaved,
+                                 cudaStream_t st);
 int zsb_dense_res_h16_launch(void* planes0, void* planes1, void* spare0, void* spare1,
-                             const float* p0, float* pw, const void* P_h16, const void* P_l16,
-                             float* scales, const float* bvec, const float* mu, const float* mass,
+                             const float* p0, float* pw, const void* P_planes, float* scales, const float* bvec, const float* mu, const float* mass,
                              const float* state, float* lp0_part, float* lp1_part, float* k_part,
                              int64_t chains, int D, int L, cudaStream_t st);
 int zsb_dense_select_planes_launch(float* q, const void* planes, const void* spare,
@@ -220,7 +220,7 @@
                                    float* scales, int64_t chains, int64_t D, void* stream) {
   ZSB_REQUIRE(q && p && mass && planes && scales && chains > 0 && D > 0,
               "zsb_hmc_dense_traj_prepare_f32: bad args");
-  return zsb_dense_h16_prepare_launch(q, p, mass, planes, scales, chains, D,
+  return zsb_dense_h16_prepare_launch(q, p, mass, planes, scales, chains, D, false,
                                       (cudaStream_t)stream);
 }
 int zsb_hmc_dense_leapfrog_h16_pass_f32(const float* q_cur, const void* q_cur_planes,
@@ -240,24 +240,32 @@
                                        (cudaStream_t)stream);
 }
 
+int zsb_hmc_dense_resident_prepare_f32(const float* q, const float* p, const float* mass,
+                                       void* planes, float* scales, int64_t chains, int64_t D,
+                                       void* stream) {
+  ZSB_REQUIRE(q && p && mass && planes && scales && chains > 0 && D > 0 && D % 64 == 0,
+              "zsb_hmc_dense_resident_prepare_f32: bad args");
+  return zsb_dense_h16_prepare_launch(q, p, mass, planes, scales, chains, D, true,
+                                      (cudaStream_t)stream);
+}
 int zsb_hmc_dense_resident_h16_f32(void* planes0, void* planes1, void* spare0, void* spare1,
-                                   const float* p0, float* pw, const void* P_h16,
-                                   const void* P_l16, float* scales, const float* bvec,
+                                   const float* p0, float* pw, const void* P_planes,
+                                   float* scales, const float* bvec,
                                    const float* mu, const float* mass, const float* state,
                                    float* lp0_part, float* lp1_part, float* k_part,
                                    int64_t chains, int64_t D, int n_leapfrogs, void* stream) {
-  ZSB_REQUIRE(planes0 && planes1 && spare0 && spare1 && p0 && pw && P_h16 && P_l16 && scales &&
+  ZSB_REQUIRE(planes0 && planes1 && spare0 && spare1 && p0 && pw && P_planes && scales &&
                   mass && state && lp0_part && lp1_part && k_part,
               "zsb_hmc_dense_resident_h16_f32: null arg");
   ZSB_REQUIRE(p0 != pw, "zsb_hmc_dense_resident_h16_f32: aliased buffers");
-  return zsb_dense_res_h16_launch(planes0, planes1, spare0, spare1, p0, pw, P_h16, P_l16, scales,
+  return zsb_dense_res_h16_launch(planes0, planes1, spare0, spare1, p0, pw, P_planes, scales,
                                   bvec, mu, mass, state, lp0_part, lp1_part, k_part, chains, (int)D,
                                   n_leapfrogs, (cudaStream_t)stream);
 }
 int zsb_hmc_dense_select_traj_planes_f32(float* q, const void* planes, const void* spare,
                                          const float* record, const int32_t* accept,
                                          int64_t chains, int64_t D, void* stream) {
-  ZSB_REQUIRE(q && planes && spare && record && accept && chains > 0 && D > 0 && D % 2 == 0,
+  ZSB_REQUIRE(q && planes && spare && record && accept && chains > 0 && D > 0 && D % 32 == 0,
               "zsb_hmc_dense_select_traj_planes_f32: bad args");
   return zsb_dense_select_planes_launch(q, planes, spare, record, accept, chains, D,
                                         (cudaStream_t)stream);
diff --git a/zhusuan_b200/csrc/hmc_dense_epilogue.cuh b/zhusuan_b200/csrc/hmc_dense_epilogue.cuh
--- a/zhusuan_b200/csrc/hmc_dense_epilogue.cuh
+++ b/zhusuan_b200/csrc/hmc_dense_epilogue.cuh
@@ -6,6 +6,9 @@
 constexpr int kScaleHdr = 8, kScaleRec = 4;
 constexpr float kPlaneKeep = 65280.f;
 constexpr float kHalfOverflow = 65520.f;
+
+constexpr int kIlvLo = 32;
+__host__ __device__ __forceinline__ int64_t ilv_hi(int64_t i) { return 2 * i - (i & 31); }
 
 __device__ __forceinline__ const float* scale_rec(const float* scales, int pass) {
   return scales + kScaleHdr + kScaleRec * pass;
diff --git a/zhusuan_b200/csrc/hmc_dense_res.cu b/zhusuan_b200/csrc/hmc_dense_res.cu
--- a/zhusuan_b200/csrc/hmc_dense_res.cu
+++ b/zhusuan_b200/csrc/hmc_dense_res.cu
@@ -3,10 +3,9 @@
 namespace {
 
 struct ResEpi {
-  const __half* __restrict__ hi_cur; const __half* __restrict__ lo_cur;
-  __half* __restrict__ hi_nxt; __half* __restrict__ lo_nxt;
-  const __half* __restrict__ hi_cur_s; const __half* __restrict__ lo_cur_s;
-  __half* __restrict__ hi_nxt_s; __half* __restrict__ lo_nxt_s;
+  const __half* __restrict__ cur;
+  __half* __restrict__ nxt;
+  const __half* __restrict__ cur_s; __half* __restrict__ nxt_s;
   const float* __restrict__ p_in; float* __restrict__ p_out;
   float* __restrict__ lp_part; float* __restrict__ k_part;
   int64_t chains; int D;
@@ -27,14 +26,19 @@
   const int64_t off_t = c0 * (int64_t)D + n;
   const float* __restrict__ pin0 = a.p_in + off_t;
   float* __restrict__ po0 = a.p_out + off_t;
+  const int64_t off_pl = ilv_hi(off_t);
+  auto at = [pin0](auto* base, const float* pe) {
+    return reinterpret_cast<decltype(base)>(reinterpret_cast<uintptr_t>(base) +
+                                            (reinterpret_cast<uintptr_t>(pe) -
+                                             reinterpret_cast<uintptr_t>(pin0)));
+  };
   const unsigned short* __restrict__ hc0 =
-      reinterpret_cast<const unsigned short*>(a.hi_cur) + off_t;
-  const unsigned short* __restrict__ lc0 =
-      reinterpret_cast<const unsigned short*>(a.lo_cur) + off_t;
-  __half* __restrict__ hn0 = NEXT ? a.hi_nxt + off_t : nullptr;
-  __half* __restrict__ ln0 = NEXT ? a.lo_nxt + off_t : nullptr;
-  __half* __restrict__ hs0 = SPARE ? a.hi_nxt_s + off_t : nullptr;
-  __half* __restrict__ ls0 = SPARE ? a.lo_nxt_s + off_t : nullptr;
+      reinterpret_cast<const unsigned short*>(a.cur) + off_pl;
+  const unsigned short* __restrict__ lc0 = hc0 + kIlvLo;
+  __half* __restrict__ hn0 = NEXT ? a.nxt + off_pl : nullptr;
+  __half* __restrict__ ln0 = NEXT ? hn0 + kIlvLo : nullptr;
+  __half* __restrict__ hs0 = SPARE ? a.nxt_s + off_pl : nullptr;
+  __half* __restrict__ ls0 = SPARE ? hs0 + kIlvLo : nullptr;
 
   auto element = [&](float acc, float p, uint32_t hl, float& pn, float& lpv, float& kv,
                      float& Qn) {
@@ -53,8 +57,8 @@
 #pragma unroll
       for (int j = 0; j < 16; ++j) {
         pe[j] = __ldcg(pin0 + cb + (uint32_t)j * D);
-        const uint32_t h = __ldcg(hc0 + cb + (uint32_t)j * D);
-        const uint32_t l = __ldcg(lc0 + cb + (uint32_t)j * D);
+        const uint32_t h = __ldcg(at(hc0, pin0 + cb + (uint32_t)j * D));
+        const uint32_t l = __ldcg(at(lc0, pin0 + cb + (uint32_t)j * D));
         he[j] = h | (l << 16);
       }
     };
@@ -78,20 +82,20 @@
           const __half2 h2 = __floats2half2_rn(Qn[0], Qn[1]);
           const float2 hf = __half22float2(h2);
           const __half2 l2 = __floats2half2_rn(Qn[0] - hf.x, Qn[1] - hf.y);
-          hn0[cb + (uint32_t)j * D] = __low2half(h2);
-          hn0[cb + (uint32_t)(j + 1) * D] = __high2half(h2);
-          ln0[cb + (uint32_t)j * D] = __low2half(l2);
-          ln0[cb + (uint32_t)(j + 1) * D] = __high2half(l2);
+          *at(hn0, pin0 + cb + (uint32_t)j * D) = __low2half(h2);
+          *at(hn0, pin0 + cb + (uint32_t)(j + 1) * D) = __high2half(h2);
+          *at(ln0, pin0 + cb + (uint32_t)j * D) = __low2half(l2);
+          *at(ln0, pin0 + cb + (uint32_t)(j + 1) * D) = __high2half(l2);
         }
         if (SPARE) {
           const float x0 = Qn[0] * a.rescale, x1 = Qn[1] * a.rescale;
           const __half2 h2 = __floats2half2_rn(x0, x1);
           const float2 hf = __half22float2(h2);
           const __half2 l2 = __floats2half2_rn(x0 - hf.x, x1 - hf.y);
-          hs0[cb + (uint32_t)j * D] = __low2half(h2);
-          hs0[cb + (uint32_t)(j + 1) * D] = __high2half(h2);
-          ls0[cb + (uint32_t)j * D] = __low2half(l2);
-          ls0[cb + (uint32_t)(j + 1) * D] = __high2half(l2);
+          *at(hs0, pin0 + cb + (uint32_t)j * D) = __low2half(h2);
+          *at(hs0, pin0 + cb + (uint32_t)(j + 1) * D) = __high2half(h2);
+          *at(ls0, pin0 + cb + (uint32_t)j * D) = __low2half(l2);
+          *at(ls0, pin0 + cb + (uint32_t)(j + 1) * D) = __high2half(l2);
         }
       }
       if (MODE >= 1) {
@@ -135,8 +139,8 @@
           uint32_t hl = 0u;
           if (ok) {
             p = __ldcg(pin0 + cb + (uint32_t)j * D);
-            hl = (uint32_t)__ldcg(hc0 + cb + (uint32_t)j * D) |
-                 ((uint32_t)__ldcg(lc0 + cb + (uint32_t)j * D) << 16);
+            hl = (uint32_t)__ldcg(at(hc0, pin0 + cb + (uint32_t)j * D)) |
+                 ((uint32_t)__ldcg(at(lc0, pin0 + cb + (uint32_t)j * D)) << 16);
           }
           float pn, lp1 = 0.f, k1 = 0.f, Qn = 0.f;
           element(__uint_as_float(v[j]), p, hl, pn, lp1, k1, Qn);
@@ -148,14 +152,14 @@
           if (ok) {
             po0[cb + (uint32_t)j * D] = pn;
             if (NEXT) {
-              hn0[cb + (uint32_t)j * D] = hh;
-              ln0[cb + (uint32_t)j * D] = ll;
+              *at(hn0, pin0 + cb + (uint32_t)j * D) = hh;
+              *at(ln0, pin0 + cb + (uint32_t)j * D) = ll;
             }
             if (SPARE) {
               const float x = Qn * a.rescale;
               const __half hs = __float2half_rn(x);
-              hs0[cb + (uint32_t)j * D] = hs;
-              ls0[cb + (uint32_t)j * D] = __float2half_rn(x - __half2float(hs));
+              *at(hs0, pin0 + cb + (uint32_t)j * D) = hs;
+              *at(ls0, pin0 + cb + (uint32_t)j * D) = __float2half_rn(x - __half2float(hs));
             }
           }
         }
@@ -176,18 +180,22 @@
 struct ProducerState {
   int spare_in, n0, c0;
 };
+extern __shared__ uint8_t res_dyn_smem[];
+template <class C>
 __device__ __forceinline__ ProducerState& producer_state() {
-  __shared__ ProducerState ps;
-  return ps;
+  constexpr int at = 112;
+  static_assert(C::SLACK == 0 && 16 * C::STAGES + 16 <= at && at + sizeof(ProducerState) <= 128,
+                "no room for the producer's state in the barrier block");
+  return *reinterpret_cast<ProducerState*>(res_dyn_smem + C::STAGES * C::STAGE + ACC_BYTES + at);
 }
 
 template <int MODE, int NEXT, int DC, int CX, int CY>
 struct ResW {
-  static constexpr int KIND = 1, RB = 64, MNA = 0, MNB = 0;
+  static constexpr int KIND = 1, RB = 128, MNA = 0, MNB = 0, ILV = 1;
   static constexpr int CLUSTER = CX * CY;
-  static constexpr int KE = RB / 2;
-  static constexpr uint32_t TX = Cfg<RB>::STAGE;
-  CUtensorMap m_phi, m_plo, m_qhi, m_qlo, m_shi, m_slo;
+  static constexpr int KE = RB / 4;
+  static constexpr uint32_t TX = Cfg<RB, ILV>::STAGE;
+  CUtensorMap m_p, m_q, m_s;
   ResEpi ea;
   const float* bvec; const float* mu; const float* mass; const float* state;
   float* scales;
@@ -211,14 +219,12 @@
     kb1 = D() / KE;
   }
   __device__ __forceinline__ void prefetch() const {
-    tma_prefetch_desc(&m_phi); tma_prefetch_desc(&m_plo);
-    tma_prefetch_desc(&m_qhi); tma_prefetch_desc(&m_qlo);
-    tma_prefetch_desc(&m_shi); tma_prefetch_desc(&m_slo);
-    producer_state().spare_in = plane_spare_in(scales, pass);
+    tma_prefetch_desc(&m_p); tma_prefetch_desc(&m_q); tma_prefetch_desc(&m_s);
+    producer_state<Cfg<RB, ILV>>().spare_in = plane_spare_in(scales, pass);
   }
   __device__ __forceinline__ void load(int64_t u, int kb, uint32_t sa, uint32_t fb) const {
-    using C = Cfg<RB>;
-    ProducerState& ps = producer_state();
+    using C = Cfg<RB, ILV>;
+    ProducerState& ps = producer_state<C>();
     if (kb == 0) {
       int nb;
       int64_t cb;
@@ -227,31 +233,24 @@
       ps.c0 = (int)cb * BN;
     }
     const int n0 = ps.n0, c0 = ps.c0;
-    const bool s = ps.spare_in != 0;
-    const CUtensorMap* qh = s ? &m_shi : &m_qhi;
-    const CUtensorMap* ql = s ? &m_slo : &m_qlo;
+    const CUtensorMap* q = ps.spare_in != 0 ? &m_s : &m_q;
+    const int k = 2 * KE * kb;
     const int r = (int)(u % CLUSTER), rx = r % CX, ry = r / CX;
     if constexpr (CY == 1) {
-      tma_load_2d(sa, &m_phi, fb, kb * KE, n0);
-      tma_load_2d(sa + C::A_TILE, &m_plo, fb, kb * KE, n0);
+      tma_load_2d(sa, &m_p, fb, k, n0);
     } else {
       constexpr int rows = BM / CY;
       uint16_t mask = 0;
 #pragma unroll
       for (int y = 0; y < CY; ++y) mask |= (uint16_t)(1u << (y * CX + rx));
-      const uint32_t o = (uint32_t)(ry * rows * RB);
-      tma_load_2d_mc(sa + o, &m_phi, fb, kb * KE, n0 + ry * rows, mask);
-      tma_load_2d_mc(sa + C::A_TILE + o, &m_plo, fb, kb * KE, n0 + ry * rows, mask);
+      tma_load_2d_mc(sa + (uint32_t)(ry * rows * RB), &m_p, fb, k, n0 + ry * rows, mask);
     }
     if constexpr (CX == 1) {
-      tma_load_2d(sa + 2 * C::A_TILE, qh, fb, kb * KE, c0);
-      tma_load_2d(sa + 2 * C::A_TILE + C::B_TILE, ql, fb, kb * KE, c0);
+      tma_load_2d(sa + C::A_TILE, q, fb, k, c0);
     } else {
       constexpr int rows = BN / CX;
       const uint16_t mask = (uint16_t)(((1u << CX) - 1u) << (ry * CX));
-      const uint32_t o = (uint32_t)(rx * rows * RB);
-      tma_load_2d_mc(sa + 2 * C::A_TILE + o, qh, fb, kb * KE, c0 + rx * rows, mask);
-      tma_load_2d_mc(sa + 2 * C::A_TILE + C::B_TILE + o, ql, fb, kb * KE, c0 + rx * rows, mask);
+      tma_load_2d_mc(sa + C::A_TILE + (uint32_t)(rx * rows * RB), q, fb, k, c0 + rx * rows, mask);
     }
   }
   __device__ __forceinline__ float sq_alt(float eps, float sq) const {
@@ -276,10 +275,7 @@
     const float mu_n = (n_ok && mu) ? mu[n] : 0.f;
     const int64_t part_row = (int64_t)(nb * 4 + quarter) * ea.chains;
     ResEpi a = ea;
-    if (spare_in) {
-      a.hi_cur = ea.hi_cur_s;
-      a.lo_cur = ea.lo_cur_s;
-    }
+    if (spare_in) a.cur = ea.cur_s;
     a.sq = sq;
     a.inv_sq = fdiv(1.f, sq);
     a.acc_scale = 1.f / (scales[3] * sq);
@@ -303,36 +299,34 @@
 constexpr int RES_CX = 2, RES_CY = 1;
 
 template <int DC, int CX, int CY>
-int res_pass(const CUtensorMap& phi, const CUtensorMap& plo, const CUtensorMap& qhi,
-             const CUtensorMap& qlo, const CUtensorMap& shi, const CUtensorMap& slo,
+int res_pass(const CUtensorMap& mp, const CUtensorMap& mq, const CUtensorMap& ms,
              const ResEpi& ea, const float* bvec, const float* mu, const float* mass,
              const float* state, float* scales, int pass, float p_scale, int n_blk, int D,
              int mode, cudaStream_t st) {
   if (mode == 1) {
-    const ResW<1, 1, DC, CX, CY> w{phi, plo, qhi, qlo, shi, slo, ea, bvec, mu, mass, state,
-                                   scales, p_scale, n_blk, D, pass};
+    const ResW<1, 1, DC, CX, CY> w{mp, mq, ms, ea, bvec, mu, mass, state, scales, p_scale, n_blk,
+                                   D, pass};
     return tc_launch(w, st, "hmc_dense_resident");
   }
   if (mode == 0) {
-    const ResW<0, 1, DC, CX, CY> w{phi, plo, qhi, qlo, shi, slo, ea, bvec, mu, mass, state,
-                                   scales, p_scale, n_blk, D, pass};
+    const ResW<0, 1, DC, CX, CY> w{mp, mq, ms, ea, bvec, mu, mass, state, scales, p_scale, n_blk,
+                                   D, pass};
     return tc_launch(w, st, "hmc_dense_resident");
   }
-  const ResW<2, 0, DC, CX, CY> w{phi, plo, qhi, qlo, shi, slo, ea, bvec, mu, mass, state, scales,
-                                 p_scale, n_blk, D, pass};
+  const ResW<2, 0, DC, CX, CY> w{mp, mq, ms, ea, bvec, mu, mass, state, scales, p_scale, n_blk, D,
+                                 pass};
   return tc_launch(w, st, "hmc_dense_resident");
 }
 
 template <int DC>
-int res_pass(bool cluster, const CUtensorMap& phi, const CUtensorMap& plo, const CUtensorMap& qhi,
-             const CUtensorMap& qlo, const CUtensorMap& shi, const CUtensorMap& slo,
+int res_pass(bool cluster, const CUtensorMap& mp, const CUtensorMap& mq, const CUtensorMap& ms,
              const ResEpi& ea, const float* bvec, const float* mu, const float* mass,
              const float* state, float* scales, int pass, float p_scale, int n_blk, int D,
              int mode, cudaStream_t st) {
-  return cluster ? res_pass<DC, RES_CX, RES_CY>(phi, plo, qhi, qlo, shi, slo, ea, bvec, mu, mass,
-                                                state, scales, pass, p_scale, n_blk, D, mode, st)
-                 : res_pass<DC, 1, 1>(phi, plo, qhi, qlo, shi, slo, ea, bvec, mu, mass, state,
-                                      scales, pass, p_scale, n_blk, D, mode, st);
+  return cluster ? res_pass<DC, RES_CX, RES_CY>(mp, mq, ms, ea, bvec, mu, mass, state, scales,
+                                                pass, p_scale, n_blk, D, mode, st)
+                 : res_pass<DC, 1, 1>(mp, mq, ms, ea, bvec, mu, mass, state, scales, pass,
+                                      p_scale, n_blk, D, mode, st);
 }
 
 __global__ void __launch_bounds__(256) select_planes_kernel(float* __restrict__ q,
@@ -349,15 +343,18 @@
   const int64_t wstride = (int64_t)gridDim.x * 8;
   for (int64_t c = (int64_t)blockIdx.x * 8 + (threadIdx.x >> 5); c < chains; c += wstride) {
     if (!accept[c]) continue;
-    const uint4* __restrict__ hi = reinterpret_cast<const uint4*>(planes + c * D);
-    const uint4* __restrict__ lo = reinterpret_cast<const uint4*>(planes + (chains + c) * D);
+    const __half* __restrict__ row = planes + ilv_hi(c * D);
     float4* __restrict__ qr = reinterpret_cast<float4*>(q + c * D);
     for (int i0 = lane; i0 < n8; i0 += 128) {
       uint4 h[4], l[4];
 #pragma unroll
       for (int u = 0; u < 4; ++u) {
         const int i = i0 + 32 * u;
-        if (i < n8) { h[u] = __ldcs(hi + i); l[u] = __ldcs(lo + i); }
+        if (i < n8) {
+          const __half* hp = row + ilv_hi(8 * i);
+          h[u] = __ldcs(reinterpret_cast<const uint4*>(hp));
+          l[u] = __ldcs(reinterpret_cast<const uint4*>(hp + kIlvLo));
+        }
       }
 #pragma unroll
       for (int u = 0; u < 4; ++u) {
@@ -385,7 +382,7 @@
 
 int zsb_dense_res_h16_launch(void* planes0, void* planes1, void* spare0, void* spare1,
                              const float* p0, float* pw,
-                             const void* P_h16, const void* P_l16, float* scales,
+                             const void* P_planes, float* scales,
                              const float* bvec, const float* mu, const float* mass,
                              const float* state, float* lp0_part, float* lp1_part, float* k_part,
                              int64_t chains, int D, int L, cudaStream_t st) {
@@ -401,36 +398,29 @@
   const int64_t c_blk = (chains + BN - 1) / BN;
   const bool cluster = n_blk % RES_CX == 0 && c_blk % RES_CY == 0;
   const uint32_t p_box = cluster ? BM / RES_CY : BM, q_box = cluster ? BN / RES_CX : BN;
-  CUtensorMap phi, plo, qhi[2], qlo[2], shi[2], slo[2];
+  CUtensorMap mp, mq[2], ms[2];
   int rc;
   constexpr int RB = ResW<0, 1, 0, 1, 1>::RB;
-  if ((rc = make_map(&phi, P_h16, (uint64_t)D, (uint64_t)D, p_box, RB, 1))) return rc;
-  if ((rc = make_map(&plo, P_l16, (uint64_t)D, (uint64_t)D, p_box, RB, 1))) return rc;
+  if ((rc = make_map(&mp, P_planes, (uint64_t)D, 2 * (uint64_t)D, p_box, RB, 1))) return rc;
   __half* pl[2] = {reinterpret_cast<__half*>(planes0), reinterpret_cast<__half*>(planes1)};
   __half* sp[2] = {reinterpret_cast<__half*>(spare0), reinterpret_cast<__half*>(spare1)};
-  const int64_t plane = chains * (int64_t)D;
   for (int b = 0; b < 2; ++b) {
-    if ((rc = make_map(&qhi[b], pl[b], (uint64_t)chains, (uint64_t)D, q_box, RB, 1))) return rc;
-    if ((rc = make_map(&qlo[b], pl[b] + plane, (uint64_t)chains, (uint64_t)D, q_box, RB, 1)))
-      return rc;
-    if ((rc = make_map(&shi[b], sp[b], (uint64_t)chains, (uint64_t)D, q_box, RB, 1))) return rc;
-    if ((rc = make_map(&slo[b], sp[b] + plane, (uint64_t)chains, (uint64_t)D, q_box, RB, 1)))
-      return rc;
+    if ((rc = make_map(&mq[b], pl[b], (uint64_t)chains, 2 * (uint64_t)D, q_box, RB, 1))) return rc;
+    if ((rc = make_map(&ms[b], sp[b], (uint64_t)chains, 2 * (uint64_t)D, q_box, RB, 1))) return rc;
   }
   for (int i = 0; i <= L; ++i) {
     const bool last = i == L;
     const int buf = i & 1;
-    const ResEpi ea{pl[buf], pl[buf] + plane, pl[buf ^ 1], pl[buf ^ 1] + plane,
-                    sp[buf], sp[buf] + plane, sp[buf ^ 1], sp[buf ^ 1] + plane,
+    const ResEpi ea{pl[buf], pl[buf ^ 1], sp[buf], sp[buf ^ 1],
                     i == 0 ? p0 : pw, pw, i == 0 ? lp0_part : lp1_part, k_part, chains, D,
                     1.f, 1.f, 1.f, 1.f};
     const int mode = last ? 2 : (i == 0 ? 1 : 0);
     const float p_scale = (i > 0 && !last) ? 1.f : 0.5f;
     rc = (D == 1024)
-             ? res_pass<1024>(cluster, phi, plo, qhi[buf], qlo[buf], shi[buf], slo[buf], ea, bvec,
-                              mu, mass, state, scales, i, p_scale, n_blk, D, mode, st)
-             : res_pass<0>(cluster, phi, plo, qhi[buf], qlo[buf], shi[buf], slo[buf], ea, bvec, mu,
-                           mass, state, scales, i, p_scale, n_blk, D, mode, st);
+             ? res_pass<1024>(cluster, mp, mq[buf], ms[buf], ea, bvec, mu, mass, state, scales, i,
+                              p_scale, n_blk, D, mode, st)
+             : res_pass<0>(cluster, mp, mq[buf], ms[buf], ea, bvec, mu, mass, state, scales, i,
+                           p_scale, n_blk, D, mode, st);
     if (rc != ZSB_OK) return rc;
   }
   return ZSB_OK;
diff --git a/zhusuan_b200/csrc/hmc_dense_tc.cu b/zhusuan_b200/csrc/hmc_dense_tc.cu
--- a/zhusuan_b200/csrc/hmc_dense_tc.cu
+++ b/zhusuan_b200/csrc/hmc_dense_tc.cu
@@ -125,6 +125,7 @@
   scales[7] = w;
   u[6] = 0u;
 }
+template <int ILV>
 __global__ void __launch_bounds__(256) split16_kernel(const float* __restrict__ q,
                                                       __half* __restrict__ planes, int64_t n,
                                                       const float* __restrict__ scales) {
@@ -133,8 +134,9 @@
        i += (int64_t)gridDim.x * blockDim.x) {
     const float x = q[i] * sq;
     const __half h = __float2half_rn(x);
-    planes[i] = h;
-    planes[n + i] = __float2half_rn(x - __half2float(h));
+    const int64_t o = ILV ? ilv_hi(i) : i;
+    planes[o] = h;
+    planes[o + (ILV ? kIlvLo : n)] = __float2half_rn(x - __half2float(h));
   }
 }
 
@@ -237,13 +239,19 @@
 }
 
 int zsb_dense_h16_prepare_launch(const float* q, const float* p, const float* mass, void* planes,
-                                 float* scales, int64_t chains, int64_t D, cudaStream_t st) {
+                                 float* scales, int64_t chains, int64_t D, bool interleaved,
+                                 cudaStream_t st) {
   const int64_t n = chains * D;
   int64_t blocks = zsb_ceil_div(n, 256 * 8);
   if (blocks > ZSB_NUM_SMS * 16) blocks = ZSB_NUM_SMS * 16;
   if (blocks < 1) blocks = 1;
   absmax_kernel<<<(unsigned)blocks, 256, 0, st>>>(q, p, mass, n, D, scales);
   scale_kernel<<<1, 32, 0, st>>>(scales, mass, D);
-  split16_kernel<<<(unsigned)blocks, 256, 0, st>>>(q, reinterpret_cast<__half*>(planes), n, scales);
+  if (interleaved)
+    split16_kernel<1><<<(unsigned)blocks, 256, 0, st>>>(q, reinterpret_cast<__half*>(planes), n,
+                                                        scales);
+  else
+    split16_kernel<0><<<(unsigned)blocks, 256, 0, st>>>(q, reinterpret_cast<__half*>(planes), n,
+                                                        scales);
   return zsb_check_launch("hmc_dense_h16_prepare");
 }
diff --git a/zhusuan_b200/csrc/tc_common.cuh b/zhusuan_b200/csrc/tc_common.cuh
--- a/zhusuan_b200/csrc/tc_common.cuh
+++ b/zhusuan_b200/csrc/tc_common.cuh
@@ -21,6 +21,7 @@
   PROF_MMA_TEMPTY,
   PROF_MMA_STORE,
   PROF_PROD_EMPTY,
+  PROF_PROD_LOAD,
   PROF_EPI_TFULL,
   PROF_EPI_UNIT,
   PROF_UNITS,
@@ -44,14 +45,15 @@
 #endif
 }
 
-template <int RB>
+template <int RB, int ILV = 0>
 struct Cfg {
   static constexpr int A_TILE = BM * RB;
   static constexpr int B_TILE = BN * RB;
-  static constexpr int STAGE = 2 * A_TILE + 2 * B_TILE;
-  static constexpr int STAGES = RB == 128 ? 2 : 5;
+  static constexpr int STAGE = ILV ? A_TILE + B_TILE : 2 * A_TILE + 2 * B_TILE;
+  static constexpr int STAGES = ILV ? 5 : 2;
   static constexpr int ALIGN = RB == 128 ? 1024 : 512;
-  static constexpr int SMEM = STAGES * STAGE + ACC_BYTES + 128 + ALIGN;
+  static constexpr int SLACK = ILV ? 0 : ALIGN;
+  static constexpr int SMEM = STAGES * STAGE + ACC_BYTES + 128 + SLACK;
   static_assert(SMEM <= 227 * 1024, "operand ring exceeds shared memory");
 };
 
@@ -208,20 +210,23 @@
   if (lane == 0 && m > 0.f) atomicMax(reinterpret_cast<unsigned int*>(scale) + 2, __float_as_uint(m));
 }
 
-template <int KIND, int RB, int MNA, int MNB, int ZLO = 0>
+template <int KIND, int RB, int MNA, int MNB, int ZLO = 0, int ILV = 0>
 __device__ __forceinline__ void mma_kblock(float (&d)[2][64], uint32_t sa) {
-  using C = Cfg<RB>;
-#pragma unroll
-  for (int k = 0; k < RB / 32; ++k) {
+  using C = Cfg<RB, ILV>;
+  static_assert(!ILV || (MNA == 0 && MNB == 0 && ZLO == 0), "interleaved rows are K-major");
+  constexpr uint32_t B0 = ILV ? C::A_TILE : 2 * C::A_TILE;
+  constexpr uint32_t A_LO = ILV ? RB / 2 : C::A_TILE, B_LO = ILV ? RB / 2 : C::B_TILE;
+#pragma unroll
+  for (int k = 0; k < (ILV ? RB / 64 : RB / 32); ++k) {
     const uint32_t bo = MNB ? (uint32_t)k * 2048u : (uint32_t)k * 32u;
-    const uint64_t b_hi = gmma_desc<MNB, RB>(sa + 2 * C::A_TILE + bo);
-    const uint64_t b_lo = gmma_desc<MNB, RB>(sa + 2 * C::A_TILE + C::B_TILE + bo);
+    const uint64_t b_hi = gmma_desc<MNB, RB>(sa + B0 + bo);
+    const uint64_t b_lo = gmma_desc<MNB, RB>(sa + B0 + B_LO + bo);
 #pragma unroll
     for (int mh = 0; mh < 2; ++mh) {
       const uint32_t ao = MNA ? (uint32_t)mh * 8192u + (uint32_t)k * 2048u
                               : (uint32_t)(mh * 64 * RB) + (uint32_t)k * 32u;
       const uint64_t a_hi = gmma_desc<MNA, RB>(sa + ao);
-      const uint64_t a_lo = gmma_desc<MNA, RB>(sa + C::A_TILE + ao);
+      const uint64_t a_lo = gmma_desc<MNA, RB>(sa + A_LO + ao);
       if (KIND == 0) {
         wgmma_tf32(d[mh], a_lo, b_hi);
         wgmma_tf32(d[mh], a_hi, b_lo);
@@ -252,6 +257,17 @@
 struct ZloOf<W, decltype((void)W::ZLO)> {
   static constexpr int value = W::ZLO;
 };
+
+template <class W, class = void>
+struct IlvOf {
+  static constexpr int value = 0;
+};
+template <class W>
+struct IlvOf<W, decltype((void)W::ILV)> {
+  static constexpr int value = W::ILV;
+};
+template <class W>
+using CfgOf = Cfg<W::RB, IlvOf<W>::value>;
 
 __device__ __forceinline__ void acc_tile_write(uint32_t acc_base, int tid, const float (&d)[2][64],
                                                bool add) {
@@ -287,10 +303,11 @@
 
 template <class W>
 __global__ void __launch_bounds__(NUM_THREADS, 1) tc_pipeline_kernel(const __grid_constant__ W w) {
-  using C = Cfg<W::RB>;
+  using C = CfgOf<W>;
   constexpr int CS = ClusterOf<W>::value;
   extern __shared__ uint8_t smem_raw[];
-  const uint32_t smem_base = (smem_u32(smem_raw) + (C::ALIGN - 1)) & ~(uint32_t)(C::ALIGN - 1);
+  constexpr uint32_t RA = C::SLACK ? C::ALIGN : 1;
+  const uint32_t smem_base = (smem_u32(smem_raw) + (RA - 1)) & ~(RA - 1);
   const uint32_t acc_base = smem_base + C::STAGES * C::STAGE;
   const uint32_t bars = acc_base + ACC_BYTES;
   const uint32_t full_bar = bars;
@@ -303,6 +320,8 @@
   const int64_t n_units = w.units();
 
   if (threadIdx.x == 0) {
+    if constexpr (C::SLACK == 0)
+      if (smem_base & (C::ALIGN - 1)) __trap();
     for (int s = 0; s < C::STAGES; ++s) {
       mbar_init(full_bar + 8 * s, 1);
       mbar_init(empty_bar + 8 * s, CS);
@@ -352,7 +371,7 @@
         mbar_spin(full_bar + 8 * stage, phase);
         t_full += prof_clock() - t0;
         wgmma_fence();
-        mma_kblock<W::KIND, W::RB, W::MNA, W::MNB, ZloOf<W>::value>(d, sa);
+        mma_kblock<W::KIND, W::RB, W::MNA, W::MNB, ZloOf<W>::value, IlvOf<W>::value>(d, sa);
         wgmma_commit();
         wgmma_wait<1>();
         if (prev >= 0 && tid == 0) release(prev);
@@ -398,21 +417,26 @@
       w.prefetch();
       int stage = 0;
       uint32_t phase = 0;
-      long long t_empty = 0;
+      long long t_empty = 0, t_load = 0;
       for (int64_t u = blockIdx.x; u < n_units; u += gridDim.x) {
         int kb0, kb1;
         w.kb_range(u, kb0, kb1);
         for (int kb = kb0; kb < kb1; ++kb) {
           const long long t0 = prof_clock();
           mbar_wait(empty_bar + 8 * stage, phase ^ 1);
-          t_empty += prof_clock() - t0;
+          const long long t1 = prof_clock();
+          t_empty += t1 - t0;
           const uint32_t fb = full_bar + 8 * stage;
           mbar_expect_tx(fb, W::TX);
           w.load(u, kb, smem_base + stage * C::STAGE, fb);
+          t_load += prof_clock() - t1;
           if (++stage == C::STAGES) { stage = 0; phase ^= 1; }
         }
       }
-      if (kPassProfile) prof_add(PROF_PROD_EMPTY, t_empty);
+      if (kPassProfile) {
+        prof_add(PROF_PROD_EMPTY, t_empty);
+        prof_add(PROF_PROD_LOAD, t_load);
+      }
     }
   } else {
     const int quarter = warp - EPI_WARP0;
@@ -444,7 +468,7 @@
 int tc_launch(const W& w, cudaStream_t st, const char* what) {
   constexpr int CS = ClusterOf<W>::value;
   static const cudaError_t attr = cudaFuncSetAttribute(
-      tc_pipeline_kernel<W>, cudaFuncAttributeMaxDynamicSharedMemorySize, Cfg<W::RB>::SMEM);
+      tc_pipeline_kernel<W>, cudaFuncAttributeMaxDynamicSharedMemorySize, CfgOf<W>::SMEM);
   if (attr != cudaSuccess) {
     zsb_set_error("%s: cudaFuncSetAttribute: %s", what, cudaGetErrorString(attr));
     return ZSB_ERR_CUDA;
@@ -462,7 +486,7 @@
     cl[0].val.clusterDim.z = 1;
     cudaLaunchConfig_t cfg = {};
     cfg.blockDim = dim3(NUM_THREADS);
-    cfg.dynamicSmemBytes = Cfg<W::RB>::SMEM;
+    cfg.dynamicSmemBytes = CfgOf<W>::SMEM;
     cfg.stream = st;
     cfg.attrs = cl;
     cfg.numAttrs = 1;
@@ -493,7 +517,7 @@
     int64_t grid = w.units();
     if (grid > sms) grid = sms;
     if (grid < 1) grid = 1;
-    tc_pipeline_kernel<W><<<(unsigned)grid, NUM_THREADS, Cfg<W::RB>::SMEM, st>>>(w);
+    tc_pipeline_kernel<W><<<(unsigned)grid, NUM_THREADS, CfgOf<W>::SMEM, st>>>(w);
     return zsb_check_launch(what);
   }
 }
diff --git a/zhusuan_b200/fused.py b/zhusuan_b200/fused.py
--- a/zhusuan_b200/fused.py
+++ b/zhusuan_b200/fused.py
@@ -60,6 +60,9 @@
         d["b_max"] = float(d["b"].abs().max()) if "b" in d else 0.0
         d["P_h16"] = torch.as_tensor(h16, device=device).contiguous()
         d["P_l16"] = torch.as_tensor(l16, device=device).contiguous()
+        if D % 64 == 0:
+            ilv = np.stack([h16.reshape(D, D // 32, 32), l16.reshape(D, D // 32, 32)], axis=2)
+            d["P_i16"] = torch.as_tensor(ilv.reshape(D, 2 * D), device=device).contiguous()
         self._zsb_fused = d
 
     def __call__(self, observed):
diff --git a/zhusuan_b200/hmc.py b/zhusuan_b200/hmc.py
--- a/zhusuan_b200/hmc.py
+++ b/zhusuan_b200/hmc.py
@@ -514,7 +514,7 @@
         self._k_part = z(nt * self._chains)
         self._ntiles = nt
         if self._res:
-            shape = (2,) + tuple(self._q[0].shape)
+            shape = (self._chains, 2 * D)
             self._planes = [torch.empty(shape, dtype=torch.float16, device=dev)
                             for _ in range(2)]
             self._spare = [torch.empty(shape, dtype=torch.float16, device=dev)
@@ -590,7 +590,7 @@
         lib.call("zsb_hmc_dense_resident_h16_f32", ptr(self._planes[0]),
                  ptr(self._planes[1]), ptr(self._spare[0]), ptr(self._spare[1]),
                  ptr(self._p0[0]), ptr(self._pw),
-                 ptr(f["P_h16"]), ptr(f["P_l16"]), ptr(self._scales), ptr(f.get("b")),
+                 ptr(f["P_i16"]), ptr(self._scales), ptr(f.get("b")),
                  ptr(f.get("mu")), ptr(self._mass[0]), ptr(self._state),
                  ptr(self._lp0_part), ptr(self._lp1_part), ptr(self._k_part),
                  self._chains, f["D"], L, s)
@@ -600,7 +600,7 @@
         q0 = self._q[0]
 
         def prepare():
-            lib.call("zsb_hmc_dense_traj_prepare_f32", ptr(q0), ptr(self._p0[0]),
+            lib.call("zsb_hmc_dense_resident_prepare_f32", ptr(q0), ptr(self._p0[0]),
                      ptr(self._mass[0]), ptr(self._planes[0]), ptr(self._scales),
                      self._chains, self._row_len[0], s)
         if init:
```
